# fonzcastellanos/scalable-video-codec

Measured on AMD Instinct MI355X. Metric: encoded frames/sec (1080p, 16x16 HBMA+DCT), higher is better.
Workload: dtype u8 (SAD, integer argmin) / f64 accumulate -> f32 (DCT, quant)

## Files before the change

### include/svc_hip.h

```cpp
#ifndef SVC_HIP_H
#define SVC_HIP_H

#include <stdint.h>

#ifdef __cplusplus
extern "C" {
#endif

typedef enum svc_status {
  SVC_OK = 0,
  SVC_ERR_INVALID_ARG = 1,
  SVC_ERR_UNSUPPORTED = 2,
  SVC_ERR_HIP = 3,
  SVC_ERR_NO_DEVICE = 4
} svc_status;

typedef struct svc_ransac_params {
  uint32_t subset_sz;
  float inlier_thresh;
  float success_prob;
  float inlier_ratio;
} svc_ransac_params;

typedef struct svc_segment_params {
// ... 4 lines not shown
  uint32_t max_iter_count;
  float epsilon;
  uint32_t connectivity;
} svc_segment_params;

#define SVC_HBMA_AUTO 0u
#define SVC_HBMA_FORCE_WAVE_PER_BLOCK 1u
#define SVC_HBMA_FORCE_FUSED 2u
#define SVC_HBMA_FORCE_TILED 4u
#define SVC_HBMA_FORCE_LANE 8u

const char* svc_hip_last_error(void);
int svc_hip_abi_version(void);
int svc_hip_device_count(int* count);

#define SVC_HOST_KEEP_LARGE_BLOCKS 1u
#define SVC_HOST_ONE_ARENA 2u
int svc_hip_tune_host_allocator(uint32_t flags);
int svc_hip_host_tuning_requested(void);

int svc_hip_probe_stream(const void* d_in, void* d_out, uint64_t bytes, uint32_t reads,
                         uint32_t writes, void* stream);

uint64_t svc_hip_pyramid_bytes(uint32_t frame_w, uint32_t frame_h, uint32_t level_count);


int svc_hip_hbma_pairs(const uint8_t* d_tracked, const uint8_t* d_anchor,
                       uint64_t pair_stride_bytes, uint32_t n_pairs,
                       uint32_t level_count, uint32_t frame_w, uint32_t frame_h,
                       uint32_t search_range, uint32_t block_w, uint32_t block_h,
                       float* d_mv_xy, float* d_min_mad, uint32_t flags,
                       void* stream);

const char* svc_hip_hbma_kernel_name(uint32_t level_count, uint32_t frame_w, uint32_t frame_h,
                                     uint32_t search_range, uint32_t block_w, uint32_t block_h,
                                     uint32_t flags);

int svc_hip_ebma_pairs(const uint8_t* d_tracked, const uint8_t* d_anchor,
                       uint64_t pair_stride_bytes, uint32_t n_pairs,
                       uint32_t frame_w, uint32_t frame_h, uint32_t search_range,
                       uint32_t block_w, uint32_t block_h, float* d_mv_xy,
                       float* d_min_mad, void* stream);

uint32_t svc_hip_ransac_iter_count(svc_ransac_params params);

int svc_hip_ransac_frames(const float* d_mv_xy, uint32_t blocks, uint32_t n_frames,
                          svc_ransac_params params, const uint32_t* d_samples,
                          uint32_t iter_count, float* d_gm_xy, float* d_rmse,
                          uint8_t* d_inlier_mask, uint32_t* d_inlier_count,
                          void* stream);

#define SVC_LAUNCH_BESIDE 1u
#define SVC_LAUNCH_NO_FORK 2u
#define SVC_LAUNCH_WIDE 4u
#define SVC_LAUNCH_NO_WIDE 8u
#define SVC_LAUNCH_DEFER_RMSE 16u
int svc_hip_ransac_frames_ex(const float* d_mv_xy, uint32_t blocks, uint32_t n_frames,
                             svc_ransac_params params, const uint32_t* d_samples,
                             uint32_t iter_count, float* d_gm_xy, float* d_rmse,
                             uint8_t* d_inlier_mask, uint32_t* d_inlier_count, uint32_t flags,
                             void* stream);

int svc_hip_ransac_rmse_frames(const float* d_mv_xy, uint32_t blocks, uint32_t n_frames,
                               svc_ransac_params params, const float* d_gm_xy,
                               const uint8_t* d_inlier_mask, const uint32_t* d_inlier_count,
                               float* d_rmse, void* stream);

int svc_hip_block_types_frames(const uint8_t* d_inlier_mask, uint32_t blocks,
                               uint32_t n_frames, uint32_t* d_block_types,
                               void* stream);

uint64_t svc_hip_segment_workspace_bytes(uint32_t mv_field_w, uint32_t mv_field_h,
                                         uint32_t n_frames, uint32_t attempt_count);

int svc_hip_segment_frames(const uint8_t* d_inlier_mask, const float* d_mv_xy,
                           uint32_t mv_field_w, uint32_t mv_field_h, uint32_t n_frames,
                           uint32_t mv_block_w, uint32_t mv_block_h,
                           svc_segment_params params, uint64_t seed,
                           uint8_t* d_workspace, uint64_t workspace_bytes,
                           uint32_t* d_block_types, void* stream);

int svc_hip_segment_frames_ex(const uint8_t* d_inlier_mask, const float* d_mv_xy,
                              uint32_t mv_field_w, uint32_t mv_field_h, uint32_t n_frames,
                              uint32_t mv_block_w, uint32_t mv_block_h,
                              svc_segment_params params, uint64_t seed,
                              uint8_t* d_workspace, uint64_t workspace_bytes,
                              uint32_t* d_block_types, uint32_t flags, void* stream);


int svc_hip_dct_frames(const uint8_t* d_bgr, uint64_t frame_stride_bytes,
                       uint32_t n_frames, uint32_t frame_w, uint32_t frame_h,
                       uint32_t block_w, uint32_t block_h, float* d_planes,
                       void* stream);

int svc_hip_dct_quant_frames(const uint8_t* d_bgr, uint64_t frame_stride_bytes,
                             uint32_t n_frames, uint32_t frame_w, uint32_t frame_h,
                             uint32_t block_w, uint32_t block_h,
                             const uint32_t* d_block_types, uint32_t mv_block_w,
                             uint32_t mv_block_h, uint32_t fg_step,
                             uint32_t bg_step, float* d_planes, void* stream);

int svc_hip_quant(float* d_coeffs, uint64_t n, uint32_t step, void* stream);

int svc_hip_quant_frames(float* d_planes, uint32_t n_frames, uint32_t frame_w,
                         uint32_t frame_h, uint32_t mv_block_w, uint32_t mv_block_h,
                         const uint32_t* d_block_types, uint32_t fg_step,
                         uint32_t bg_step, void* stream);


typedef struct svc_wire_header {
  uint32_t frame_count;
  uint32_t frame_w;
  uint32_t frame_h;
  uint32_t frame_excess_w;
  uint32_t frame_excess_h;
  uint32_t transform_block_w;
  uint32_t transform_block_h;
  uint32_t channel_count;
} svc_wire_header;

int svc_hip_wire_header(uint32_t clip_frame_count, uint32_t frame_w, uint32_t frame_h,
                        uint32_t mv_block_w, uint32_t mv_block_h, uint32_t level_count,
                        uint32_t transform_block_w, uint32_t transform_block_h,
                        svc_wire_header* out);

uint64_t svc_hip_serialized_frame_bytes(uint32_t frame_w, uint32_t frame_h,
                                        uint32_t transform_block_w, uint32_t transform_block_h);

int svc_hip_serialize_frames(const float* d_planes, uint64_t plane_elems, uint32_t n_frames,
                             const uint32_t* d_block_types, uint32_t frame_w, uint32_t frame_h,
                             uint32_t transform_block_w, uint32_t transform_block_h,
                             uint32_t mv_field_w, uint32_t mv_field_h, uint32_t mv_block_w,
                             uint32_t mv_block_h, uint8_t* d_out, uint64_t out_stride_bytes,
                             void* stream);

int svc_hip_dct_records_frames(const uint8_t* d_bgr, uint64_t frame_stride_bytes,
                               uint32_t n_frames, uint32_t frame_w, uint32_t frame_h,
                               uint32_t block, const uint32_t* d_block_types,
                               uint32_t mv_block_w, uint32_t mv_block_h, uint32_t fg_step,
                               uint32_t bg_step, uint32_t emit_frame_h, uint8_t* d_records,
                               uint64_t records_stride_bytes, void* stream);

int svc_hip_dct_records_luma_frames(const uint8_t* d_bgr, uint64_t frame_stride_bytes, uint32_t n_frames,
                                    uint32_t frame_w, uint32_t frame_h, uint32_t block, uint32_t emit_frame_h,
                                    uint8_t* d_records, uint64_t records_stride_bytes, uint8_t* d_pyr,
                                    uint64_t pyr_stride_bytes, void* stream);
int svc_hip_wire_patch_types_frames(const uint32_t* d_block_types, uint32_t n_frames, uint32_t frame_w, uint32_t frame_h,
                                    uint32_t emit_frame_h, uint32_t block, uint32_t mv_block_w, uint32_t mv_block_h,
                                    uint8_t* d_records, uint64_t records_stride_bytes, int all_tiles, void* stream);

int svc_hip_dct_quant_luma_frames(const uint8_t* d_bgr, uint64_t frame_stride_bytes, uint32_t n_frames, uint32_t frame_w,
                                  uint32_t frame_h, uint32_t block, uint32_t bg_step, float* d_planes, uint8_t* d_pyr,
                                  uint64_t pyr_stride_bytes, void* stream);
int svc_hip_count_foreground(const uint32_t* d_block_types, uint64_t n, uint32_t* d_count, void* stream);
uint64_t svc_hip_dct_redo_workspace_bytes(uint32_t n_frames, uint32_t frame_w, uint32_t frame_h, uint32_t mv_block_w,
                                          uint32_t mv_block_h);
int svc_hip_dct_quant_redo_frames(const uint8_t* d_bgr, uint64_t frame_stride_bytes, uint32_t n_frames, uint32_t frame_w,
                                  uint32_t frame_h, uint32_t block, const uint32_t* d_block_types, uint32_t mv_block_w,
                                  uint32_t mv_block_h, uint32_t fg_step, float* d_planes, uint8_t* d_ws, uint64_t ws_bytes,
                                  void* stream);

int svc_hip_decode_frames(const float* d_planes, uint32_t n_frames, uint32_t frame_w,
                          uint32_t frame_h, uint32_t block, const uint32_t* d_block_types,
                          uint32_t mv_block_w, uint32_t mv_block_h, uint32_t fg_step,
                          uint32_t bg_step, uint32_t gaze_x, uint32_t gaze_y, uint32_t gaze_w,
                          uint32_t gaze_h, float* d_bgr_f32, void* stream);

int svc_hip_sse_frames(const uint8_t* d_src_bgr, uint64_t src_frame_stride_bytes,
                       const float* d_rec_bgr_f32, uint32_t n_frames, uint32_t frame_w,
                       uint32_t frame_h, uint32_t region_w, uint32_t region_h, uint64_t* d_sse,
                       void* stream);


uint64_t svc_hip_levels_max_bytes(uint32_t n_frames, uint32_t frame_w, uint32_t frame_h,
                                  uint32_t block_w, uint32_t block_h, uint32_t mv_block_w,
                                  uint32_t mv_block_h);

uint64_t svc_hip_pack_levels_workspace_bytes(uint32_t n_frames, uint32_t frame_w,
                                             uint32_t frame_h, uint32_t block_w,
                                             uint32_t block_h);

int svc_hip_pack_levels_frames(const float* d_planes, const uint32_t* d_block_types,
                               uint32_t n_frames, uint32_t frame_w, uint32_t frame_h,
                               uint32_t block_w, uint32_t block_h, uint32_t mv_block_w,
                               uint32_t mv_block_h, uint32_t fg_step, uint32_t bg_step,
                               uint8_t* d_workspace, uint64_t workspace_bytes, uint8_t* d_out,
                               uint64_t out_capacity, uint64_t* d_frame_offsets, void* stream);

int svc_hip_unpack_levels_frames(const uint8_t* d_frames, uint64_t stream_bytes,
                                 const uint64_t* d_frame_offsets, uint32_t n_frames,
                                 uint32_t frame_w, uint32_t frame_h, uint32_t block_w,
                                 uint32_t block_h, uint32_t mv_block_w, uint32_t mv_block_h,
                                 uint8_t* d_workspace, uint64_t workspace_bytes, float* d_planes,
                                 uint32_t* d_block_types, uint32_t* d_status, void* stream);

int svc_hip_levels_drain(const uint8_t* d_frames, const uint64_t* d_frame_offsets,
                         uint32_t n_frames, uint32_t frame_w, uint32_t frame_h,
                         uint32_t block_w, uint32_t block_h, uint32_t mv_block_w,
                         uint32_t mv_block_h, void* host_dst, uint64_t capacity, void* stream);

uint64_t svc_hip_dct_pack_levels_workspace_bytes(uint32_t n_frames, uint32_t frame_w,
                                                 uint32_t frame_h, uint32_t block,
                                                 uint32_t mv_block_w, uint32_t mv_block_h);
int svc_hip_dct_pack_levels_frames(const uint8_t* d_bgr, uint64_t frame_stride_bytes,
                                   uint32_t n_frames, uint32_t frame_w, uint32_t frame_h,
                                   uint32_t block, const uint32_t* d_block_types,
                                   uint32_t mv_block_w, uint32_t mv_block_h, uint32_t fg_step,
                                   uint32_t bg_step, uint8_t* d_workspace,
                                   uint64_t workspace_bytes, uint8_t* d_out,
                                   uint64_t out_capacity, uint64_t* d_frame_offsets,
                                   void* stream);


uint64_t svc_hip_entropy_max_bytes(uint32_t n_frames, uint32_t frame_w, uint32_t frame_h, uint32_t block_w,
                                   uint32_t block_h, uint32_t mv_block_w, uint32_t mv_block_h);
uint64_t svc_hip_entropy_workspace_bytes(uint32_t n_frames, uint32_t frame_w, uint32_t frame_h, uint32_t block_w,
                                         uint32_t block_h, uint32_t mv_block_w, uint32_t mv_block_h);

int svc_hip_entropy_encode_frames(const uint8_t* d_svcq, uint64_t svcq_bytes, const uint64_t* d_svcq_offsets,
                                  uint32_t n_frames, uint32_t frame_w, uint32_t frame_h, uint32_t block_w,
                                  uint32_t block_h, uint32_t mv_block_w, uint32_t mv_block_h, uint8_t* d_workspace,
                                  uint64_t workspace_bytes, uint8_t* d_out, uint64_t out_capacity,
                                  uint64_t* d_out_offsets, uint32_t* d_status, void* stream);

int svc_hip_entropy_decode_frames(const uint8_t* d_svce, uint64_t svce_bytes, const uint64_t* d_offsets,
                                  uint32_t n_frames, uint32_t frame_w, uint32_t frame_h, uint32_t block_w,
                                  uint32_t block_h, uint32_t mv_block_w, uint32_t mv_block_h, uint8_t* d_workspace,
                                  uint64_t workspace_bytes, uint8_t* d_svcq_out, uint64_t capacity,
                                  uint64_t* d_svcq_offsets, uint32_t* d_status, void* stream);

int svc_hip_entropy_drain(const uint8_t* d_frames, const uint64_t* d_frame_offsets, uint32_t n_frames,
                          uint32_t frame_w, uint32_t frame_h, uint32_t block_w, uint32_t block_h,
                          uint32_t mv_block_w, uint32_t mv_block_h, void* host_dst, uint64_t capacity,
                          void* stream);

typedef struct {
  uint32_t fg_step, bg_step;
} svc_step_pair;

uint64_t svc_hip_pack_levels_budget_workspace_bytes(uint32_t n_frames, uint32_t frame_w, uint32_t frame_h,
                                                    uint32_t block_w, uint32_t block_h, uint32_t ladder_len);
int svc_hip_pack_levels_budget_frames(const float* d_planes, const uint32_t* d_block_types, uint32_t n_frames,
                                      uint32_t frame_w, uint32_t frame_h, uint32_t block_w, uint32_t block_h,
                                      uint32_t mv_block_w, uint32_t mv_block_h,
                                      const svc_step_pair* ladder , uint32_t ladder_len,
                                      const uint32_t* d_budget ,
                                      uint8_t* d_workspace, uint64_t workspace_bytes, uint8_t* d_out, uint64_t out_capacity,
                                      uint64_t* d_frame_offsets, uint32_t* d_choice , void* stream);

uint64_t svc_hip_dct_pack_levels_budget_workspace_bytes(uint32_t n_frames, uint32_t frame_w, uint32_t frame_h,
                                                        uint32_t block, uint32_t mv_block_w, uint32_t mv_block_h,
                                                        uint32_t ladder_len);
int svc_hip_dct_pack_levels_budget_frames(const uint8_t* d_bgr, uint64_t frame_stride_bytes, uint32_t n_frames,
                                          uint32_t frame_w, uint32_t frame_h, uint32_t block,
                                          const uint32_t* d_block_types, uint32_t mv_block_w, uint32_t mv_block_h,
                                          const svc_step_pair* ladder , uint32_t ladder_len,
                                          const uint32_t* d_budget ,
                                          uint8_t* d_workspace, uint64_t workspace_bytes, uint8_t* d_out, uint64_t out_capacity,
                                          uint64_t* d_frame_offsets, uint32_t* d_choice , void* stream);

uint64_t svc_hip_decode_levels_workspace_bytes(uint32_t n_frames, uint32_t frame_w,
                                               uint32_t frame_h, uint32_t block_w,
                                               uint32_t block_h);
int svc_hip_decode_levels_frames(const uint8_t* d_frames, uint64_t stream_bytes,
                                 const uint64_t* d_frame_offsets, uint32_t n_frames,
                                 uint32_t frame_w, uint32_t frame_h, uint32_t block_w,
                                 uint32_t block_h, uint32_t mv_block_w, uint32_t mv_block_h,
                                 uint32_t fg_step, uint32_t bg_step,
                                 const uint32_t* d_gaze ,
                                 uint8_t* d_workspace, uint64_t workspace_bytes,
                                 float* d_rec ,
                                 uint8_t* d_display ,
                                 uint32_t display_w, uint32_t display_h, uint32_t* d_status,
                                 void* stream);

int svc_hip_gaze_rect(uint32_t cx, uint32_t cy, uint32_t max_w, uint32_t max_h, uint32_t frame_w,
                      uint32_t frame_h, uint32_t padded_w, uint32_t padded_h,
                      uint32_t out_xywh[4]);

int svc_hip_decode_records_frames(const uint8_t* d_records, uint64_t records_stride_bytes, uint32_t n_frames,
                                  uint32_t frame_w, uint32_t frame_h , uint32_t block,
                                  uint32_t emit_frame_h, uint32_t fg_step, uint32_t bg_step,
                                  const uint32_t* d_gaze ,
                                  float* d_rec, uint8_t* d_display, uint32_t display_w, uint32_t display_h,
                                  void* stream);

int svc_hip_wire_layout(const svc_wire_header* hdr, uint64_t stream_bytes, uint32_t* emit_frame_h,
                        uint64_t* frame_bytes);

int svc_hip_luma_pyramid_frames(const uint8_t* d_bgr, uint64_t frame_stride_bytes,
                                uint32_t n_frames, uint32_t frame_w,
                                uint32_t frame_h, uint32_t level_count,
                                uint8_t* d_pyr, uint64_t pyr_stride_bytes,
                                void* stream);
int svc_hip_pyramid_levels_frames(uint8_t* d_pyr, uint64_t pyr_stride_bytes, uint32_t n_frames, uint32_t frame_w,
                                  uint32_t frame_h, uint32_t level_count, void* stream);

uint64_t svc_hip_global_ebma_workspace_bytes(uint32_t search_range, uint32_t n_pairs);

int svc_hip_global_ebma_pairs(const uint8_t* d_tracked, const uint8_t* d_anchor,
                              uint64_t pair_stride_bytes, uint32_t n_pairs, uint32_t frame_w,
                              uint32_t frame_h, uint32_t search_range, uint8_t* d_workspace,
                              uint64_t workspace_bytes, float* d_gm_xy, float* d_min_mad,
                              void* stream);

int svc_hip_global_avg_frames(const float* d_mv_xy, uint32_t blocks, uint32_t n_frames,
                              float* d_avg_xy, void* stream);

#define SVC_COMM_ID_BYTES 128u
#define SVC_SHIFT_CYCLIC 1u

int svc_hip_comm_available(void);
int svc_hip_comm_info(void* comm, uint32_t* ranks, uint32_t* rank, int32_t* device);
int svc_hip_comm_unique_id(uint8_t id[SVC_COMM_ID_BYTES]);
int svc_hip_comm_create(const uint8_t id[SVC_COMM_ID_BYTES], uint32_t rank, uint32_t world,
                        void** comm);
int svc_hip_comm_destroy(void* comm);

int svc_hip_halo_shift(void* comm, const uint8_t* d_send, uint8_t* d_recv, uint64_t bytes,
                       uint32_t rank, uint32_t world, uint32_t flags, void* stream);

int svc_hip_hbma_host(const uint8_t* const* tracked_pyr,
                      const uint8_t* const* anchor_pyr, uint32_t level_count,
                      uint32_t frame_w, uint32_t frame_h, uint32_t search_range,
                      uint32_t block_w, uint32_t block_h, float* mv_xy,
                      float* min_mad, uint32_t flags);

int svc_hip_ebma_host(const uint8_t* tracked, const uint8_t* anchor,
                      uint32_t frame_w, uint32_t frame_h, uint32_t search_range,
                      uint32_t block_w, uint32_t block_h, float* mv_xy,
                      float* min_mad);

int svc_hip_ransac_host(const float* mv_xy, uint32_t blocks,
                        svc_ransac_params params, const uint32_t* samples,
                        uint32_t iter_count, float* gm_xy, float* rmse,
                        uint32_t* inlier_indices, uint32_t* inlier_count);

int svc_hip_dct_host(const uint8_t* bgr, uint32_t frame_w, uint32_t frame_h,
                     uint32_t block_w, uint32_t block_h, float* planes);

int svc_hip_dct_planes_host(const uint8_t* bgr, uint32_t frame_w, uint32_t frame_h, uint32_t block_w,
                            uint32_t block_h, float* const planes[3]);


int svc_hip_bgr2yuv_host(const uint8_t* bgr, uint32_t w, uint32_t h, uint8_t* yuv);

int svc_hip_build_pyramid_host(const uint8_t* level0, uint32_t w, uint32_t h, uint32_t level_count,
                               uint8_t* const* out_levels);

#define SVC_MORPH_ERODE 0u
#define SVC_MORPH_DILATE 1u
#define SVC_MORPH_OPEN 2u
#define SVC_MORPH_CLOSE 3u
int svc_hip_morph_rect_host(const uint8_t* src, uint32_t w, uint32_t h, uint32_t kernel_w, uint32_t kernel_h,
                            uint32_t op, uint8_t* dst);

int svc_hip_kmeans_host(const float* features, uint32_t n, uint32_t dims, uint32_t k, uint32_t attempts,
                        uint32_t max_iter, float epsilon, uint64_t seed, int32_t* labels, double* compactness);

int svc_hip_connected_components_host(const uint8_t* image, uint32_t w, uint32_t h, uint32_t connectivity,
                                      int32_t* labels, uint32_t* count);

int svc_hip_dct_tiles_host(float* image, uint32_t w, uint32_t h, uint32_t block_w, uint32_t block_h,
                           const uint32_t* tiles_xy, uint32_t n_tiles);

int svc_hip_dct_quant_host(const uint8_t* bgr, uint32_t frame_w, uint32_t frame_h,
                           uint32_t block_w, uint32_t block_h,
                           const uint32_t* block_types, uint32_t mv_block_w,
                           uint32_t mv_block_h, uint32_t fg_step, uint32_t bg_step,
                           float* planes);

int svc_hip_quant_host(float* coeffs, uint64_t n, uint32_t step);

int svc_hip_global_ebma_host(const uint8_t* tracked, const uint8_t* anchor, uint32_t frame_w,
                             uint32_t frame_h, uint32_t search_range, float* gm_xy,
                             float* min_mad);

int svc_hip_global_hbma_host(const uint8_t* const* tracked_pyr,
                             const uint8_t* const* anchor_pyr, uint32_t level_count,
                             uint32_t frame_w, uint32_t frame_h, uint32_t search_range,
                             float* gm_xy);

int svc_hip_global_avg_host(const float* mv_xy, uint32_t blocks, float* avg_xy);

#ifdef __cplusplus
}
#endif

#endif
```

### scalable_video_codec_amd/csrc/capi.hip

```cpp
#include <algorithm>
#include <cmath>
#include <cstdlib>
#include <cstring>

#include <malloc.h>

#include "host/copy_crew.hpp"

#include <vector>
#include "svc_common.hpp"

namespace svc {

static thread_local char g_err[kErrBufSize] = "";
char* last_error_buf() { return g_err; }

bool fused_supported(uint32_t levels, uint32_t w, uint32_t h, uint32_t range, uint32_t bw, uint32_t bh);
bool tiled_supported(uint32_t levels, uint32_t w, uint32_t h, uint32_t range, uint32_t bw, uint32_t bh);
bool tiled_is_default();
int launch_hbma_fused(const uint8_t*, const uint8_t*, uint64_t, uint32_t, uint32_t, uint32_t, uint32_t,
                      uint32_t, uint32_t mv_block, float*, float*, int kernel, hipStream_t);
int launch_hbma_wave(const uint8_t*, const uint8_t*, uint64_t, uint32_t, uint32_t, uint32_t, uint32_t,
                     uint32_t, uint32_t, uint32_t, float*, float*, hipStream_t);

// ... 363 lines not shown
              (unsigned long long)svc_hip_segment_workspace_bytes(mv_field_w, mv_field_h, n_frames, params.attempt_count));
  SVC_REQUIRE(aligned(d_workspace, 16) && aligned(d_mv_xy, 8), "segment: workspace must be 16-byte, motion field 8-byte aligned");
  return launch_segment(d_inlier_mask, d_mv_xy, mv_field_w, mv_field_h, n_frames, mv_block_w, mv_block_h, params,
                        seed, d_workspace, d_block_types, flags, static_cast<hipStream_t>(stream));
}

static int validate_dct(const void* in, const void* out, uint32_t w, uint32_t h, uint32_t bw, uint32_t bh) {
  SVC_REQUIRE(in && out, "dct: null pointer");
  SVC_REQUIRE(bw > 0 && bh > 0, "dct: block must be positive (encoder.cpp:325-326)");
  SVC_REQUIRE(w > 0 && h > 0 && w % bw == 0 && h % bh == 0, "dct: frame %ux%u not divisible by block %ux%u", w, h, bw, bh);
  return SVC_OK;
}

static int validate_dct_alignment(const uint8_t* d_bgr, uint64_t frame_stride, const float* d_planes, uint32_t w, uint32_t bw,
                                  uint32_t bh) {
  if (bw == bh && (bw == 8 || bw == 16) && w % 16 == 0)
    SVC_REQUIRE(aligned(d_bgr, 16) && frame_stride % 16 == 0 && aligned(d_planes, 8),
                "dct: frames must be 16-byte aligned (stride too), planes 8-byte aligned");
  else
    SVC_REQUIRE(aligned(d_planes, 4), "dct: planes must be 4-byte aligned");
  return SVC_OK;
}

int svc_hip_dct_frames(const uint8_t* d_bgr, uint64_t frame_stride_bytes, uint32_t n_frames, uint32_t frame_w,
                       uint32_t frame_h, uint32_t block_w, uint32_t block_h, float* d_planes, void* stream) {
  if (n_frames == 0) return SVC_OK;
  int rc = validate_dct(d_bgr, d_planes, frame_w, frame_h, block_w, block_h);
  if (rc) return rc;
  rc = validate_dct_alignment(d_bgr, frame_stride_bytes, d_planes, frame_w, block_w, block_h);
  if (rc) return rc;
  return launch_dct(d_bgr, frame_stride_bytes, n_frames, frame_w, frame_h, block_w, block_h, nullptr, 0, 0, 1, 1,
                    false, d_planes, static_cast<hipStream_t>(stream));
}

int svc_hip_dct_quant_frames(const uint8_t* d_bgr, uint64_t frame_stride_bytes, uint32_t n_frames,
                             uint32_t frame_w, uint32_t frame_h, uint32_t block_w, uint32_t block_h,
                             const uint32_t* d_block_types, uint32_t mv_block_w, uint32_t mv_block_h,
                             uint32_t fg_step, uint32_t bg_step, float* d_planes, void* stream) {
  if (n_frames == 0) return SVC_OK;
  int rc = validate_dct(d_bgr, d_planes, frame_w, frame_h, block_w, block_h);
  if (rc) return rc;
  SVC_REQUIRE(d_block_types, "dct_quant: null block types");
  SVC_REQUIRE(fg_step > 0 && bg_step > 0, "dct_quant: quant steps must be positive (decoder.cpp:35-47)");
  SVC_REQUIRE(mv_block_w > 0 && mv_block_h > 0 && mv_block_w % block_w == 0 && mv_block_h % block_h == 0 &&
                  frame_w % mv_block_w == 0 && frame_h % mv_block_h == 0,
              "dct_quant: MV block %ux%u must be a multiple of the transform block %ux%u and divide the frame",
              mv_block_w, mv_block_h, block_w, block_h);
  rc = validate_dct_alignment(d_bgr, frame_stride_bytes, d_planes, frame_w, block_w, block_h);
  if (rc) return rc;
  return launch_dct(d_bgr, frame_stride_bytes, n_frames, frame_w, frame_h, block_w, block_h, d_block_types,
                    mv_block_w, mv_block_h, fg_step, bg_step, true, d_planes, static_cast<hipStream_t>(stream));
}

int svc_hip_dct_records_frames(const uint8_t* d_bgr, uint64_t frame_stride_bytes, uint32_t n_frames,
                               uint32_t frame_w, uint32_t frame_h, uint32_t block, const uint32_t* d_block_types,
                               uint32_t mv_block_w, uint32_t mv_block_h, uint32_t fg_step, uint32_t bg_step,
                               uint32_t emit_frame_h, uint8_t* d_records, uint64_t records_stride_bytes,
                               void* stream) {
  if (n_frames == 0) return SVC_OK;
  int rc = validate_dct(d_bgr, d_records, frame_w, frame_h, block, block);
  if (rc) return rc;
  SVC_REQUIRE(d_block_types, "dct_records: null block types");
  SVC_REQUIRE((fg_step == 0) == (bg_step == 0), "dct_records: give both quant steps or neither (0, 0 = no quant)");
  SVC_REQUIRE(mv_block_w > 0 && mv_block_h > 0 && mv_block_w % block == 0 && mv_block_h % block == 0 &&
                  frame_w % mv_block_w == 0 && frame_h % mv_block_h == 0,
              "dct_records: MV block %ux%u must be a multiple of the transform block %u and divide the frame",
              mv_block_w, mv_block_h, block);
  SVC_REQUIRE(emit_frame_h > 0 && emit_frame_h <= frame_h, "dct_records: emit_frame_h %u outside (0, %u]", emit_frame_h, frame_h);
  SVC_REQUIRE(aligned(d_bgr, 16) && frame_stride_bytes % 16 == 0 && aligned(d_records, 4) && records_stride_bytes % 4 == 0 &&
                  records_stride_bytes >= svc_hip_serialized_frame_bytes(frame_w, emit_frame_h, block, block),
              "dct_records: frames must be 16-byte aligned; records 4-byte aligned with a stride of at least one frame");
  const bool quant = fg_step != 0;
  return launch_dct(d_bgr, frame_stride_bytes, n_frames, frame_w, frame_h, block, block, d_block_types, mv_block_w,
                    mv_block_h, quant ? fg_step : 1, quant ? bg_step : 1, quant, nullptr,
                    static_cast<hipStream_t>(stream), d_records, records_stride_bytes, emit_frame_h);
}

int svc_hip_decode_frames(const float* d_planes, uint32_t n_frames, uint32_t frame_w, uint32_t frame_h,
                          uint32_t block, const uint32_t* d_block_types, uint32_t mv_block_w, uint32_t mv_block_h,
                          uint32_t fg_step, uint32_t bg_step, uint32_t gaze_x, uint32_t gaze_y, uint32_t gaze_w,
                          uint32_t gaze_h, float* d_bgr_f32, void* stream) {
  if (n_frames == 0) return SVC_OK;
  SVC_REQUIRE(d_planes && d_block_types && d_bgr_f32, "decode: null pointer");
  SVC_REQUIRE(block > 0 && frame_w > 0 && frame_h > 0 && frame_w % block == 0 && frame_h % block == 0,
              "decode: frame %ux%u not divisible by block %u", frame_w, frame_h, block);
  SVC_REQUIRE(fg_step > 0 && bg_step > 0, "decode: quant steps must be positive (libs/decoder.cpp:35-47)");
  SVC_REQUIRE(mv_block_w > 0 && mv_block_h > 0 && mv_block_w % block == 0 && mv_block_h % block == 0 &&
                  frame_w % mv_block_w == 0 && frame_h % mv_block_h == 0,
              "decode: MV block %ux%u must be a multiple of the transform block %u and divide the frame", mv_block_w, mv_block_h, block);
  SVC_REQUIRE(aligned(d_planes, 16) && aligned(d_bgr_f32, 8), "decode: planes must be 16-byte, output 8-byte aligned");
  return launch_decode(d_planes, n_frames, frame_w, frame_h, block, d_block_types, mv_block_w, mv_block_h, fg_step,
                       bg_step, gaze_x, gaze_y, gaze_w, gaze_h, d_bgr_f32, static_cast<hipStream_t>(stream));
}

int svc_hip_sse_frames(const uint8_t* d_src_bgr, uint64_t src_frame_stride_bytes, const float* d_rec_bgr_f32,
                       uint32_t n_frames, uint32_t frame_w, uint32_t frame_h, uint32_t region_w, uint32_t region_h,
                       uint64_t* d_sse, void* stream) {
  if (n_frames == 0) return SVC_OK;
  SVC_REQUIRE(d_src_bgr && d_rec_bgr_f32 && d_sse, "sse: null pointer");
  SVC_REQUIRE(region_w > 0 && region_h > 0 && region_w <= frame_w && region_h <= frame_h,
              "sse: region %ux%u outside the frame %ux%u", region_w, region_h, frame_w, frame_h);
  SVC_REQUIRE(aligned(d_sse, 8), "sse: output must be 8-byte aligned");
  return launch_sse(d_src_bgr, src_frame_stride_bytes, d_rec_bgr_f32, n_frames, frame_w, frame_h, region_w, region_h,
                    d_sse, static_cast<hipStream_t>(stream));
}

int svc_hip_quant(float* d_coeffs, uint64_t n, uint32_t step, void* stream) {
  SVC_REQUIRE(d_coeffs || n == 0, "quant: null pointer");
  SVC_REQUIRE(step > 0, "quant: step must be positive (decoder.cpp:35-47)");
  return launch_quant(d_coeffs, n, step, static_cast<hipStream_t>(stream));
}

int svc_hip_quant_frames(float* d_planes, uint32_t n_frames, uint32_t frame_w, uint32_t frame_h,
                         uint32_t mv_block_w, uint32_t mv_block_h, const uint32_t* d_block_types,
                         uint32_t fg_step, uint32_t bg_step, void* stream) {
  if (n_frames == 0) return SVC_OK;
  SVC_REQUIRE(d_planes && d_block_types, "quant_frames: null pointer");
  SVC_REQUIRE(fg_step > 0 && bg_step > 0, "quant_frames: steps must be positive");
  SVC_REQUIRE(mv_block_w > 0 && mv_block_h > 0 && frame_w % mv_block_w == 0 && frame_h % mv_block_h == 0,
              "quant_frames: frame %ux%u not divisible by MV block %ux%u", frame_w, frame_h, mv_block_w, mv_block_h);
  return launch_quant_frames(d_planes, n_frames, frame_w, frame_h, mv_block_w, mv_block_h, d_block_types,
                             fg_step, bg_step, static_cast<hipStream_t>(stream));
}

int svc_hip_luma_pyramid_frames(const uint8_t* d_bgr, uint64_t frame_stride_bytes, uint32_t n_frames,
                                uint32_t frame_w, uint32_t frame_h, uint32_t level_count, uint8_t* d_pyr,
                                uint64_t pyr_stride_bytes, void* stream) {
  if (n_frames == 0) return SVC_OK;
  SVC_REQUIRE(d_bgr && d_pyr, "luma_pyramid: null pointer");
  SVC_REQUIRE(level_count > 0 && level_count <= 16, "luma_pyramid: level_count %u out of range", level_count);
  const uint32_t f = 1u << (level_count - 1);
  SVC_REQUIRE(frame_w > 0 && frame_h > 0 && frame_w % f == 0 && frame_h % f == 0,
              "luma_pyramid: frame %ux%u must be divisible by 2^(levels-1) = %u", frame_w, frame_h, f);
  SVC_REQUIRE(aligned(d_bgr, 16) && frame_stride_bytes % 16 == 0 && aligned(d_pyr, 16) && pyr_stride_bytes % 16 == 0,
              "luma_pyramid: frames and pyramids must be 16-byte aligned (strides too)");
  SVC_REQUIRE(n_frames <= 1 || pyr_stride_bytes >= pyramid_bytes(frame_w, frame_h, level_count),
              "luma_pyramid: pyramid stride too small");
  return launch_luma_pyramid(d_bgr, frame_stride_bytes, n_frames, frame_w, frame_h, level_count, d_pyr,
                             pyr_stride_bytes, static_cast<hipStream_t>(stream));
}

int svc_hip_pyramid_levels_frames(uint8_t* d_pyr, uint64_t pyr_stride_bytes, uint32_t n_frames, uint32_t frame_w, uint32_t frame_h,
                                  uint32_t level_count, void* stream) {
  if (n_frames == 0) return SVC_OK;
  SVC_REQUIRE(d_pyr, "pyramid_levels: null pointer");
  SVC_REQUIRE(level_count > 0 && level_count <= 16, "pyramid_levels: level_count %u out of range", level_count);
  const uint32_t f = 1u << (level_count - 1);
  SVC_REQUIRE(frame_w > 0 && frame_h > 0 && frame_w % f == 0 && frame_h % f == 0,
              "pyramid_levels: frame %ux%u must be divisible by 2^(levels-1) = %u", frame_w, frame_h, f);
  SVC_REQUIRE(n_frames <= 1 || pyr_stride_bytes >= pyramid_bytes(frame_w, frame_h, level_count), "pyramid_levels: pyramid stride too small");
  return launch_pyr_down_levels(d_pyr, pyr_stride_bytes, n_frames, frame_w, frame_h, level_count, 0, static_cast<hipStream_t>(stream));
}

int svc_hip_dct_records_luma_frames(const uint8_t* d_bgr, uint64_t frame_stride_bytes, uint32_t n_frames, uint32_t frame_w,
                                    uint32_t frame_h, uint32_t block, uint32_t emit_frame_h, uint8_t* d_records,
                                    uint64_t records_stride_bytes, uint8_t* d_pyr, uint64_t pyr_stride_bytes, void* stream) {
  if (n_frames == 0) return SVC_OK;
  int rc = validate_dct(d_bgr, d_records, frame_w, frame_h, block, block);
  if (rc) return rc;
  SVC_REQUIRE(d_pyr, "dct_records_luma: null pyramid");
  SVC_REQUIRE(emit_frame_h > 0 && emit_frame_h <= frame_h, "dct_records_luma: emit_frame_h %u outside (0, %u]", emit_frame_h, frame_h);
  SVC_REQUIRE(aligned(d_bgr, 16) && frame_stride_bytes % 16 == 0 && aligned(d_records, 4) && records_stride_bytes % 4 == 0 &&
                  records_stride_bytes >= svc_hip_serialized_frame_bytes(frame_w, emit_frame_h, block, block),
              "dct_records_luma: frames must be 16-byte aligned; records 4-byte aligned with a stride of at least one frame");
  SVC_REQUIRE(aligned(d_pyr, 16) && pyr_stride_bytes % 16 == 0 && (n_frames <= 1 || pyr_stride_bytes >= (uint64_t)frame_w * frame_h),
              "dct_records_luma: pyramids must be 16-byte aligned (stride too), a stride of at least one luma plane");
  return launch_dct(d_bgr, frame_stride_bytes, n_frames, frame_w, frame_h, block, block, nullptr, block, block, 1, 1, false, nullptr,
                    static_cast<hipStream_t>(stream), d_records, records_stride_bytes, emit_frame_h, d_pyr, pyr_stride_bytes);
}

int svc_hip_dct_quant_luma_frames(const uint8_t* d_bgr, uint64_t frame_stride_bytes, uint32_t n_frames, uint32_t frame_w,
                                  uint32_t frame_h, uint32_t block, uint32_t bg_step, float* d_planes, uint8_t* d_pyr,
                                  uint64_t pyr_stride_bytes, void* stream) {
  if (n_frames == 0) return SVC_OK;
  int rc = validate_dct(d_bgr, d_planes, frame_w, frame_h, block, block);
  if (rc) return rc;
  SVC_REQUIRE(d_pyr, "dct_quant_luma: null pyramid");
  SVC_REQUIRE(bg_step > 0, "dct_quant_luma: quant step must be positive (libs/decoder.cpp:35-47)");
  if ((rc = validate_dct_alignment(d_bgr, frame_stride_bytes, d_planes, frame_w, block, block))) return rc;
  SVC_REQUIRE(aligned(d_pyr, 16) && pyr_stride_bytes % 16 == 0 && (n_frames <= 1 || pyr_stride_bytes >= (uint64_t)frame_w * frame_h),
              "dct_quant_luma: pyramids must be 16-byte aligned (stride too), a stride of at least one luma plane");
  return launch_dct_quant_speculative(d_bgr, frame_stride_bytes, n_frames, frame_w, frame_h, block, bg_step, d_planes, d_pyr,
                                      pyr_stride_bytes, static_cast<hipStream_t>(stream));
}

int svc_hip_count_foreground(const uint32_t* d_block_types, uint64_t n, uint32_t* d_count, void* stream) {
  SVC_REQUIRE(d_count && (d_block_types || n == 0), "count_foreground: null pointer");
  return launch_count_foreground(d_block_types, n, d_count, static_cast<hipStream_t>(stream));
}

uint64_t svc_hip_dct_redo_workspace_bytes(uint32_t n_frames, uint32_t frame_w, uint32_t frame_h, uint32_t mv_block_w, uint32_t mv_block_h) {
  if (!mv_block_w || !mv_block_h) return 0;
  return dct_redo_workspace_bytes(n_frames, (frame_w / mv_block_w) * (frame_h / mv_block_h));
}

int svc_hip_dct_quant_redo_frames(const uint8_t* d_bgr, uint64_t frame_stride_bytes, uint32_t n_frames, uint32_t frame_w, uint32_t frame_h,
                                  uint32_t block, const uint32_t* d_block_types, uint32_t mv_block_w, uint32_t mv_block_h,
                                  uint32_t fg_step, float* d_planes, uint8_t* d_ws, uint64_t ws_bytes, void* stream) {
  if (n_frames == 0) return SVC_OK;
  int rc = validate_dct(d_bgr, d_planes, frame_w, frame_h, block, block);
  if (rc) return rc;
  SVC_REQUIRE(d_block_types && d_ws, "dct_quant_redo: null pointer");
  SVC_REQUIRE(fg_step > 0, "dct_quant_redo: quant step must be positive (libs/decoder.cpp:35-47)");
  SVC_REQUIRE(mv_block_w > 0 && mv_block_h > 0 && mv_block_w % block == 0 && mv_block_h % block == 0 &&
                  frame_w % mv_block_w == 0 && frame_h % mv_block_h == 0,
              "dct_quant_redo: MV block %ux%u must be a multiple of the transform block %u and divide the frame", mv_block_w, mv_block_h, block);
  if ((rc = validate_dct_alignment(d_bgr, frame_stride_bytes, d_planes, frame_w, block, block))) return rc;
  SVC_REQUIRE(aligned(d_ws, 16) && ws_bytes >= svc_hip_dct_redo_workspace_bytes(n_frames, frame_w, frame_h, mv_block_w, mv_block_h),
              "dct_quant_redo: workspace must be 16-byte aligned and hold svc_hip_dct_redo_workspace_bytes()");
  return launch_dct_quant_redo_foreground(d_bgr, frame_stride_bytes, n_frames, frame_w, frame_h, block, d_block_types, mv_block_w, mv_block_h,
                                          fg_step, d_planes, d_ws, static_cast<hipStream_t>(stream));
}

int svc_hip_wire_patch_types_frames(const uint32_t* d_block_types, uint32_t n_frames, uint32_t frame_w, uint32_t frame_h,
                                    uint32_t emit_frame_h, uint32_t block, uint32_t mv_block_w, uint32_t mv_block_h, uint8_t* d_records,
                                    uint64_t records_stride_bytes, int all_tiles, void* stream) {
  if (n_frames == 0) return SVC_OK;
  SVC_REQUIRE(d_block_types && d_records, "wire_patch_types: null pointer");
  SVC_REQUIRE(block > 0 && frame_w > 0 && frame_h > 0 && frame_w % block == 0 && frame_h % block == 0 && block <= 64,
              "wire_patch_types: frame %ux%u not divisible by block %u", frame_w, frame_h, block);
  SVC_REQUIRE(mv_block_w > 0 && mv_block_h > 0 && mv_block_w % block == 0 && mv_block_h % block == 0 &&
                  frame_w % mv_block_w == 0 && frame_h % mv_block_h == 0,
              "wire_patch_types: MV block %ux%u must be a multiple of the transform block %u and divide the frame", mv_block_w, mv_block_h, block);
  SVC_REQUIRE(emit_frame_h > 0 && emit_frame_h <= frame_h, "wire_patch_types: emit_frame_h %u outside (0, %u]", emit_frame_h, frame_h);
  SVC_REQUIRE(aligned(d_records, 4) && records_stride_bytes % 4 == 0 &&
                  records_stride_bytes >= svc_hip_serialized_frame_bytes(frame_w, emit_frame_h, block, block),
              "wire_patch_types: records 4-byte aligned with a stride of at least one frame");
  return launch_wire_patch_types(d_block_types, n_frames, frame_w, frame_h, emit_frame_h, block, mv_block_w, mv_block_h, d_records,
                                 records_stride_bytes, all_tiles != 0, static_cast<hipStream_t>(stream));
}


static int validate_global_ebma(uint32_t w, uint32_t h, uint32_t range) {
  SVC_REQUIRE(w > 0 && h > 0, "global ebma: frame %ux%u must be positive", w, h);
  SVC_REQUIRE(range < w && range < h, "global ebma: search range %u must be smaller than the frame %ux%u (motion.cpp:63-64)", range, w, h);
  SVC_REQUIRE(range <= 1024, "global ebma: search range %u out of range", range);
  return SVC_OK;
}

uint64_t svc_hip_global_ebma_workspace_bytes(uint32_t search_range, uint32_t n_pairs) {
  return global_ebma_workspace_bytes(search_range, n_pairs);
}

int svc_hip_global_ebma_pairs(const uint8_t* d_tracked, const uint8_t* d_anchor, uint64_t pair_stride_bytes, uint32_t n_pairs,
                              uint32_t frame_w, uint32_t frame_h, uint32_t search_range, uint8_t* d_workspace,
                              uint64_t workspace_bytes, float* d_gm_xy, float* d_min_mad, void* stream) {
  if (n_pairs == 0) return SVC_OK;
  SVC_REQUIRE(d_tracked && d_anchor && d_gm_xy && d_workspace, "global ebma: null pointer (motion.cpp:58-61)");
  int rc = validate_global_ebma(frame_w, frame_h, search_range);
  if (rc) return rc;
  SVC_REQUIRE(workspace_bytes >= global_ebma_workspace_bytes(search_range, n_pairs) && aligned(d_workspace, 8),
              "global ebma: workspace too small or not 8-byte aligned");
  return launch_global_ebma(d_tracked, d_anchor, pair_stride_bytes, n_pairs, frame_w, frame_h, search_range, d_workspace,
                            d_gm_xy, d_min_mad, false, static_cast<hipStream_t>(stream));
}

int svc_hip_global_avg_frames(const float* d_mv_xy, uint32_t blocks, uint32_t n_frames, float* d_avg_xy, void* stream) {
  if (n_frames == 0) return SVC_OK;
  SVC_REQUIRE(d_mv_xy && d_avg_xy, "global avg: null pointer (motion.cpp:46)");
  return launch_global_avg(d_mv_xy, blocks, n_frames, d_avg_xy, static_cast<hipStream_t>(stream));
}

int svc_hip_hbma_host(const uint8_t* const* tracked_pyr, const uint8_t* const* anchor_pyr, uint32_t level_count,
                      uint32_t frame_w, uint32_t frame_h, uint32_t search_range, uint32_t block_w,
                      uint32_t block_h, float* mv_xy, float* min_mad, uint32_t flags) {
  SVC_REQUIRE(tracked_pyr && anchor_pyr && mv_xy && min_mad, "hbma: null pointer (motion.cpp:417-420)");
  int rc = validate_hbma(level_count, frame_w, frame_h, search_range, block_w, block_h);
  if (rc) return rc;
  for (uint32_t l = 0; l < level_count; ++l)
    SVC_REQUIRE(tracked_pyr[l] && anchor_pyr[l], "hbma: null plane at level %u", l);
  if ((rc = require_device())) return rc;
  const size_t pyr = up256(pyramid_bytes(frame_w, frame_h, level_count));
  const size_t blocks = (size_t)(frame_w / block_w) * (frame_h / block_h);
  const size_t out_off = 2 * pyr, out_bytes = blocks * 12;
  if ((rc = g_stage.ensure(out_off + up256(out_bytes)))) return rc;
  size_t o = 0;
  for (uint32_t l = 0; l < level_count; ++l) {
    const size_t n = (size_t)(frame_w >> l) * (frame_h >> l);
    host_copy(g_stage.pin + o, tracked_pyr[l], n);
    host_copy(g_stage.pin + pyr + o, anchor_pyr[l], n);
    o += n;
  }
  SVC_HIP_TRY(hipMemcpyAsync(g_stage.dev, g_stage.pin, 2 * pyr, hipMemcpyHostToDevice, g_stage.stream));
  float* d_mv = reinterpret_cast<float*>(g_stage.dev + out_off);
  float* d_mad = d_mv + 2 * blocks;
  rc = launch_hbma(g_stage.dev, g_stage.dev + pyr, pyr, 1, level_count, frame_w, frame_h, search_range, block_w,
                   block_h, d_mv, d_mad, flags, g_stage.stream);
  if (rc) return rc;
  SVC_HIP_TRY(hipMemcpyAsync(g_stage.pin + out_off, d_mv, out_bytes, hipMemcpyDeviceToHost, g_stage.stream));
  SVC_HIP_TRY(hipStreamSynchronize(g_stage.stream));
  std::memcpy(mv_xy, g_stage.pin + out_off, blocks * 8);
  std::memcpy(min_mad, g_stage.pin + out_off + blocks * 8, blocks * 4);
  return SVC_OK;
}

int svc_hip_ebma_host(const uint8_t* tracked, const uint8_t* anchor, uint32_t frame_w, uint32_t frame_h,
                      uint32_t search_range, uint32_t block_w, uint32_t block_h, float* mv_xy, float* min_mad) {
  SVC_REQUIRE(tracked && anchor && mv_xy && min_mad, "ebma: null pointer (motion.cpp:273-276)");
  SVC_REQUIRE(block_w > 0 && block_h > 0, "ebma: block must be positive (motion.cpp:278-279)");
  SVC_REQUIRE(frame_w > 0 && frame_h > 0 && frame_w % block_w == 0 && frame_h % block_h == 0,
              "ebma: frame %ux%u not divisible by block %ux%u (motion.cpp:281-282)", frame_w, frame_h, block_w, block_h);
  int rc = require_device();
  if (rc) return rc;
  const size_t plane = up256((size_t)frame_w * frame_h);
  const size_t blocks = (size_t)(frame_w / block_w) * (frame_h / block_h);
  const size_t out_off = 2 * plane, out_bytes = blocks * 12;
  if ((rc = g_stage.ensure(out_off + up256(out_bytes)))) return rc;
  host_copy(g_stage.pin, tracked, (size_t)frame_w * frame_h);
  host_copy(g_stage.pin + plane, anchor, (size_t)frame_w * frame_h);
  SVC_HIP_TRY(hipMemcpyAsync(g_stage.dev, g_stage.pin, 2 * plane, hipMemcpyHostToDevice, g_stage.stream));
  float* d_mv = reinterpret_cast<float*>(g_stage.dev + out_off);
  float* d_mad = d_mv + 2 * blocks;
  rc = launch_ebma(g_stage.dev, g_stage.dev + plane, plane, 1, frame_w, frame_h, search_range, block_w, block_h,
                   d_mv, d_mad, g_stage.stream);
  if (rc) return rc;
  SVC_HIP_TRY(hipMemcpyAsync(g_stage.pin + out_off, d_mv, out_bytes, hipMemcpyDeviceToHost, g_stage.stream));
  SVC_HIP_TRY(hipStreamSynchronize(g_stage.stream));
  std::memcpy(mv_xy, g_stage.pin + out_off, blocks * 8);
  std::memcpy(min_mad, g_stage.pin + out_off + blocks * 8, blocks * 4);
  return SVC_OK;
}

int svc_hip_ransac_host(const float* mv_xy, uint32_t blocks, svc_ransac_params params, const uint32_t* samples,
                        uint32_t iter_count, float* gm_xy, float* rmse, uint32_t* inlier_indices,
                        uint32_t* inlier_count) {
  SVC_REQUIRE(mv_xy && gm_xy && rmse && inlier_indices && inlier_count, "ransac: null pointer (motion.cpp:189-192)");
  SVC_REQUIRE(iter_count == 0 || samples, "ransac: null samples");
  SVC_REQUIRE(params.subset_sz > 0 && blocks >= params.subset_sz,
              "ransac: motion field of %u smaller than subset %u (motion.cpp:194)", blocks, params.subset_sz);
  for (size_t i = 0; i < (size_t)iter_count * params.subset_sz; ++i)
    SVC_REQUIRE(samples[i] < blocks, "ransac: sample index %u out of range [0, %u)", samples[i], blocks);
  int rc = require_device();
  if (rc) return rc;
  const size_t mv_b = up256((size_t)blocks * 8), smp_b = up256((size_t)iter_count * params.subset_sz * 4 + 4);
  const size_t mask_b = up256(blocks), misc_b = 256;
  if ((rc = g_stage.ensure(mv_b + smp_b + mask_b + misc_b))) return rc;
// ... 168 lines not shown
```

### scalable_video_codec_amd/csrc/dct.hip

```cpp
#include <algorithm>

#include "dct_core.hpp"
#include "luma16.hpp"
#include "quant_core.hpp"
#include "svc_common.hpp"

namespace svc {

struct DctArgs {
  const uint8_t* bgr;
  uint64_t frame_stride;
  uint32_t w, h;
  uint32_t segs_per_band;
  uint32_t bands_per_frame;
  uint32_t total_segcols;
  float* planes;
  const uint32_t* types;
  uint32_t mv_bw, mv_bh, mfw, mv_blocks;
  float fg_step, bg_step;
  float fg_inv, bg_inv;
  uint8_t* records;
  uint64_t records_stride;
  uint32_t emit_bands;
  uint8_t* luma;
  uint64_t luma_stride;
  const uint32_t* fg_list;
  const uint32_t* fg_count;
  uint32_t segs_per_block_x, segs_per_block;
};



constexpr int kSlabWire8 = 1664, kSlabWire16 = 3200;

typedef uint32_t u32x4_a4 __attribute__((ext_vector_type(4), aligned(4)));

template <int N, bool QUANT, bool WIRE, bool LUMA = false, int SPEC = 0>
__global__ __launch_bounds__(256) void dct_kernel(DctArgs a) {
  static_assert(!LUMA || (WIRE && !QUANT) || (QUANT && !WIRE && SPEC == 1), "the luma by-product rides on the raw-coefficient record emitter or on the speculative quantiser");
  static_assert(SPEC == 0 || (QUANT && !WIRE), "speculation is about the quantiser's step");
  constexpr int kSegPerWg = 256 / N;
  constexpr int kSlab = WIRE ? (N == 8 ? kSlabWire8 : kSlabWire16) : (N == 8 ? kSlab8 : kSlab16);
  __shared__ __attribute__((aligned(16))) uint8_t lds[kSegPerWg * kSlab];

  const uint32_t tid = threadIdx.x;
  const uint32_t sc_local = tid / N, j = tid % N;
  uint32_t n_units = 1, unit = 0;
  if (SPEC == 2) {
    const uint32_t total = *a.fg_count * a.segs_per_block;
    n_units = (total + kSegPerWg - 1) / kSegPerWg;
    unit = blockIdx.x;
  }
  for (; unit < n_units; unit += SPEC == 2 ? gridDim.x : 1u) {
  uint32_t gsc, frame, band, seg;
  if (SPEC == 2) {
    gsc = unit * kSegPerWg + sc_local;
    if (gsc >= *a.fg_count * a.segs_per_block) break;
    const uint32_t item = a.fg_list[gsc / a.segs_per_block], sub = gsc % a.segs_per_block;
    frame = item / a.mv_blocks;
    const uint32_t b = item - frame * a.mv_blocks, by = b / a.mfw, bx = b - by * a.mfw;
    band = by * (a.mv_bh / N) + sub / a.segs_per_block_x;
    seg = bx * a.segs_per_block_x + sub % a.segs_per_block_x;
  } else {
    gsc = xcd_contiguous_block(blockIdx.x, gridDim.x) * kSegPerWg + sc_local;
    if (gsc >= a.total_segcols) return;
    const uint32_t band_g = gsc / a.segs_per_band;
    seg = gsc - band_g * a.segs_per_band;
    frame = band_g / a.bands_per_frame;
    band = band_g - frame * a.bands_per_frame;
  }
  const uint32_t y_pix = band * N, x_pix = seg * 16;

  const uint8_t* src = a.bgr + (size_t)frame * a.frame_stride +
                       ((size_t)(y_pix + j) * a.w + x_pix) * 3;
  uint32_t wds[12];
  {
    const uint4* p = reinterpret_cast<const uint4*>(src);
    uint4 v0 = p[0], v1 = p[1], v2 = p[2];
    wds[0] = v0.x; wds[1] = v0.y; wds[2] = v0.z; wds[3] = v0.w;
    wds[4] = v1.x; wds[5] = v1.y; wds[6] = v1.z; wds[7] = v1.w;
    wds[8] = v2.x; wds[9] = v2.y; wds[10] = v2.z; wds[11] = v2.w;
  }

  if (LUMA) {
    uint32_t y16[4];
    luma16(wds, y16);
    *reinterpret_cast<uint4*>(a.luma + (size_t)frame * a.luma_stride + (size_t)(y_pix + j) * a.w + x_pix) = make_uint4(y16[0], y16[1], y16[2], y16[3]);
  }

  uint8_t* slab = lds + sc_local * kSlab;
  float* out_frame = a.planes + (size_t)frame * 3 * a.w * a.h;

  float step = 1.f, inv_step = 1.f;
  uint32_t t = SPEC == 2 ? 1u : 0u;
  if ((QUANT || WIRE) && !LUMA && SPEC == 0) {
    const uint32_t col = N == 8 ? x_pix + 2 * j : x_pix + j;
    t = a.types[(size_t)frame * a.mv_blocks + (y_pix / a.mv_bh) * a.mfw + col / a.mv_bw];
  }
  if (QUANT) {
    step = t == 0 ? a.bg_step : a.fg_step;
    inv_step = t == 0 ? a.bg_inv : a.fg_inv;
  }
  constexpr uint32_t kRec = 4 + 12 * N * N;
  const bool emit = WIRE && band < a.emit_bands;
  uint8_t* rec0 = nullptr;
  if (WIRE) {
    const uint32_t tiles_x = a.w / N, tile0 = band * tiles_x + (N == 8 ? 2 * seg : seg);
    rec0 = a.records + (size_t)frame * a.records_stride + (size_t)tile0 * kRec;
  }
  float keep[WIRE ? 3 : 1][16];

#pragma unroll
  for (int c = 0; c < 3; ++c) {
    int x[16];
    double r[16];
#pragma unroll
    for (int p = 0; p < 16; ++p) x[p] = (int)((wds[(3 * p + c) >> 2] >> (8 * ((3 * p + c) & 3))) & 0xFFu);
    if (N == 8) {
      dct1d<8, int>(x, r);
      dct1d<8, int>(x + 8, r + 8);
    } else {
      dct1d<16, int>(x, r);
    }
    double2* row = reinterpret_cast<double2*>(slab + j * kRowPitch);
#pragma unroll
    for (int i = 0; i < 8; ++i) row[i] = make_double2(r[2 * i], r[2 * i + 1]);
    wave_lds_sync();

    float* plane = out_frame + (size_t)c * a.w * a.h;
    if (N == 8) {
      double ca[8], cb[8], ya[8], yb[8];
#pragma unroll
      for (int y = 0; y < 8; ++y) {
        double2 t = *reinterpret_cast<const double2*>(slab + y * kRowPitch + j * 16);
        ca[y] = t.x;
        cb[y] = t.y;
      }
      dct1d<8, double>(ca, ya);
      dct1d<8, double>(cb, yb);
      float* dst = plane + (size_t)y_pix * a.w + x_pix + 2 * j;
#pragma unroll
      for (int v = 0; v < 8; ++v) {
        float fa = (float)ya[v], fb = (float)yb[v];
        if (QUANT) {
          const f32x2 qq = quant2_fast(f32x2{fa, fb}, step, inv_step);
          fa = qq.x; fb = qq.y;
        }
        if (WIRE) { keep[WIRE ? c : 0][2 * v] = fa; keep[WIRE ? c : 0][2 * v + 1] = fb; }
        else *reinterpret_cast<float2*>(dst + (size_t)v * a.w) = make_float2(fa, fb);
      }
    } else {
      double cc[16], yy[16];
#pragma unroll
      for (int y = 0; y < 16; ++y)
        cc[y] = *reinterpret_cast<const double*>(slab + y * kRowPitch + j * 8);
      dct1d<16, double>(cc, yy);
      float* dst = plane + (size_t)y_pix * a.w + x_pix + j;
#pragma unroll
      for (int v = 0; v < 16; v += 2) {
        f32x2 f = {(float)yy[v], (float)yy[v + 1]};
        if (QUANT) f = quant2_fast(f, step, inv_step);
        if (WIRE) {
          keep[WIRE ? c : 0][v] = f.x;
          keep[WIRE ? c : 0][v + 1] = f.y;
        } else {
          dst[(size_t)v * a.w] = f.x;
          dst[(size_t)(v + 1) * a.w] = f.y;
        }
      }
    }
    wave_lds_sync();
  }

  if constexpr (WIRE) {
    constexpr uint32_t kGroupBytes = N == 8 ? 2 * kRec : kRec;
    constexpr uint32_t kGroups = 64 / N;
    constexpr uint32_t kWaveBytes = kGroups * kGroupBytes;
    static_assert(kGroups * (uint32_t)kSlab >= kWaveBytes + 16, "a wave's slabs hold its stretch of the stream plus alignment slack");
    const uint32_t lane = tid & 63u, g = lane / N;
    const uint32_t gsc_last = gsc - g + kGroups - 1;
    bool stretch = gsc_last < a.total_segcols;
    if (stretch) {
      const uint32_t bg_last = gsc_last / a.segs_per_band, bg_first = (gsc - g) / a.segs_per_band;
      const uint32_t f_last = bg_last / a.bands_per_frame;
      stretch = f_last == bg_first / a.bands_per_frame && bg_last - f_last * a.bands_per_frame < a.emit_bands;
    }
    const uint32_t q = N == 8 ? j >> 2 : 0u;
    const uint32_t col_off = N == 8 ? (j & 3u) * 8u : j * 4u;
    if (stretch) {
      uint8_t* wave_rec = rec0 - (size_t)g * kGroupBytes;
      const uint32_t delta = (uint32_t)(reinterpret_cast<uintptr_t>(wave_rec) & 15u);
      uint8_t* wbase = lds + (sc_local - g) * kSlab + delta;
      uint8_t* mine = wbase + g * kGroupBytes + q * kRec;
      if (N == 8 ? (j & 3u) == 0 : j == 0) *reinterpret_cast<uint32_t*>(mine) = t;
#pragma unroll
      for (int c = 0; c < 3; ++c)
#pragma unroll
        for (int v = 0; v < N; ++v) {
          uint32_t* d = reinterpret_cast<uint32_t*>(mine + 4 + c * (4 * N * N) + v * (4 * N) + col_off);
          if (N == 8) { d[0] = __float_as_uint(keep[c][2 * v]); d[1] = __float_as_uint(keep[c][2 * v + 1]); }
          else d[0] = __float_as_uint(keep[c][v]);
        }
      wave_lds_sync();
      const uint32_t head = (16u - delta) & 15u;
      const uint32_t nfull = (kWaveBytes - head) / 16u, tail = (kWaveBytes - head) % 16u;
      for (uint32_t k = lane; k < nfull; k += 64u) {
        const uint32_t o = head + 16u * k;
        *reinterpret_cast<uint4*>(wave_rec + o) = *reinterpret_cast<const uint4*>(wbase + o);
      }
      const uint32_t hd = head / 4u, ne = hd + tail / 4u;
      if (lane < ne) {
        const uint32_t o = lane < hd ? 4u * lane : head + 16u * nfull + 4u * (lane - hd);
        *reinterpret_cast<uint32_t*>(wave_rec + o) = *reinterpret_cast<const uint32_t*>(wbase + o);
      }
    } else if (emit) {
      uint8_t* mine = rec0 + q * kRec;
      if (N == 8 ? (j & 3u) == 0 : j == 0) *reinterpret_cast<uint32_t*>(mine) = t;
#pragma unroll
      for (int c = 0; c < 3; ++c)
#pragma unroll
        for (int v = 0; v < N; ++v) {
          uint32_t* d = reinterpret_cast<uint32_t*>(mine + 4 + c * (4 * N * N) + v * (4 * N) + col_off);
          if (N == 8) { d[0] = __float_as_uint(keep[c][2 * v]); d[1] = __float_as_uint(keep[c][2 * v + 1]); }
          else d[0] = __float_as_uint(keep[c][v]);
        }
    }
  }
  }
}

__global__ __launch_bounds__(256) void fg_list_kernel(const uint32_t* types, uint32_t total_blocks, uint32_t* list, uint32_t* count) {
  const uint32_t g = blockIdx.x * 256u + threadIdx.x;
  const bool fg = g < total_blocks && types[g] != 0;
  const uint64_t m = __builtin_amdgcn_ballot_w64(fg);
  if (m == 0) return;
  const uint32_t lane = threadIdx.x & 63u, n = (uint32_t)__builtin_popcountll(m);
  uint32_t base = 0;
  if (lane == (uint32_t)__builtin_ctzll(m)) base = atomicAdd(count, n);
  base = __builtin_amdgcn_readlane(base, __builtin_ctzll(m));
  if (fg) list[base + (uint32_t)__builtin_popcountll(m & ((1ull << lane) - 1ull))] = g;
}

struct DctGenArgs {
  const uint8_t* bgr;
  uint64_t frame_stride;
  uint32_t w, h, bw, bh;
  uint32_t sw;
  uint32_t strips_per_band;
  uint32_t bands_per_frame;
  uint32_t total_strips;
  float* planes;
  const uint32_t* types;
  uint32_t mv_bw, mv_bh, mfw, mv_blocks;
  float fg_step, bg_step, fg_inv, bg_inv;
  uint8_t* records;
  uint64_t records_stride;
  uint32_t emit_bands;
};

__device__ __forceinline__ double dct_basis(uint32_t k, uint32_t n, uint32_t N) {
  const uint32_t j = ((2 * n + 1) * k) % (4 * N);
  const double s = k == 0 ? 1.0 / (double)N : 2.0 / (double)N;
  return __builtin_sqrt(s) * cospi((double)j / (double)(2 * N));
}

template <bool QUANT, bool WIRE>
__global__ __launch_bounds__(256) void dct_general_kernel(DctGenArgs a) {
  extern __shared__ __attribute__((aligned(16))) uint8_t gen_lds[];
  const uint32_t tid = threadIdx.x, bw = a.bw, bh = a.bh, sw = a.sw;
  const uint32_t pw = bw + 1, ph = bh + 1;
  double* cw = reinterpret_cast<double*>(gen_lds);
  double* ch = cw + bw * pw;
  double* yrow = ch + bh * ph;
  float* xin = reinterpret_cast<float*>(yrow + bh * sw);
  for (uint32_t i = tid; i < bw * bw; i += 256) cw[(i / bw) * pw + i % bw] = dct_basis(i / bw, i % bw, bw);
  for (uint32_t i = tid; i < bh * bh; i += 256) ch[(i / bh) * ph + i % bh] = dct_basis(i / bh, i % bh, bh);
  __syncthreads();
  for (uint32_t unit = blockIdx.x; unit < a.total_strips; unit += gridDim.x) {
    const uint32_t band_g = unit / a.strips_per_band, strip = unit - band_g * a.strips_per_band;
    const uint32_t frame = band_g / a.bands_per_frame, band = band_g - frame * a.bands_per_frame;
    const uint32_t y0 = band * bh, x0 = strip * sw;
    const uint32_t cols = a.w - x0 < sw ? a.w - x0 : sw;
    const uint32_t n = bh * cols;
    const uint8_t* src = a.bgr + (size_t)frame * a.frame_stride;
    float* out_frame = a.planes + (size_t)frame * 3 * a.w * a.h;
    for (uint32_t c = 0; c < 3; ++c) {
      for (uint32_t i = tid; i < n; i += 256) {
        const uint32_t r = i / cols, x = i - r * cols;
        xin[r * sw + x] = (float)src[((size_t)(y0 + r) * a.w + x0 + x) * 3 + c];
      }
      __syncthreads();
      for (uint32_t i = tid; i < n; i += 256) {
        const uint32_t r = i / cols, x = i - r * cols, u = x % bw;
        const float* xr = xin + r * sw + (x - u);
        const double* cr = cw + u * pw;
        double acc = 0.0;
        for (uint32_t k = 0; k < bw; ++k) acc = __builtin_fma(cr[k], (double)xr[k], acc);
        yrow[r * sw + x] = acc;
      }
      __syncthreads();
      float* plane = out_frame + (size_t)c * a.w * a.h;
      for (uint32_t i = tid; i < n; i += 256) {
        const uint32_t v = i / cols, x = i - v * cols;
        const double* cr = ch + v * ph;
        double acc = 0.0;
        for (uint32_t m = 0; m < bh; ++m) acc = __builtin_fma(cr[m], yrow[m * sw + x], acc);
        float f = (float)acc;
        uint32_t t = 0;
        if (QUANT || WIRE)
          t = a.types[(size_t)frame * a.mv_blocks + (y0 / a.mv_bh) * a.mfw + (x0 + x) / a.mv_bw];
        if (QUANT) f = quant1_fast(f, t == 0 ? a.bg_step : a.fg_step, t == 0 ? a.bg_inv : a.fg_inv);
        if (WIRE) {
          if (band < a.emit_bands) {
            const uint32_t u = x % bw, tile = band * (a.w / bw) + (x0 + x) / bw, rec_dw = 1 + 3 * bw * bh;
            uint32_t* rec = reinterpret_cast<uint32_t*>(a.records + (size_t)frame * a.records_stride) + (size_t)tile * rec_dw;
            rec[1 + c * bw * bh + v * bh + u] = __float_as_uint(f);
            if (c == 0 && v == 0 && u == 0) rec[0] = t;
          }
        } else {
          plane[(size_t)(y0 + v) * a.w + x0 + x] = f;
        }
      }
      __syncthreads();
    }
  }
}

constexpr uint32_t kDctGenMaxSide = 64;

static int launch_dct_general(const uint8_t* d_bgr, uint64_t frame_stride, uint32_t n_frames, uint32_t w, uint32_t h,
                              uint32_t bw, uint32_t bh, const uint32_t* d_types, uint32_t mv_bw, uint32_t mv_bh,
                              uint32_t fg_step, uint32_t bg_step, bool quant, float* d_planes, hipStream_t stream,
                              uint8_t* d_records = nullptr, uint64_t records_stride = 0, uint32_t emit_h = 0) {
  const bool wire = d_records != nullptr;
  if (wire && (bw != bh || w % bw != 0))
    return fail(SVC_ERR_UNSUPPORTED, "dct_records: the fused record emitter takes square transform blocks that divide the frame "
                                     "width; for %ux%u call svc_hip_dct[_quant]_frames, then svc_hip_serialize_frames", bw, bh);
  if ((bw > 1 && bw % 2) || (bh > 1 && bh % 2) || (bw == 1 && bh == 1))
    return fail(SVC_ERR_INVALID_ARG, "dct: transform block %ux%u: cv::dct implements even sizes only", bw, bh);
  if (bw > kDctGenMaxSide || bh > kDctGenMaxSide)
    return fail(SVC_ERR_UNSUPPORTED, "dct: transform block %ux%u exceeds %ux%u", bw, bh, kDctGenMaxSide, kDctGenMaxSide);
  DctGenArgs a{};
  a.bgr = d_bgr; a.frame_stride = frame_stride;
  a.w = w; a.h = h; a.bw = bw; a.bh = bh;
  uint32_t tiles = 4096 / (bw * bh);
  if (tiles < 1) tiles = 1;
  if (tiles > w / bw) tiles = w / bw;
  a.sw = tiles * bw;
  a.strips_per_band = div_up(w, a.sw);
  a.bands_per_frame = h / bh;
  const uint64_t total = (uint64_t)n_frames * a.strips_per_band * a.bands_per_frame;
  if (total == 0) return SVC_OK;
  if (total > 0x7FFFFFFFull) return fail(SVC_ERR_UNSUPPORTED, "dct: %llu strips exceed one launch", (unsigned long long)total);
  a.total_strips = (uint32_t)total;
  a.planes = d_planes;
  a.records = d_records;
  a.records_stride = records_stride;
  a.emit_bands = wire ? div_up(emit_h, bh) : 0;
  if (quant || wire) {
    a.types = d_types;
    a.mv_bw = mv_bw; a.mv_bh = mv_bh;
    a.mfw = w / mv_bw;
    a.mv_blocks = a.mfw * (h / mv_bh);
  }
  if (quant) {
    a.fg_step = (float)fg_step; a.bg_step = (float)bg_step;
    a.fg_inv = 1.0f / a.fg_step; a.bg_inv = 1.0f / a.bg_step;
  }
  const size_t lds = 8 * ((size_t)bw * (bw + 1) + (size_t)bh * (bh + 1) + (size_t)bh * a.sw) + 4 * (size_t)bh * a.sw;
  const uint32_t grid = (uint32_t)(total < 4096 ? total : 4096);
  if (wire) {
    if (quant) hipLaunchKernelGGL((dct_general_kernel<true, true>), dim3(grid), dim3(256), lds, stream, a);
    else hipLaunchKernelGGL((dct_general_kernel<false, true>), dim3(grid), dim3(256), lds, stream, a);
  } else {
    if (quant) hipLaunchKernelGGL((dct_general_kernel<true, false>), dim3(grid), dim3(256), lds, stream, a);
    else hipLaunchKernelGGL((dct_general_kernel<false, false>), dim3(grid), dim3(256), lds, stream, a);
  }
  return check_launch("dct_general_kernel");
}

int launch_dct(const uint8_t* d_bgr, uint64_t frame_stride, uint32_t n_frames, uint32_t w,
               uint32_t h, uint32_t bw, uint32_t bh, const uint32_t* d_types, uint32_t mv_bw,
               uint32_t mv_bh, uint32_t fg_step, uint32_t bg_step, bool quant, float* d_planes,
               hipStream_t stream, uint8_t* d_records, uint64_t records_stride, uint32_t emit_h, uint8_t* d_luma,
               uint64_t luma_stride) {
  const bool wire = d_records != nullptr;
  const bool fast = bw == bh && (bw == 8 || bw == 16) && w % 16 == 0;
  if (d_luma && !(fast && wire && !quant))
    return fail(SVC_ERR_UNSUPPORTED, "dct: the luma by-product needs the tuned record emitter (8x8 / 16x16 blocks, width a multiple of 16, no quant)");
  if (!fast)
    return launch_dct_general(d_bgr, frame_stride, n_frames, w, h, bw, bh, d_types, mv_bw, mv_bh, fg_step, bg_step, quant,
                              d_planes, stream, d_records, records_stride, emit_h);
  DctArgs a{};
  a.bgr = d_bgr;
  a.frame_stride = frame_stride;
  a.w = w; a.h = h;
  a.segs_per_band = w / 16;
  a.bands_per_frame = h / bh;
  const uint64_t total = (uint64_t)n_frames * a.segs_per_band * a.bands_per_frame;
  if (total == 0) return SVC_OK;
  if (total > 0x7FFFFFFFull) return fail(SVC_ERR_UNSUPPORTED, "dct: %llu segment columns exceed one launch", (unsigned long long)total);
  a.total_segcols = (uint32_t)total;
  a.planes = d_planes;
  a.records = d_records;
  a.records_stride = records_stride;
  a.emit_bands = wire ? div_up(emit_h, bh) : 0;
  a.luma = d_luma;
  a.luma_stride = luma_stride;
  if (quant || wire) {
    a.types = d_types;
    a.mv_bw = mv_bw; a.mv_bh = mv_bh;
    a.mfw = w / mv_bw;
    a.mv_blocks = a.mfw * (h / mv_bh);
  }
  if (quant) {
    a.fg_step = (float)fg_step;
    a.bg_step = (float)bg_step;
    a.fg_inv = 1.0f / a.fg_step;
    a.bg_inv = 1.0f / a.bg_step;
  }
  const uint32_t seg_per_wg = 256 / bw;
  const dim3 grid(div_up(a.total_segcols, seg_per_wg)), block(256);
#define SVC_DCT_LAUNCH(N_, Q_, W_) hipLaunchKernelGGL((dct_kernel<N_, Q_, W_>), grid, block, 0, stream, a)
  if (d_luma) {
    if (bw == 8) hipLaunchKernelGGL((dct_kernel<8, false, true, true>), grid, block, 0, stream, a);
    else hipLaunchKernelGGL((dct_kernel<16, false, true, true>), grid, block, 0, stream, a);
  } else if (bw == 8) {
    if (wire) { if (quant) SVC_DCT_LAUNCH(8, true, true); else SVC_DCT_LAUNCH(8, false, true); }
    else { if (quant) SVC_DCT_LAUNCH(8, true, false); else SVC_DCT_LAUNCH(8, false, false); }
  } else {
    if (wire) { if (quant) SVC_DCT_LAUNCH(16, true, true); else SVC_DCT_LAUNCH(16, false, true); }
    else { if (quant) SVC_DCT_LAUNCH(16, true, false); else SVC_DCT_LAUNCH(16, false, false); }
  }
#undef SVC_DCT_LAUNCH
  return check_launch("dct_kernel");
}

__global__ __launch_bounds__(256) void fg_count_kernel(const uint32_t* types, uint32_t total_blocks, uint32_t* count) {
  __shared__ uint32_t part[4];
  uint32_t n = 0;
  for (uint32_t g = blockIdx.x * 256u + threadIdx.x; g < total_blocks; g += gridDim.x * 256u) n += types[g] != 0 ? 1u : 0u;
#pragma unroll
  for (int o = 32; o > 0; o >>= 1) n += __shfl_down(n, o, 64);
  if ((threadIdx.x & 63u) == 0) part[threadIdx.x >> 6] = n;
  __syncthreads();
  if (threadIdx.x == 0) {
    const uint32_t s = part[0] + part[1] + part[2] + part[3];
    if (s) atomicAdd(count, s);
  }
}

int launch_count_foreground(const uint32_t* d_types, uint64_t n, uint32_t* d_count, hipStream_t stream) {
  hipError_t e = hipMemsetAsync(d_count, 0, 4, stream);
  if (e != hipSuccess) return fail(SVC_ERR_HIP, "count_foreground: hipMemsetAsync: %s", hipGetErrorString(e));
  if (n == 0) return SVC_OK;
  if (n > 0x7FFFFFFFull) return fail(SVC_ERR_UNSUPPORTED, "count_foreground: too many MV blocks for one launch");
  hipLaunchKernelGGL(fg_count_kernel, dim3(std::min<uint32_t>(div_up((uint32_t)n, 1024), 512u)), dim3(256), 0, stream, d_types, (uint32_t)n, d_count);
  return check_launch("fg_count_kernel");
}

static bool spec_shape_ok(uint32_t w, uint32_t block) { return (block == 8 || block == 16) && w % 16 == 0; }

int launch_dct_quant_speculative(const uint8_t* d_bgr, uint64_t frame_stride, uint32_t n_frames, uint32_t w, uint32_t h, uint32_t block,
                                 uint32_t bg_step, float* d_planes, uint8_t* d_luma, uint64_t luma_stride, hipStream_t stream) {
  if (!spec_shape_ok(w, block))
    return fail(SVC_ERR_UNSUPPORTED, "dct_quant_luma: the speculative form needs the tuned transform (8x8 / 16x16 blocks, width a multiple of 16)");
  DctArgs a{};
  a.bgr = d_bgr; a.frame_stride = frame_stride;
  a.w = w; a.h = h;
  a.segs_per_band = w / 16;
  a.bands_per_frame = h / block;
  const uint64_t total = (uint64_t)n_frames * a.segs_per_band * a.bands_per_frame;
  if (total == 0) return SVC_OK;
  if (total > 0x7FFFFFFFull) return fail(SVC_ERR_UNSUPPORTED, "dct: %llu segment columns exceed one launch", (unsigned long long)total);
  a.total_segcols = (uint32_t)total;
  a.planes = d_planes;
  a.luma = d_luma; a.luma_stride = luma_stride;
  a.fg_step = a.bg_step = (float)bg_step;
  a.fg_inv = a.bg_inv = 1.0f / a.bg_step;
  const dim3 grid(div_up(a.total_segcols, 256 / block)), blk(256);
  if (block == 8) hipLaunchKernelGGL((dct_kernel<8, true, false, true, 1>), grid, blk, 0, stream, a);
  else hipLaunchKernelGGL((dct_kernel<16, true, false, true, 1>), grid, blk, 0, stream, a);
  return check_launch("dct_kernel<speculative>");
}

uint64_t dct_redo_workspace_bytes(uint32_t n_frames, uint32_t mv_blocks) { return 16 + 4ull * n_frames * mv_blocks; }

int launch_dct_quant_redo_foreground(const uint8_t* d_bgr, uint64_t frame_stride, uint32_t n_frames, uint32_t w, uint32_t h, uint32_t block,
                                     const uint32_t* d_types, uint32_t mv_bw, uint32_t mv_bh, uint32_t fg_step, float* d_planes,
                                     uint8_t* d_ws, hipStream_t stream) {
  if (!spec_shape_ok(w, block) || mv_bw % 16 != 0 || mv_bh % block != 0)
    return fail(SVC_ERR_UNSUPPORTED, "dct_quant_redo: needs the tuned transform (8x8 / 16x16, width a multiple of 16) and MV blocks that are whole "
                                     "16-pixel segments wide and whole transform blocks tall");
  DctArgs a{};
  a.bgr = d_bgr; a.frame_stride = frame_stride;
  a.w = w; a.h = h;
  a.segs_per_band = w / 16;
  a.bands_per_frame = h / block;
  a.planes = d_planes;
  a.mv_bw = mv_bw; a.mv_bh = mv_bh;
  a.mfw = w / mv_bw;
  a.mv_blocks = a.mfw * (h / mv_bh);
  const uint64_t total_blocks = (uint64_t)n_frames * a.mv_blocks;
  if (total_blocks == 0) return SVC_OK;
  if (total_blocks * (mv_bw / 16) * (mv_bh / block) > 0x7FFFFFFFull) return fail(SVC_ERR_UNSUPPORTED, "dct_quant_redo: too many MV blocks for one launch");
  a.fg_step = a.bg_step = (float)fg_step;
  a.fg_inv = a.bg_inv = 1.0f / a.fg_step;
  uint32_t* count = reinterpret_cast<uint32_t*>(d_ws);
  uint32_t* list = reinterpret_cast<uint32_t*>(d_ws + 16);
  a.fg_count = count; a.fg_list = list;
  a.segs_per_block_x = mv_bw / 16;
  a.segs_per_block = a.segs_per_block_x * (mv_bh / block);
  hipError_t e = hipMemsetAsync(count, 0, 16, stream);
  if (e != hipSuccess) return fail(SVC_ERR_HIP, "dct_quant_redo: hipMemsetAsync: %s", hipGetErrorString(e));
  hipLaunchKernelGGL(fg_list_kernel, dim3(div_up((uint32_t)total_blocks, 256)), dim3(256), 0, stream, d_types, (uint32_t)total_blocks, list, count);
  int rc = check_launch("fg_list_kernel");
  if (rc) return rc;
  const uint64_t worst = div_up((uint32_t)(total_blocks * a.segs_per_block), 256 / block);
  const dim3 grid((uint32_t)std::min<uint64_t>(worst, 2048)), blk(256);
  if (block == 8) hipLaunchKernelGGL((dct_kernel<8, true, false, false, 2>), grid, blk, 0, stream, a);
  else hipLaunchKernelGGL((dct_kernel<16, true, false, false, 2>), grid, blk, 0, stream, a);
  return check_launch("dct_kernel<redo foreground>");
}

struct DctTilesArgs {
  float* img;
  const uint32_t* xy;
  uint32_t w, h, bw, bh, n_tiles, grid_w, tpb;
};

__global__ __launch_bounds__(256) void dct_tiles_kernel(DctTilesArgs a) {
  extern __shared__ __attribute__((aligned(16))) uint8_t tiles_lds[];
  const uint32_t tid = threadIdx.x, bw = a.bw, bh = a.bh, area = bw * bh;
  const uint32_t pw = bw + 1, ph = bh + 1;
  double* cw = reinterpret_cast<double*>(tiles_lds);
  double* ch = cw + bw * pw;
  double* yrow = ch + bh * ph;
  float* xin = reinterpret_cast<float*>(yrow + (size_t)a.tpb * area);
  for (uint32_t i = tid; i < bw * bw; i += 256) cw[(i / bw) * pw + i % bw] = dct_basis(i / bw, i % bw, bw);
  for (uint32_t i = tid; i < bh * bh; i += 256) ch[(i / bh) * ph + i % bh] = dct_basis(i / bh, i % bh, bh);
  __syncthreads();
  for (uint32_t base = blockIdx.x * a.tpb; base < a.n_tiles; base += gridDim.x * a.tpb) {
    const uint32_t nt = a.n_tiles - base < a.tpb ? a.n_tiles - base : a.tpb, ne = nt * area;
    auto origin = [&](uint32_t t, uint32_t& tx, uint32_t& ty) {
      const uint32_t g = base + t;
      if (a.xy) { tx = a.xy[2 * g]; ty = a.xy[2 * g + 1]; }
      else { ty = (g / a.grid_w) * bh; tx = (g % a.grid_w) * bw; }
    };
    for (uint32_t i = tid; i < ne; i += 256) {
      const uint32_t t = i / area, e = i - t * area, r = e / bw, u = e - r * bw;
      uint32_t tx, ty;
      origin(t, tx, ty);
      xin[i] = a.img[(size_t)(ty + r) * a.w + tx + u];
    }
    __syncthreads();
    for (uint32_t i = tid; i < ne; i += 256) {
      const uint32_t t = i / area, e = i - t * area, r = e / bw, u = e - r * bw;
      const float* xr = xin + t * area + r * bw;
      const double* cr = cw + u * pw;
      double acc = 0.0;
      for (uint32_t k = 0; k < bw; ++k) acc = __builtin_fma(cr[k], (double)xr[k], acc);
      yrow[i] = acc;
    }
    __syncthreads();
    for (uint32_t i = tid; i < ne; i += 256) {
      const uint32_t t = i / area, e = i - t * area, v = e / bw, u = e - v * bw;
      const double* cr = ch + v * ph;
      const double* yc = yrow + t * area + u;
      double acc = 0.0;
      for (uint32_t m = 0; m < bh; ++m) acc = __builtin_fma(cr[m], yc[m * bw], acc);
      uint32_t tx, ty;
      origin(t, tx, ty);
      a.img[(size_t)(ty + v) * a.w + tx + u] = (float)acc;
    }
    __syncthreads();
  }
}

int launch_dct_tiles(float* d_img, uint32_t w, uint32_t h, uint32_t bw, uint32_t bh, const uint32_t* d_xy, uint32_t n_tiles,
                     hipStream_t stream) {
  if ((bw > 1 && bw % 2) || (bh > 1 && bh % 2) || (bw == 1 && bh == 1) || bw == 0 || bh == 0)
    return fail(SVC_ERR_INVALID_ARG, "dct: transform block %ux%u: cv::dct implements even sizes only", bw, bh);
  if (bw > kDctGenMaxSide || bh > kDctGenMaxSide)
    return fail(SVC_ERR_UNSUPPORTED, "dct: transform block %ux%u exceeds %ux%u", bw, bh, kDctGenMaxSide, kDctGenMaxSide);
  if (n_tiles == 0) return SVC_OK;
  DctTilesArgs a{};
  a.img = d_img; a.xy = d_xy;
  a.w = w; a.h = h; a.bw = bw; a.bh = bh; a.n_tiles = n_tiles;
  a.grid_w = w / bw;
  uint32_t tpb = 4096 / (bw * bh);
  a.tpb = tpb < 1 ? 1 : tpb > 64 ? 64 : tpb;
  const size_t lds = 8 * ((size_t)bw * (bw + 1) + (size_t)bh * (bh + 1)) + (size_t)a.tpb * bw * bh * 12;
  const uint32_t trips = div_up(n_tiles, a.tpb);
  hipLaunchKernelGGL(dct_tiles_kernel, dim3(trips < 2048 ? trips : 2048), dim3(256), lds, stream, a);
  return check_launch("dct_tiles_kernel");
}


__global__ __launch_bounds__(256) void quant_kernel(float* c, uint64_t n, float step) {
  const uint64_t stride = (uint64_t)gridDim.x * 256 * 4;
  for (uint64_t i = ((uint64_t)blockIdx.x * 256 + threadIdx.x) * 4; i < n; i += stride) {
    if (i + 4 <= n && (reinterpret_cast<uintptr_t>(c + i) & 15) == 0) {
      float4 v = *reinterpret_cast<float4*>(c + i);
      v.x = quant1(v.x, step); v.y = quant1(v.y, step);
      v.z = quant1(v.z, step); v.w = quant1(v.w, step);
      *reinterpret_cast<float4*>(c + i) = v;
    } else {
      for (uint64_t k = i; k < n && k < i + 4; ++k) c[k] = quant1(c[k], step);
    }
  }
}

struct QuantFramesArgs {
  float* planes;
  const uint32_t* types;
  uint32_t w, h, mv_bw, mv_bh, mfw, mv_blocks;
  uint64_t total;
  float fg_step, bg_step;
};

__global__ __launch_bounds__(256) void quant_frames_kernel(QuantFramesArgs a) {
  const uint64_t stride = (uint64_t)gridDim.x * 256;
  const uint64_t plane_sz = (uint64_t)a.w * a.h;
  for (uint64_t i = (uint64_t)blockIdx.x * 256 + threadIdx.x; i < a.total; i += stride) {
    const uint64_t pl = i / plane_sz, rem = i - pl * plane_sz;
    const uint32_t frame = (uint32_t)(pl / 3);
    const uint32_t y = (uint32_t)(rem / a.w), x = (uint32_t)(rem - (uint64_t)y * a.w);
    const uint32_t t = a.types[(size_t)frame * a.mv_blocks + (y / a.mv_bh) * a.mfw + x / a.mv_bw];
    a.planes[i] = quant1(a.planes[i], t == 0 ? a.bg_step : a.fg_step);
  }
}

// ... 29 lines not shown
```

### scalable_video_codec_amd/csrc/host/clip_encoder.cpp

```cpp
#include "svc/clip_encoder.hpp"

#include <algorithm>
#include <cstring>
#include <stdexcept>
#include <string>
#include <utility>
#include <vector>

#include "encode_geometry.hpp"
#include "hip_raii.hpp"
#include "svc_clip.h"

namespace svc {
namespace {

using namespace host;

constexpr Who kWho{"svc::ClipEncoder"};
void Hip(hipError_t e, const char* what) { kWho.Hip(e, what); }
void Abi(int rc, const char* what) { kWho.Abi(rc, what); }
bool Ready(hipEvent_t e) { return kWho.Ready(e); }

constexpr uint32_t kStages = (uint32_t)Stage::kCount;

}

Shard PlanShard(uint32_t clip_frames, uint32_t world, uint32_t rank) {
  Shard s;
  if (world == 0 || rank >= world) return s;
  const uint32_t base = clip_frames / world, extra = clip_frames % world;
  s.frames = base + (rank < extra ? 1u : 0u);
  s.first_frame = rank * base + std::min(rank, extra);
  s.needs_halo = s.first_frame > 0 && s.frames > 0;
  s.pairs = s.frames == 0 ? 0 : s.frames - (s.needs_halo ? 0u : 1u);
  s.first_encoded = s.needs_halo ? s.first_frame : s.first_frame + 1;
  return s;
}

struct ClipEncoder::Impl : EncodeGeometry {
  ClipEncoderConfig c;
  Shard sh;
  uint32_t iters = 0;
  uint64_t record_bytes = 0, seg_ws_bytes = 0;
  static constexpr int kMaxDepth = 3, kSets = kMaxDepth + 2;
  int depth = 1, nsets = 1;
  uint32_t nch = 1, cp = 0;
  struct Micro { uint32_t step = 0, p0 = 0, pn = 0; bool first = true; uint8_t order = 0; const uint8_t* frames = nullptr; };
  static constexpr int kRing = 8;
  Micro ring[kRing], next_micro;
  uint32_t n_steps = 0;
  const uint8_t* step_frames = nullptr;
  Event e_step[kRing];
  uint64_t step_last_micro[kRing] = {};
  void MarkStepDone(uint64_t d) {
    const uint32_t s = StepOf(d);
    if (step_last_micro[s % kRing] == d) Hip(hipEventRecord(e_step[s % kRing], sM), "hipEventRecord");
  }
  const Micro& At(uint64_t m) const { return ring[(int)(m % (uint64_t)kRing)]; }
  uint32_t StepOf(uint64_t m) const { return At(m).step; }
  uint32_t P0(uint64_t m) const { return At(m).p0; }
  uint32_t Pn(uint64_t m) const { return At(m).pn; }
  int Slot(uint64_t m) const { return (int)(m % (uint64_t)nsets); }
  DevBuf<uint8_t> bgr, pyr[2], mask[kSets], seg_ws[kMaxDepth], records[kSets + 1];
  DevBuf<float> mv[kSets], mad[kSets], gm[kSets], rmse[kSets], coeffs[kSets + 1];
  DevBuf<uint8_t> redo_ws[kMaxDepth];
  DevBuf<uint32_t> count[kSets], types[kSets], samples;
  DevBuf<uint8_t> compact, compact_ws;
  DevBuf<uint64_t> compact_off;
  std::vector<svc_step_pair> budget_ladder;
  DevBuf<uint32_t> compact_budget, compact_choice;
  Event e_pyr[2], e_halo[2], e_fork, e_join[kSets], e_rfork, e_rmse[kSets];
  bool halo_recorded[2] = {false, false}, join_pending[kSets] = {}, rmse_pending[kSets] = {};
  bool defer_rmse = false;
  uint64_t iter = 0, fork_iter[kSets] = {};
  void* comm = nullptr;
  HaloFn halo;
  uint64_t n_luma = 0, n_hbma = 0, n_lat = 0, n_dct = 0;
  uint32_t lat_flags = 0;
  bool fused_records = false;
  bool one_bgr_pass = false;
  int rec_sets = 1;
  DevBuf<uint8_t>& Records(uint64_t m) { return records[(int)(StepOf(m) % (uint32_t)rec_sets)]; }
  bool spec_quant = false;
  int coeff_sets = 1;
  DevBuf<float>& Coeffs(uint64_t m) { return coeffs[coeff_sets > 1 ? (int)(StepOf(m) % (uint32_t)coeff_sets) : 0]; }
  bool GrowCoeffSets() {
    if (coeff_sets == rec_sets) return true;
    while (n_dct < n_luma) Iterate(false, last_timed);
    for (int b = 1; b < rec_sets; ++b)
      if (!coeffs[b].TryAlloc(coeffs[0].n)) {
        for (int k = 1; k < b; ++k) coeffs[k].Free();
        spec_quant = false;
        return false;
      }
    coeff_sets = rec_sets;
    return true;
  }
  bool spec_step[kSets + 1] = {};
  bool& SpecStep(uint64_t m) { return spec_step[(int)(m % (uint64_t)(kSets + 1))]; }
  static constexpr int kFgSlots = 8;
  static constexpr double kSpecMaxShare = 0.02;
  static constexpr uint64_t kSpecMinPixels = 50000000ull;
  static constexpr uint64_t kChunkMinPixels = 300000000ull;
  static constexpr uint64_t kIdleRuleMinPixels = 400000000ull;
  static constexpr uint32_t kMaxAutoChunks = 1;
  DevBuf<uint32_t> fg_dev;
  PinBuf<uint32_t> fg_host;
  Event e_fg[kFgSlots];
  bool fg_pending[kFgSlots] = {};
  uint64_t fg_blocks[kFgSlots] = {};
  uint64_t n_fg = 0;
  double fg_share = -1.0;
  uint64_t n_spec = 0, n_decided = 0;
  void MeasureForeground(uint64_t m, hipStream_t st) {
    if (!spec_quant || c.two_bgr_passes || c.always_speculate || !Pn(m)) return;
    const int slot = (int)(n_fg % kFgSlots);
    if (fg_pending[slot] && !Ready(e_fg[slot])) return;
    Abi(svc_hip_count_foreground(types[Set(m)].p + (uint64_t)P0(m) * blocks, (uint64_t)Pn(m) * blocks, fg_dev.p + slot, st), "svc_hip_count_foreground");
    Hip(hipMemcpyAsync(fg_host.p + slot, fg_dev.p + slot, 4, hipMemcpyDeviceToHost, st), "hipMemcpyAsync");
    Hip(hipEventRecord(e_fg[slot], st), "hipEventRecord");
    fg_pending[slot] = true;
    fg_blocks[slot] = (uint64_t)Pn(m) * blocks;
    ++n_fg;
  }
  void PollForeground() {
    for (uint64_t k = n_fg; k > 0 && k + kFgSlots > n_fg; --k) {
      const int slot = (int)((k - 1) % kFgSlots);
      if (!fg_pending[slot]) continue;
      if (!Ready(e_fg[slot])) continue;
      fg_share = (double)fg_host.p[slot] / (double)fg_blocks[slot];
      break;
    }
  }
  bool DecideSpeculation(uint64_t m) {
    if (!spec_quant || c.two_bgr_passes) return false;
    ++n_decided;
    bool yes = c.always_speculate;
    if (c.random_policy) {
      const uint32_t s = StepOf(m);
      yes = s == 0 ? false : s == 1 ? !At(m).first : (Hash32(n_decided * kHashStride) & 1u) != 0;
    } else if (!yes) {
      PollForeground();
      yes = fg_share >= 0.0 && fg_share <= kSpecMaxShare;
    }
    n_spec += yes;
    return yes;
  }
  bool WouldReadOnce() {
    if (one_bgr_pass) return true;
    if (!spec_quant || c.two_bgr_passes) return false;
    if (c.always_speculate) return true;
    PollForeground();
    return fg_share >= 0.0 && fg_share <= kSpecMaxShare;
  }
  void ResetPolicy() {
    fg_share = -1.0;
    n_fg = 0;
    for (bool& p : fg_pending) p = false;
  }
  bool last_timed = false;
  std::vector<std::pair<Event, Event>> timed[kStages];
  std::vector<Event> event_pool;

  Event TimingEvent() {
    if (event_pool.empty()) return Event(kWho, true);
    Event e = std::move(event_pool.back());
    event_pool.pop_back();
    return e;
  }

  uint64_t timed_pairs[kStages] = {};
  uint64_t cur_pairs = 0;
  template <typename F> void Run(Stage st, hipStream_t stream, bool timing, F&& fn) {
    if (!timing) { fn(); return; }
    timed_pairs[(uint32_t)st] += cur_pairs;
    Event a = TimingEvent(), b = TimingEvent();
    Hip(hipEventRecord(a, stream), "hipEventRecord");
    fn();
    Hip(hipEventRecord(b, stream), "hipEventRecord");
    timed[(uint32_t)st].emplace_back(std::move(a), std::move(b));
  }

  int Par(uint64_t m) const { return c.schedule == Schedule::kPipelined ? (int)(StepOf(m) & 1u) : 0; }
  int Set(uint64_t m) const { return (int)(StepOf(m) % (uint32_t)nsets); }

  uint32_t Skip() const { return sh.needs_halo ? 0u : 1u; }
  bool decided = false;
  void Decide(uint64_t m) {
    if (At(m).order && spec_quant && Pn(m)) {
      decided = At(m).order == 2;
      ++n_decided;
      n_spec += decided;
      return;
    }
    decided = spec_quant && Pn(m) && DecideSpeculation(m);
    if (decided && coeff_sets != rec_sets && (!At(m).first || !GrowCoeffSets())) {
      decided = false;
      --n_spec;
    }
  }
  template <typename Between> void Luma(uint64_t m, hipStream_t st, bool timing, Between&& between) {
    cur_pairs = Pn(m);
    const int b = Par(m);
    const uint32_t p0 = P0(m), pn = Pn(m), skip = Skip();
    const bool first_chunk = At(m).first;
    if (spec_quant) SpecStep(m) = pn ? decided : false;
    if (pn && (one_bgr_pass || (spec_quant && SpecStep(m)))) {
      const uint8_t* enc = At(m).frames + (uint64_t)(skip + p0) * frame_bytes;
      uint8_t* slots = pyr[b].p + (uint64_t)(1 + skip + p0) * pyr_stride;
      Run(Stage::kTransform, st, timing, [&] {
        if (!one_bgr_pass)
          Abi(svc_hip_dct_quant_luma_frames(enc, frame_bytes, pn, pw, ph, c.dct_block_w, c.bg_step,
                                            Coeffs(m).p + (uint64_t)p0 * 3 * plane_elems, slots, pyr_stride, st), "svc_hip_dct_quant_luma_frames");
        else
          Abi(svc_hip_dct_records_luma_frames(enc, frame_bytes, pn, pw, ph, c.dct_block_w, ph,
                                              Records(m).p + (uint64_t)p0 * record_bytes, record_bytes, slots, pyr_stride, st), "svc_hip_dct_records_luma_frames");
      });
      between();
      cur_pairs = pn;
      Run(Stage::kLumaPyramid, st, timing, [&] {
        if (skip && first_chunk)
          Abi(svc_hip_luma_pyramid_frames(At(m).frames, frame_bytes, 1, pw, ph, c.levels, pyr[b].p + pyr_stride, pyr_stride, st),
              "svc_hip_luma_pyramid_frames");
        Abi(svc_hip_pyramid_levels_frames(slots, pyr_stride, pn, pw, ph, c.levels, st), "svc_hip_pyramid_levels_frames");
      });
      return;
    }
    const uint32_t f0 = first_chunk ? 0u : p0 + skip, f1 = p0 + pn + skip;
    if (f1 <= f0) return;
    Run(Stage::kLumaPyramid, st, timing, [&] {
      Abi(svc_hip_luma_pyramid_frames(At(m).frames + (uint64_t)f0 * frame_bytes, frame_bytes, f1 - f0, pw, ph, c.levels,
                                      pyr[b].p + (uint64_t)(1 + f0) * pyr_stride, pyr_stride, st), "svc_hip_luma_pyramid_frames");
    });
  }

  void Halo(uint64_t m, bool timing) {
    cur_pairs = 0;
    const int b = Par(m);
    Hip(hipEventRecord(e_pyr[b], sM), "hipEventRecord");
    Hip(hipStreamWaitEvent(sC, e_pyr[b], 0), "hipStreamWaitEvent");
    Run(Stage::kHalo, sC, timing, [&] {
      const uint8_t* send = pyr[b].p + (uint64_t)sh.frames * pyr_stride;
      if (halo) halo(send, pyr[b].p, pyr_stride, sC);
      else if (comm) Abi(svc_hip_halo_shift(comm, send, pyr[b].p, pyr_stride, c.rank, c.world, 0, sC), "svc_hip_halo_shift");
      else throw std::runtime_error("svc::ClipEncoder: world > 1 needs SetComm() or SetHaloTransport() before Step()");
    });
    Hip(hipEventRecord(e_halo[b], sC), "hipEventRecord");
    halo_recorded[b] = true;
  }

  void Hbma(uint64_t m, hipStream_t st, bool timing) {
    cur_pairs = Pn(m);
    const uint32_t p0 = P0(m), pn = Pn(m);
    if (!pn) return;
    const int b = Par(m), q = Set(m), k = Slot(m);
    const uint64_t t0 = (sh.needs_halo ? 0 : 1) + p0;
    if (rmse_pending[k]) {
      Hip(hipStreamWaitEvent(st, e_rmse[k], 0), "hipStreamWaitEvent");
      rmse_pending[k] = false;
    }
    Run(Stage::kHbma, st, timing, [&] {
      Abi(svc_hip_hbma_pairs(pyr[b].p + t0 * pyr_stride, pyr[b].p + (t0 + 1) * pyr_stride, pyr_stride, pn, c.levels, pw, ph,
                             c.search_range, c.mv_block, c.mv_block, mv[q].p + (uint64_t)p0 * blocks * 2, mad[q].p + (uint64_t)p0 * blocks,
                             c.hbma_flags, st), "svc_hip_hbma_pairs");
    });
  }

  void Lat(uint64_t m, hipStream_t st, bool timing) {
    cur_pairs = Pn(m);
    const uint32_t p0 = P0(m), pn = Pn(m);
    if (!pn) return;
    const int b = Set(m), k = Slot(m);
    DevBuf<uint8_t>& ws = seg_ws[c.schedule == Schedule::kPipelined ? (int)(m % (uint64_t)depth) : 0];
    const uint64_t g0 = sh.first_encoded - 1 + p0;
    float* gm_c = gm[b].p + (uint64_t)p0 * 2;
    float* rmse_c = rmse[b].p + p0;
    const float* mv_c = mv[b].p + (uint64_t)p0 * blocks * 2;
    uint8_t* mask_c = mask[b].p + (uint64_t)p0 * blocks;
    uint32_t* count_c = count[b].p + p0;
    uint32_t* types_c = types[b].p + (uint64_t)p0 * blocks;
    const uint32_t* samples_c = samples.p + (uint64_t)p0 * iters * c.ransac.subset_sz;
    Run(Stage::kRansac, st, timing, [&] {
      Hip(hipMemsetAsync(gm_c, 0, (size_t)pn * 2 * sizeof(float), st), "hipMemsetAsync");
      Abi(svc_hip_ransac_frames_ex(mv_c, blocks, pn, c.ransac, samples_c, iters, gm_c, rmse_c, mask_c, count_c,
                                   lat_flags | (defer_rmse ? SVC_LAUNCH_DEFER_RMSE : 0u), st), "svc_hip_ransac_frames");
    });
    if (defer_rmse && c.world == 1) {
      Hip(hipEventRecord(e_rfork, st), "hipEventRecord");
      Hip(hipStreamWaitEvent(sC, e_rfork, 0), "hipStreamWaitEvent");
      Abi(svc_hip_ransac_rmse_frames(mv_c, blocks, pn, c.ransac, gm_c, mask_c, count_c, rmse_c, sC), "svc_hip_ransac_rmse_frames");
      Hip(hipEventRecord(e_rmse[k], sC), "hipEventRecord");
      rmse_pending[k] = true;
    }
    Run(Stage::kSegment, st, timing, [&] {
      if (c.segmentation)
        Abi(svc_hip_segment_frames_ex(mask_c, mv_c, mfw, mfh, pn, c.mv_block, c.mv_block, c.segment,
                                      c.seed * 1000003ull + g0, ws.p, seg_ws_bytes, types_c, lat_flags, st),
            "svc_hip_segment_frames");
      else
        Abi(svc_hip_block_types_frames(mask_c, blocks, pn, types_c, st), "svc_hip_block_types_frames");
    });
    MeasureForeground(m, st);
    if (c.schedule == Schedule::kPipelined && OnePassStep(m)) FinishOnePass(m, st, timing);
  }

  bool OnePassStep(uint64_t m) { return Pn(m) && (one_bgr_pass || (spec_quant && SpecStep(m))); }

  void FinishOnePass(uint64_t m, hipStream_t st, bool timing) {
    cur_pairs = Pn(m);
    const uint32_t p0 = P0(m), pn = Pn(m);
    if (!pn || !c.dct_block_w) return;
    const int b = Set(m);
    const uint8_t* enc = At(m).frames + (uint64_t)(Skip() + p0) * frame_bytes;
    const uint32_t* types_c = types[b].p + (uint64_t)p0 * blocks;
    DevBuf<uint8_t>& rws = redo_ws[c.schedule == Schedule::kPipelined ? (int)(m % (uint64_t)depth) : 0];
    Run(Stage::kTypePatch, st, timing, [&] {
      if (one_bgr_pass)
        Abi(svc_hip_wire_patch_types_frames(types_c, pn, pw, ph, ph, c.dct_block_w, c.mv_block, c.mv_block,
                                            Records(m).p + (uint64_t)p0 * record_bytes, record_bytes, 0, st), "svc_hip_wire_patch_types_frames");
      else
        Abi(svc_hip_dct_quant_redo_frames(enc, frame_bytes, pn, pw, ph, c.dct_block_w, types_c, c.mv_block, c.mv_block, c.fg_step,
                                          Coeffs(m).p + (uint64_t)p0 * 3 * plane_elems, rws.p, rws.bytes(), st), "svc_hip_dct_quant_redo_frames");
    });
  }

  void Transform(uint64_t m, hipStream_t st, bool timing) {
    cur_pairs = Pn(m);
    const uint32_t p0 = P0(m), pn = Pn(m);
    if (!pn || !c.dct_block_w) return;
    const int b = Set(m);
    const uint8_t* enc = At(m).frames + (uint64_t)(Skip() + p0) * frame_bytes;
    const uint32_t* types_c = types[b].p + (uint64_t)p0 * blocks;
    if (OnePassStep(m)) {
      if (c.schedule != Schedule::kPipelined) FinishOnePass(m, st, timing);
      return;
    }
    Run(Stage::kTransform, st, timing, [&] {
      if (c.compact && !budget_ladder.empty())
        Abi(svc_hip_dct_pack_levels_budget_frames(enc, frame_bytes, pn, pw, ph, c.dct_block_w, types_c, c.mv_block, c.mv_block,
                                                  budget_ladder.data(), (uint32_t)budget_ladder.size(), compact_budget.p, compact_ws.p,
                                                  compact_ws.bytes(), compact.p, compact.bytes(), compact_off.p, compact_choice.p, st),
            "svc_hip_dct_pack_levels_budget_frames");
      else if (c.compact)
        Abi(svc_hip_dct_pack_levels_frames(enc, frame_bytes, pn, pw, ph, c.dct_block_w, types_c, c.mv_block, c.mv_block, c.fg_step, c.bg_step,
                                           compact_ws.p, compact_ws.bytes(), compact.p, compact.bytes(), compact_off.p, st),
            "svc_hip_dct_pack_levels_frames");
      else if (c.wire && fused_records)
        Abi(svc_hip_dct_records_frames(enc, frame_bytes, pn, pw, ph, c.dct_block_w, types_c, c.mv_block, c.mv_block,
                                       0, 0, ph, Records(m).p + (uint64_t)p0 * record_bytes, record_bytes, st), "svc_hip_dct_records_frames");
      else if (c.wire) {
        float* planes = coeffs[0].p + (uint64_t)p0 * 3 * plane_elems;
        Abi(svc_hip_dct_frames(enc, frame_bytes, pn, pw, ph, c.dct_block_w, c.dct_block_h, planes, st), "svc_hip_dct_frames");
        Abi(svc_hip_serialize_frames(planes, plane_elems, pn, types_c, pw, ph, c.dct_block_w, c.dct_block_h, mfw, mfh,
                                     c.mv_block, c.mv_block, Records(m).p + (uint64_t)p0 * record_bytes, record_bytes, st), "svc_hip_serialize_frames");
      } else
        Abi(svc_hip_dct_quant_frames(enc, frame_bytes, pn, pw, ph, c.dct_block_w, c.dct_block_h, types_c, c.mv_block,
                                     c.mv_block, c.fg_step, c.bg_step, Coeffs(m).p + (uint64_t)p0 * 3 * plane_elems, st), "svc_hip_dct_quant_frames");
    });
  }

  void ForkLat(uint64_t l, bool timing) {
    hipStream_t st = sL[l % (uint64_t)depth];
    Hip(hipEventRecord(e_fork, sM), "hipEventRecord");
    Hip(hipStreamWaitEvent(st, e_fork, 0), "hipStreamWaitEvent");
    Lat(l, st, timing);
    Hip(hipEventRecord(e_join[Slot(l)], st), "hipEventRecord");
    join_pending[Slot(l)] = true;
    fork_iter[Slot(l)] = iter;
    if (defer_rmse && c.world > 1 && Pn(l)) {
      const int b = Set(l);
      const uint32_t p0 = P0(l), pn = Pn(l);
      Abi(svc_hip_ransac_rmse_frames(mv[b].p + (uint64_t)p0 * blocks * 2, blocks, pn, c.ransac, gm[b].p + (uint64_t)p0 * 2,
                                     mask[b].p + (uint64_t)p0 * blocks, count[b].p + p0, rmse[b].p + p0, st), "svc_hip_ransac_rmse_frames");
      Hip(hipEventRecord(e_rmse[Slot(l)], st), "hipEventRecord");
      rmse_pending[Slot(l)] = true;
    }
  }
  void JoinLat(uint64_t l) {
    if (!join_pending[Slot(l)]) return;
    Hip(hipStreamWaitEvent(sM, e_join[Slot(l)], 0), "hipStreamWaitEvent");
    join_pending[Slot(l)] = false;
  }

  void Iterate(bool new_step, bool timing) {
    if (new_step) {
      ring[(int)(n_luma % (uint64_t)kRing)] = next_micro;
      Decide(n_luma);
    }
    const uint64_t lumas_before = n_luma, hbmas = n_hbma, lats = n_lat;
    const bool do_lat = n_lat < hbmas;
    const uint64_t l = n_lat, d = n_dct;
    const bool do_dct = n_dct < lats && (!new_step || iter - fork_iter[Slot(d)] >= (uint64_t)depth);
    const bool fork_late = c.fork_behind_front && c.world == 1 && new_step && next_micro.pn && (one_bgr_pass || (spec_quant && decided));
    if (do_lat && !fork_late) ForkLat(l, timing);
    const bool reorder = c.search_after_transform && c.world == 1;
    bool hbma_done = false;
    auto pending_searches = [&](uint64_t upto) {
      while (n_hbma < upto) { Hbma(n_hbma, sM, timing); ++n_hbma; }
    };
    if (new_step) {
      const uint64_t m = n_luma;
      const int b = Par(m);
      if (c.world > 1 && halo_recorded[b])
        Hip(hipStreamWaitEvent(sM, e_halo[b], 0), "hipStreamWaitEvent");
      Luma(m, sM, timing, [&] {
        if (do_lat && fork_late) ForkLat(l, timing);
        if (reorder) { pending_searches(lumas_before); hbma_done = true; }
      });
      if (c.world > 1) Halo(m, timing);
      ++n_luma;
    }
    if (reorder) {
      if (do_dct) { JoinLat(d); Transform(d, sM, timing); MarkStepDone(d); }
      if (!hbma_done) pending_searches(n_luma);
      n_lat += do_lat; n_dct += do_dct;
      ++iter;
      return;
    }
    const bool do_hbma = (c.world > 1 && new_step) ? n_hbma < lumas_before : n_hbma < n_luma;
    const uint64_t h = n_hbma;
    if (do_hbma && c.world > 1) Hip(hipStreamWaitEvent(sM, e_halo[Par(h)], 0), "hipStreamWaitEvent");
    if (do_hbma) Hbma(h, sM, timing);
    if (do_dct) {
      JoinLat(d);
      Transform(d, sM, timing);
      MarkStepDone(d);
    }
    n_hbma += do_hbma; n_lat += do_lat; n_dct += do_dct;
    ++iter;
  }

  void SerialStep(bool timing) {
    const uint64_t s = n_luma;
    ring[(int)(s % (uint64_t)kRing)] = Micro{n_steps++, 0u, sh.pairs, true, 0, step_frames};
    step_last_micro[(n_steps - 1) % kRing] = s;
    Decide(s);
    const int b = Par(s);
    if (c.world > 1 && halo_recorded[b]) Hip(hipStreamWaitEvent(sM, e_halo[b], 0), "hipStreamWaitEvent");
    Luma(s, sM, timing, [] {});
    if (c.world > 1) {
      Halo(s, timing);
      Hip(hipStreamWaitEvent(sM, e_halo[b], 0), "hipStreamWaitEvent");
    }
    Hbma(s, sM, timing);
    Lat(s, sM, timing);
    Transform(s, sM, timing);
    MarkStepDone(s);
    ++n_luma; ++n_hbma; ++n_lat; ++n_dct;
  }

  Stream sM, sL[kMaxDepth], sC;
};

ClipEncoder::ClipEncoder(const ClipEncoderConfig& config) : p_(new Impl) {
  Impl& m = *p_;
  m.c = config;
  const ClipEncoderConfig& c = m.c;
  if (!c.width || !c.height || !c.levels || c.levels > 16 || !c.mv_block || c.world == 0 || c.rank >= c.world)
    throw std::runtime_error("svc::ClipEncoder: invalid configuration");
  if (c.clip_frames < 2 || c.clip_frames < c.world)
    throw std::runtime_error("svc::ClipEncoder: a clip needs at least two frames and one frame per rank");
  if ((c.dct_block_w == 0) != (c.dct_block_h == 0))
    throw std::runtime_error("svc::ClipEncoder: transform block needs both sides");
  if (c.compact) {
    if (c.wire) throw std::runtime_error("svc::ClipEncoder: compact and wire are two different outputs: choose one");
    if (c.chunk_pairs) throw std::runtime_error("svc::ClipEncoder: compact needs whole-shard launches (chunk_pairs = 0): one launch per step makes the shard's frames one stream");
    if (c.dct_block_w != c.dct_block_h || (c.dct_block_w != 8 && c.dct_block_w != 16))
      throw std::runtime_error("svc::ClipEncoder: compact needs an 8x8 or 16x16 transform block");
    if (c.mv_block % c.dct_block_w != 0) throw std::runtime_error("svc::ClipEncoder: compact needs an MV block that is a multiple of the transform block");
    if (c.fg_step == 0 || c.bg_step == 0) throw std::runtime_error("svc::ClipEncoder: compact needs quant steps > 0");
  }
  m.sh = PlanShard(c.clip_frames, c.world, c.rank);
  if (c.schedule == Schedule::kPipelined) {
    if (!c.standalone_shapes) m.lat_flags |= SVC_LAUNCH_BESIDE;
    if (!c.segment_fork) m.lat_flags |= SVC_LAUNCH_NO_FORK;
  }
  if (c.narrow_attempts) m.lat_flags |= SVC_LAUNCH_NO_WIDE;
  if (c.lat_depth > (uint32_t)Impl::kMaxDepth) throw std::runtime_error("svc::ClipEncoder: lat_depth must be 0..3");
  static_cast<EncodeGeometry&>(m) = EncodeGeometry(c.width, c.height, c.levels, c.mv_block, c.mv_block);
  const bool transform = c.dct_block_w != 0;
  if (c.compact && m.pw % 16 != 0) throw std::runtime_error("svc::ClipEncoder: compact needs a padded width of whole 16-pixel segments");
  m.record_bytes = (c.wire && transform) ? svc_hip_serialized_frame_bytes(m.pw, m.ph, c.dct_block_w, c.dct_block_h) : 0;
  m.iters = svc_hip_ransac_iter_count(c.ransac);
  const uint32_t P = m.sh.pairs, N = m.sh.frames;
  const bool pipelined = c.schedule == Schedule::kPipelined;
  m.depth = 1;
  if (pipelined) m.depth = c.lat_depth ? (int)c.lat_depth : 2;
  m.nsets = !pipelined ? 1 : m.depth + 2;
  m.nch = 1;
  if (pipelined && c.world == 1 && P > 1) {
    if (c.chunk_pairs) m.nch = (P + c.chunk_pairs - 1) / c.chunk_pairs;
    else m.nch = (uint32_t)std::min<uint64_t>(Impl::kMaxAutoChunks, std::max<uint64_t>(1, (uint64_t)P * m.pw * m.ph / Impl::kChunkMinPixels));
    m.nch = std::min(m.nch, P);
  }
  m.cp = P ? (P + m.nch - 1) / m.nch : 0;
  if (m.cp) m.nch = (P + m.cp - 1) / m.cp;
  m.defer_rmse = pipelined && !c.inline_rmse && m.blocks > 8192;
  m.sM = Stream(kWho);
  m.sC = Stream(kWho);
  if (m.defer_rmse) {
    m.e_rfork = Event(kWho);
    for (int b = 0; b < m.nsets; ++b) m.e_rmse[b] = Event(kWho);
  }
  for (int k = 0; k < m.depth; ++k) m.sL[k] = Stream(kWho);
  for (Event* e : {&m.e_pyr[0], &m.e_pyr[1], &m.e_halo[0], &m.e_halo[1], &m.e_fork}) *e = Event(kWho);
  for (int b = 0; b < m.nsets; ++b) m.e_join[b] = Event(kWho);
  for (Event& e : m.e_step) e = Event(kWho);
  m.bgr.Alloc(kWho, (size_t)N * m.frame_bytes);
  for (int b = 0; b < (pipelined ? 2 : 1); ++b) {
    m.pyr[b].Alloc(kWho, (size_t)(N + 1) * m.pyr_stride);
    Hip(hipMemset(m.pyr[b].p, 0, (size_t)(N + 1) * m.pyr_stride), "hipMemset");
  }
  for (int b = 0; b < m.nsets; ++b) {
    m.mv[b].Alloc(kWho, (size_t)P * m.blocks * 2); m.mad[b].Alloc(kWho, (size_t)P * m.blocks);
    m.gm[b].Alloc(kWho, (size_t)P * 2); m.rmse[b].Alloc(kWho, P);
    m.mask[b].Alloc(kWho, (size_t)P * m.blocks); m.count[b].Alloc(kWho, P); m.types[b].Alloc(kWho, (size_t)P * m.blocks);
  }
  m.seg_ws_bytes = c.segmentation ? svc_hip_segment_workspace_bytes(m.mfw, m.mfh, std::max(m.cp, 1u), c.segment.attempt_count) : 0;
  for (int k = 0; k < m.depth; ++k) m.seg_ws[k].Alloc(kWho, m.seg_ws_bytes);
  m.fused_records = c.wire && c.dct_block_w == c.dct_block_h && c.dct_block_w <= 64 && c.dct_block_w % 2 == 0;
  m.one_bgr_pass = m.fused_records && !c.two_bgr_passes && transform && (c.dct_block_w == 8 || c.dct_block_w == 16) && m.pw % 16 == 0 &&
                   c.mv_block % c.dct_block_w == 0 && P > 0;
  m.spec_quant = !c.wire && !c.compact && !c.two_bgr_passes && transform && c.dct_block_w == c.dct_block_h && (c.dct_block_w == 8 || c.dct_block_w == 16) &&
                 m.pw % 16 == 0 && c.mv_block % 16 == 0 && c.mv_block % c.dct_block_w == 0 && c.fg_step > 0 && c.bg_step > 0 && P > 0 &&
                 (c.always_speculate || c.idle_rule_any_size || (uint64_t)P * m.pw * m.ph >= Impl::kSpecMinPixels);
  m.rec_sets = (m.one_bgr_pass || m.spec_quant) && pipelined ? (m.nsets + 1 + (int)m.nch - 1) / (int)m.nch : 1;
  if (transform) {
    if (c.wire)
      for (int b = 0; b < m.rec_sets; ++b) m.records[b].Alloc(kWho, (size_t)P * m.record_bytes);
    if (c.compact) {
      m.compact.Alloc(kWho, svc_hip_levels_max_bytes(P, m.pw, m.ph, c.dct_block_w, c.dct_block_h, c.mv_block, c.mv_block));
      m.compact_off.Alloc(kWho, (size_t)P + 1);
      m.compact_ws.Alloc(kWho, svc_hip_dct_pack_levels_workspace_bytes(P, m.pw, m.ph, c.dct_block_w, c.mv_block, c.mv_block));
    } else if (!c.wire || !m.fused_records)
      m.coeffs[0].Alloc(kWho, (size_t)P * 3 * m.plane_elems);
    if (m.spec_quant) {
      for (int k = 0; k < m.depth; ++k) m.redo_ws[k].Alloc(kWho, svc_hip_dct_redo_workspace_bytes(m.cp, m.pw, m.ph, c.mv_block, c.mv_block));
      m.fg_dev.Alloc(kWho, Impl::kFgSlots);
      m.fg_host.Alloc(kWho, Impl::kFgSlots);
      for (Event& e : m.e_fg) e = Event(kWho);
    }
  }
  {
    const size_t n = (size_t)P * m.iters * c.ransac.subset_sz;
    std::vector<uint32_t> h(std::max<size_t>(n, 1));
    FillRansacDraws(h.data(), m.sh.first_encoded - 1, P, m.iters, c.ransac.subset_sz, m.blocks, c.seed);
    m.samples.Alloc(kWho, n);
    if (n) Hip(hipMemcpy(m.samples.p, h.data(), n * sizeof(uint32_t), hipMemcpyHostToDevice), "hipMemcpy");
  }
  Hip(hipDeviceSynchronize(), "hipDeviceSynchronize");
}

ClipEncoder::~ClipEncoder() = default;
const Shard& ClipEncoder::shard() const { return p_->sh; }
uint32_t ClipEncoder::padded_width() const { return p_->pw; }
uint32_t ClipEncoder::padded_height() const { return p_->ph; }
uint32_t ClipEncoder::blocks() const { return p_->blocks; }
uint64_t ClipEncoder::pyramid_stride() const { return p_->pyr_stride; }
uint32_t ClipEncoder::steps_submitted() const { return p_->n_steps; }
uint32_t ClipEncoder::chunks_per_step() const { return p_->nch; }
uint32_t ClipEncoder::output_sets() const { return (uint32_t)(p_->one_bgr_pass ? p_->rec_sets : p_->coeff_sets); }

void ClipEncoder::ResetPolicy() {
  Sync();
  p_->ResetPolicy();
}

void ClipEncoder::PolicyInfo(uint64_t* chunks_decided, uint64_t* chunks_speculated, double* foreground_share) {
  Sync();
  p_->PollForeground();
  if (chunks_decided) *chunks_decided = p_->n_decided;
  if (chunks_speculated) *chunks_speculated = p_->n_spec;
  if (foreground_share) *foreground_share = p_->fg_share;
}

void ClipEncoder::LoadFrames(const uint8_t* src, uint32_t first_local, uint32_t n, bool src_on_device) {
  Impl& m = *p_;
  if (!src || (uint64_t)first_local + n > m.sh.frames) throw std::runtime_error("svc::ClipEncoder: LoadFrames out of range");
  Sync();
  if (!m.c.keep_foreground_prior) m.ResetPolicy();
  Hip(hipMemcpy(m.bgr.p + (size_t)first_local * m.frame_bytes, src, (size_t)n * m.frame_bytes,
                src_on_device ? hipMemcpyDeviceToDevice : hipMemcpyHostToDevice), "hipMemcpy");
  Hip(hipStreamSynchronize(nullptr), "hipStreamSynchronize");
}

void ClipEncoder::SetComm(void* nccl_comm) { p_->comm = nccl_comm; }
void ClipEncoder::SetHaloTransport(HaloFn fn) { p_->halo = std::move(fn); }

void ClipEncoder::Step(bool timed) { StepOn(p_->bgr.p, timed); }

uint32_t ClipEncoder::StepFrames(const uint8_t* device_frames, bool timed) {
  if (!device_frames) throw std::runtime_error("svc::ClipEncoder: StepFrames needs the shard's frames in device memory");
  if (reinterpret_cast<uintptr_t>(device_frames) % 16 != 0) throw std::runtime_error("svc::ClipEncoder: StepFrames: the frames must be 16-byte aligned");
  StepOn(device_frames, timed);
  return p_->n_steps - 1;
}

void ClipEncoder::WaitStep(uint32_t step) {
  Impl& m = *p_;
  if (step >= m.n_steps) throw std::runtime_error("svc::ClipEncoder: WaitStep of a step that has not been submitted");
  if (m.n_steps - step > (uint32_t)Impl::kRing) step = m.n_steps - (uint32_t)Impl::kRing;
  if (m.step_last_micro[step % Impl::kRing] >= m.n_dct) Flush();
  Hip(hipEventSynchronize(m.e_step[step % Impl::kRing]), "hipEventSynchronize");
}

void ClipEncoder::StepOn(const uint8_t* frames, bool timed) {
  Impl& m = *p_;
  m.last_timed = timed;
  m.step_frames = frames;
  if (m.c.schedule != Schedule::kPipelined) { m.SerialStep(timed); return; }
  const uint32_t P = m.sh.pairs;
  uint32_t n = m.nch, cp = m.cp;
  uint8_t order[2] = {0, 0};
  const bool idle = !m.c.chunk_pairs && !m.c.compact && m.c.world == 1 && !m.c.whole_shard_steps && m.n_dct == m.n_luma && P >= 2 &&
                    (m.c.idle_rule_any_size || (uint64_t)P * m.pw * m.ph >= Impl::kIdleRuleMinPixels);
  if (idle && !m.WouldReadOnce()) {
    n = 2; cp = (P + 1) / 2;
    if (m.spec_quant && !m.c.two_bgr_passes && m.c.mixed_steps && m.fg_share < 0.0) { order[0] = 1; order[1] = 2; }
  }
  for (uint32_t k = 0; k < n; ++k) {
    const uint32_t p0 = std::min(P, k * cp);
    m.next_micro = Impl::Micro{m.n_steps, p0, std::min(cp, P - p0), k == 0, n == 2 ? order[k] : (uint8_t)0, frames};
    if (k + 1 == n) m.step_last_micro[m.n_steps % Impl::kRing] = m.n_luma;
    m.Iterate(true, timed);
  }
  ++m.n_steps;
}

void ClipEncoder::SetCompactBudget(const svc_step_pair* ladder, uint32_t ladder_len, uint32_t bytes_per_frame) {
  Sync();
  Impl& m = *p_;
  const ClipEncoderConfig& c = m.c;
  if (!c.compact) throw std::runtime_error("svc::ClipEncoder: a byte budget is a setting of the compact stream (compact)");
  if (ladder_len == 0) { m.budget_ladder.clear(); return; }
  const uint32_t P = m.sh.pairs;
  Abi(svc_hip_dct_pack_levels_budget_frames(nullptr, m.frame_bytes, 0, m.pw, m.ph, c.dct_block_w, nullptr, c.mv_block, c.mv_block, ladder, ladder_len,
                                            nullptr, nullptr, ~0ull, nullptr, ~0ull, nullptr, nullptr, nullptr),
      "svc_hip_dct_pack_levels_budget_frames");
  if (!m.compact_budget.p) {
    m.compact_ws.Alloc(kWho, svc_hip_dct_pack_levels_budget_workspace_bytes(P, m.pw, m.ph, c.dct_block_w, c.mv_block, c.mv_block, 64));
    m.compact_budget.Alloc(kWho, std::max(P, 1u));
    m.compact_choice.Alloc(kWho, std::max(P, 1u));
    Hip(hipMemset(m.compact_choice.p, 0, m.compact_choice.bytes()), "hipMemset");
  }
  const std::vector<uint32_t> b(std::max(P, 1u), bytes_per_frame);
  Hip(hipMemcpy(m.compact_budget.p, b.data(), b.size() * sizeof(uint32_t), hipMemcpyHostToDevice), "hipMemcpy");
  m.budget_ladder.assign(ladder, ladder + ladder_len);
}

void ClipEncoder::Flush() {
  Impl& m = *p_;
  while (m.n_dct < m.n_luma) m.Iterate(false, m.last_timed);
}

void ClipEncoder::Sync() {
  Flush();
  for (const Stream* s : {&p_->sC, &p_->sL[0], &p_->sL[1], &p_->sL[2], &p_->sM})
    if (*s) Hip(hipStreamSynchronize(*s), "hipStreamSynchronize");
}

uint64_t ClipEncoder::StagePairs(Stage s) {
  Sync();
  return p_->timed_pairs[(uint32_t)s];
}

void ClipEncoder::StageTime(Stage s, double* total_ms, uint32_t* launches) {
  Sync();
  double t = 0;
  for (auto& pr : p_->timed[(uint32_t)s]) {
    float ms = 0;
    Hip(hipEventElapsedTime(&ms, pr.first, pr.second), "hipEventElapsedTime");
    t += ms;
  }
  if (total_ms) *total_ms = t;
  if (launches) *launches = (uint32_t)p_->timed[(uint32_t)s].size();
}

void ClipEncoder::ResetTimers() {
// ... 221 lines not shown
```

### scalable_video_codec_amd/csrc/luma_pyramid.hip

```cpp
#include "luma16.hpp"
#include "svc_common.hpp"

namespace svc {

struct LumaArgs {
  const uint8_t* bgr;
  uint64_t frame_stride;
  uint8_t* pyr;
  uint64_t pyr_stride;
  uint32_t groups_per_frame;
  uint32_t total_groups;
};

__global__ __launch_bounds__(256) void luma_kernel(LumaArgs a) {
  const uint32_t g = blockIdx.x * 256u + threadIdx.x;
  if (g >= a.total_groups) return;
  const uint32_t frame = g / a.groups_per_frame, gi = g - frame * a.groups_per_frame;
  const uint4* src = reinterpret_cast<const uint4*>(a.bgr + (size_t)frame * a.frame_stride + (size_t)gi * 48);
  const uint4 v0 = src[0], v1 = src[1], v2 = src[2];
  const uint32_t w[12] = {v0.x, v0.y, v0.z, v0.w, v1.x, v1.y, v1.z, v1.w, v2.x, v2.y, v2.z, v2.w};
  uint32_t out[4];
  luma16(w, out);
  uint4* dst = reinterpret_cast<uint4*>(a.pyr + (size_t)frame * a.pyr_stride + (size_t)gi * 16);
  *dst = make_uint4(out[0], out[1], out[2], out[3]);
}

typedef uint32_t u32x4_a4 __attribute__((ext_vector_type(4), aligned(4)));

struct PyrDownArgs {
  uint8_t* pyr;
  uint64_t pyr_stride;
  uint64_t src_off, dst_off;
  uint32_t sw, sh;
  uint32_t dw, dh;
  uint32_t quads_per_row;
  uint32_t total;
  uint32_t bytewise;
};

__device__ __forceinline__ int reflect101(int i, int n) {
  i = i < 0 ? -i : i;
  return i >= n ? 2 * (n - 1) - i : i;
}

__global__ __launch_bounds__(256) void pyr_down_kernel(PyrDownArgs a) {
  const uint32_t q = xcd_contiguous_block(blockIdx.x, gridDim.x) * 256u + threadIdx.x;
  if (q >= a.total) return;
  const uint32_t pairs = (a.dh + 1) / 2, per_frame = pairs * a.quads_per_row;
  const uint32_t frame = q / per_frame, rem = q - frame * per_frame;
  const uint32_t dp = rem / a.quads_per_row, dq = rem - dp * a.quads_per_row;
  const uint32_t dy = 2 * dp;
  const uint8_t* src = a.pyr + (size_t)frame * a.pyr_stride + a.src_off;
  const int sx0 = (int)dq * 8;
  const bool border = dq == 0 || dq + 1 == a.quads_per_row || a.bytewise != 0;

  uint32_t acc0[4] = {0, 0, 0, 0}, acc1[4] = {0, 0, 0, 0};
  const uint32_t taps[5] = {1, 4, 6, 4, 1};
  const uint8_t* rows[7];
#pragma unroll
  for (int r = 0; r < 7; ++r)
    rows[r] = src + (size_t)reflect101(min((int)dy * 2 + r - 2, 2 * (int)a.sh - 2), (int)a.sh) * a.sw;
  constexpr uint32_t kTaps = 1u | (4u << 8) | (6u << 16) | (4u << 24);

  uint32_t h[7][4];
  if (!border) {
    u32x4_a4 w[7];
#pragma unroll
    for (int r = 0; r < 7; ++r) w[r] = *reinterpret_cast<const u32x4_a4*>(rows[r] + sx0 - 4);
#pragma unroll
    for (int r = 0; r < 7; ++r) {
      const uint32_t w0 = w[r].x, w1 = w[r].y, w2 = w[r].z, w3 = w[r].w;
      h[r][0] = __builtin_amdgcn_udot4(__builtin_amdgcn_alignbyte(w1, w0, 2), kTaps, (w1 >> 16) & 0xFFu, false);
      h[r][1] = __builtin_amdgcn_udot4(w1, kTaps, w2 & 0xFFu, false);
      h[r][2] = __builtin_amdgcn_udot4(__builtin_amdgcn_alignbyte(w2, w1, 2), kTaps, (w2 >> 16) & 0xFFu, false);
      h[r][3] = __builtin_amdgcn_udot4(w2, kTaps, w3 & 0xFFu, false);
    }
  } else {
#pragma unroll
    for (int r = 0; r < 7; ++r) {
      uint32_t px[11];
#pragma unroll
      for (int i = 0; i < 11; ++i)
        px[i] = rows[r][min(max(reflect101(sx0 - 2 + i, (int)a.sw), 0), (int)a.sw - 1)];
#pragma unroll
      for (int o = 0; o < 4; ++o) h[r][o] = px[2 * o] + 4 * px[2 * o + 1] + 6 * px[2 * o + 2] + 4 * px[2 * o + 3] + px[2 * o + 4];
    }
  }
#pragma unroll
  for (int r = 0; r < 7; ++r)
#pragma unroll
    for (int o = 0; o < 4; ++o) {
      if (r < 5) acc0[o] += taps[r] * h[r][o];
      if (r >= 2) acc1[o] += taps[r - 2] * h[r][o];
    }
  uint32_t out0 = 0, out1 = 0;
#pragma unroll
  for (int o = 0; o < 4; ++o) {
    out0 |= ((acc0[o] + 128u) >> 8) << (8 * o);
    out1 |= ((acc1[o] + 128u) >> 8) << (8 * o);
  }
  uint8_t* dst = a.pyr + (size_t)frame * a.pyr_stride + a.dst_off;
  if (a.bytewise) {
    const uint32_t n = min(4u, a.dw - dq * 4);
    for (uint32_t o = 0; o < n; ++o) {
      dst[(size_t)dy * a.dw + dq * 4 + o] = (uint8_t)(out0 >> (8 * o));
      if (dy + 1 < a.dh) dst[(size_t)(dy + 1) * a.dw + dq * 4 + o] = (uint8_t)(out1 >> (8 * o));
    }
    return;
  }
  *reinterpret_cast<uint32_t*>(dst + (size_t)dy * a.dw + dq * 4) = out0;
  if (dy + 1 < a.dh) *reinterpret_cast<uint32_t*>(dst + (size_t)(dy + 1) * a.dw + dq * 4) = out1;
}

constexpr int kTW = 128, kTH = 32, kOff = 16, kPitch = kTW + 2 * kOff;
static_assert(kPitch % 16 == 0 && kOff % 16 == 0, "LDS rows keep 16-byte alignment for the ds_write_b128");

struct LumaPyr1Args {
  const uint8_t* bgr;
  uint64_t frame_stride;
  uint8_t* pyr;
  uint64_t pyr_stride;
  uint64_t src_off;
  uint64_t dst_off;
  uint32_t w, h;
  uint32_t tiles_x, tiles_per_frame, total_tiles;
};

__device__ __forceinline__ uint32_t luma_of(uint32_t b, uint32_t g, uint32_t r) {
  return (1868u * b + 9617u * g + 4899u * r + 8192u) >> 14;
}

__device__ __forceinline__ void luma_pyr1_tile(const LumaPyr1Args& a, uint32_t t, uint8_t* tile) {
  const uint32_t tid = threadIdx.x;
  const uint32_t frame = t / a.tiles_per_frame, tr = t - frame * a.tiles_per_frame;
  const uint32_t ty = tr / a.tiles_x, tx = tr - ty * a.tiles_x;
  const int x0 = (int)tx * kTW, y0 = (int)ty * kTH;
  const int w = (int)a.w, h = (int)a.h;
  const int segs = min(kTW, w - x0) / 16;
  const int xe = x0 + segs * 16;
  const uint8_t* src = a.bgr + (size_t)frame * a.frame_stride;
  uint8_t* y_plane = a.pyr + (size_t)frame * a.pyr_stride;

  const int rows = min(kTH + 4, h - y0 + 3);
  for (int task = (int)tid; task < rows * segs; task += 256) {
    const int r = task / segs, sgm = task - r * segs;
    const int y = y0 - 2 + r, yr = reflect101(y, h);
    const int x = x0 + sgm * 16;
    const uint4* p = reinterpret_cast<const uint4*>(src + ((size_t)yr * w + x) * 3);
    const uint4 v0 = p[0], v1 = p[1], v2 = p[2];
    const uint32_t wd[12] = {v0.x, v0.y, v0.z, v0.w, v1.x, v1.y, v1.z, v1.w, v2.x, v2.y, v2.z, v2.w};
    uint32_t out[4];
    luma16(wd, out);
    const uint4 o4 = make_uint4(out[0], out[1], out[2], out[3]);
    *reinterpret_cast<uint4*>(&tile[r * kPitch + kOff + sgm * 16]) = o4;
    if (r >= 2 && r < kTH + 2 && y < h) *reinterpret_cast<uint4*>(y_plane + (size_t)y * w + x) = o4;
  }
  for (int task = (int)tid; task < rows * 4; task += 256) {
    const int r = task >> 2, k = task & 3;
    const int yr = reflect101(y0 - 2 + r, h);
    const int x = k < 2 ? x0 - 2 + k : xe + (k - 2);
    const uint8_t* p = src + ((size_t)yr * w + reflect101(x, w)) * 3;
    tile[r * kPitch + kOff + (x - x0)] = (uint8_t)luma_of(p[0], p[1], p[2]);
  }
  __syncthreads();

  constexpr int kQuads = kTW / 8;
  constexpr uint32_t kTaps = 1u | (4u << 8) | (6u << 16) | (4u << 24);
  constexpr int taps[5] = {1, 4, 6, 4, 1};
  for (int task = (int)tid; task < kQuads * (kTH / 2); task += 256) {
    const int q = task % kQuads, oy = task / kQuads;
    const int gx = (x0 >> 1) + 4 * q, gy = (y0 >> 1) + oy;
    if (gx >= (w >> 1) || gy >= (h >> 1)) continue;
    uint32_t acc[4] = {0, 0, 0, 0};
#pragma unroll
    for (int r = 0; r < 5; ++r) {
      const uint8_t* rowp = &tile[(2 * oy + r) * kPitch + kOff + 8 * q];
      const uint32_t w0 = *reinterpret_cast<const uint32_t*>(rowp - 4);
      const uint2 mid = *reinterpret_cast<const uint2*>(rowp);
      const uint32_t w3 = *reinterpret_cast<const uint32_t*>(rowp + 8);
      const uint32_t h0 = __builtin_amdgcn_udot4(__builtin_amdgcn_alignbyte(mid.x, w0, 2), kTaps, (mid.x >> 16) & 0xFFu, false);
      const uint32_t h1 = __builtin_amdgcn_udot4(mid.x, kTaps, mid.y & 0xFFu, false);
      const uint32_t h2 = __builtin_amdgcn_udot4(__builtin_amdgcn_alignbyte(mid.y, mid.x, 2), kTaps, (mid.y >> 16) & 0xFFu, false);
      const uint32_t h3 = __builtin_amdgcn_udot4(mid.y, kTaps, w3 & 0xFFu, false);
      acc[0] += (uint32_t)taps[r] * h0;
      acc[1] += (uint32_t)taps[r] * h1;
      acc[2] += (uint32_t)taps[r] * h2;
      acc[3] += (uint32_t)taps[r] * h3;
    }
#pragma unroll
    for (int o = 0; o < 1; ++o) {
      if (gy + o >= (h >> 1)) break;
      uint32_t out = 0;
#pragma unroll
      for (int k = 0; k < 4; ++k) out |= ((acc[k] + 128u) >> 8) << (8 * k);
      *reinterpret_cast<uint32_t*>(y_plane + a.dst_off + (size_t)gy * (w >> 1) + gx) = out;
    }
  }
}

__global__ __launch_bounds__(256) void luma_pyr1_kernel(LumaPyr1Args a) {
  __shared__ __attribute__((aligned(16))) uint8_t tile[(kTH + 4) * kPitch + 16];
  const uint32_t t = xcd_contiguous_block(blockIdx.x, gridDim.x);
  if (t < a.total_tiles) luma_pyr1_tile(a, t, tile);
}

struct PyrStripArgs {
  uint8_t* pyr;
  uint64_t pyr_stride, src_off, dst_off;
  uint32_t sw, sh;
  uint32_t strips, bands, total_waves;
};

typedef uint16_t u16x2_t __attribute__((ext_vector_type(2)));
__device__ __forceinline__ uint32_t pk_mad(uint32_t a, uint16_t k, uint32_t c) {
  return __builtin_bit_cast(uint32_t, (u16x2_t)(__builtin_bit_cast(u16x2_t, a) * k + __builtin_bit_cast(u16x2_t, c)));
}

template <int OB>
__global__ __launch_bounds__(256) void pyr_strip_kernel(PyrStripArgs a, const uint8_t* __restrict__ pyr_in, uint8_t* __restrict__ pyr_out) {
  const uint32_t lane = threadIdx.x & 63u;
  const uint32_t wv = __builtin_amdgcn_readfirstlane(xcd_contiguous_block(blockIdx.x, gridDim.x) * 4u + (threadIdx.x >> 6));
  if (wv >= a.total_waves) return;
  const uint32_t strip = wv % a.strips, t = wv / a.strips, band = t % a.bands, frame = t / a.bands;
  const int w = (int)a.sw, h = (int)a.sh, dw = w >> 1, dh = h >> 1;
  const int x0 = (int)strip * 512, valid = min(512, w - x0), la = valid / 8 - 1, xe = x0 + valid;
  const int oy0 = (int)band * OB, rows = min(OB, dh - oy0);
  const uint8_t* src = pyr_in + (size_t)frame * a.pyr_stride + a.src_off;
  uint8_t* dst = pyr_out + (size_t)frame * a.pyr_stride + a.dst_off;

  const uint32_t col = (uint32_t)x0 + min(lane, (uint32_t)la) * 8u;
  const bool last = lane == (uint32_t)la;
  const uint32_t hcol_l = x0 ? (uint32_t)x0 - 4u : 0u, hcol_r = xe < w ? (uint32_t)xe : (uint32_t)w - 4u;
  const uint32_t hsel_l = x0 ? 0x0c030c02u : 0x0c010c02u, hsel_r = xe < w ? 0x0c0c0c00u : 0x0c0c0c02u;
  uint32_t hcol = col, hsel = 0x0c0c0c0cu;
  if (lane == 0) { hcol = hcol_l; hsel = hsel_l; }
  if (last) { hcol = hcol_r; hsel = hsel_r; }

  struct Row { uint32_t e0, o0, e1, o1; };
  auto row_offset = [&](int r) { return (uint32_t)reflect101(min(2 * oy0 - 2 + r, h), h) * (uint32_t)w; };
  auto split = [&](const uint2& v) {
    Row r;
    r.e0 = v.x & 0x00FF00FFu; r.o0 = __builtin_amdgcn_perm(0u, v.x, 0x0c030c01u);
    r.e1 = v.y & 0x00FF00FFu; r.o1 = __builtin_amdgcn_perm(0u, v.y, 0x0c030c01u);
    return r;
  };

  constexpr int kRows = 2 * OB + 3;
  uint2 rv[kRows];
  uint32_t hh[kRows];
#pragma unroll
  for (int r = 0; r < kRows; ++r) hh[r] = 0;
  if (lane == 0 || last) {
#pragma unroll
    for (int r = 0; r < kRows; ++r) hh[r] = *reinterpret_cast<const uint32_t*>(src + row_offset(r) + hcol);
  }
#pragma unroll
  for (int r = 0; r < kRows; ++r) hh[r] = __builtin_amdgcn_perm(0u, hh[r], hsel);
#pragma unroll
  for (int r = 0; r < kRows; ++r)
    rv[r] = *reinterpret_cast<const uint2*>(src + row_offset(r) + col);

  constexpr uint32_t k8 = 0x00080008u;
  Row s, e;
  uint32_t s_h, e_h;
  {
    const Row r0 = split(rv[0]), r1 = split(rv[1]);
    e = split(rv[2]);
    s.e0 = (r1.e0 << 2) + r0.e0 + k8; s.o0 = (r1.o0 << 2) + r0.o0 + k8;
    s.e1 = (r1.e1 << 2) + r0.e1 + k8; s.o1 = (r1.o1 << 2) + r0.o1 + k8;
    s_h = (hh[1] << 2) + hh[0] + k8; e_h = hh[2];
  }
  uint8_t* out = dst + (size_t)oy0 * dw + (x0 >> 1) + 4 * lane;
  const bool mine = lane <= (uint32_t)la;
#pragma unroll
  for (int i = 0; i < OB; ++i) {
    const Row o = split(rv[3 + 2 * i]), n = split(rv[4 + 2 * i]);
    Row v;
    { const uint32_t q = o.e0 << 2; v.e0 = pk_mad(e.e0, 6, s.e0) + q + n.e0; s.e0 = q + e.e0 + k8; }
    { const uint32_t q = o.o0 << 2; v.o0 = pk_mad(e.o0, 6, s.o0) + q + n.o0; s.o0 = q + e.o0 + k8; }
    { const uint32_t q = o.e1 << 2; v.e1 = pk_mad(e.e1, 6, s.e1) + q + n.e1; s.e1 = q + e.e1 + k8; }
    { const uint32_t q = o.o1 << 2; v.o1 = pk_mad(e.o1, 6, s.o1) + q + n.o1; s.o1 = q + e.o1 + k8; }
    e = n;
    uint32_t v_h;
    { const uint32_t q = hh[3 + 2 * i] << 2; v_h = pk_mad(e_h, 6, s_h) + q + hh[4 + 2 * i]; s_h = q + e_h + k8; e_h = hh[4 + 2 * i]; }
    const uint32_t pe = __builtin_amdgcn_update_dpp(v_h << 16, v.e1, 0x138, 0xf, 0xf, false);
    const uint32_t po = __builtin_amdgcn_update_dpp(v_h, v.o1, 0x138, 0xf, 0xf, false);
    uint32_t ne = __builtin_amdgcn_update_dpp(v_h, v.e0, 0x130, 0xf, 0xf, false);
    ne = last ? v_h : ne;
    const uint32_t l2a = __builtin_amdgcn_alignbyte(v.e0, pe, 2), l1a = __builtin_amdgcn_alignbyte(v.o0, po, 2);
    const uint32_t mid = __builtin_amdgcn_alignbyte(v.e1, v.e0, 2), l1b = __builtin_amdgcn_alignbyte(v.o1, v.o0, 2);
    const uint32_t r2b = __builtin_amdgcn_alignbyte(ne, v.e1, 2);
    const uint32_t qa = pk_mad(v.e0, 6, ((l1a + v.o0) << 2) + l2a + mid);
    const uint32_t qb = pk_mad(v.e1, 6, ((l1b + v.o1) << 2) + mid + r2b);
    const uint32_t px = __builtin_amdgcn_perm(qb, qa, 0x07050301u);
    if (mine && i < rows) *reinterpret_cast<uint32_t*>(out) = px;
    out += dw;
  }
}

__global__ __launch_bounds__(256) void luma_any_kernel(const uint8_t* bgr, uint64_t frame_stride, uint8_t* pyr, uint64_t pyr_stride,
                                                        uint32_t px_per_frame, uint32_t total) {
  const uint32_t i = blockIdx.x * 256u + threadIdx.x;
  if (i >= total) return;
  const uint32_t frame = i / px_per_frame, p = i - frame * px_per_frame;
  const uint8_t* s = bgr + (size_t)frame * frame_stride + (size_t)p * 3;
  pyr[(size_t)frame * pyr_stride + p] = (uint8_t)luma_of(s[0], s[1], s[2]);
}

int launch_luma_pyramid(const uint8_t* d_bgr, uint64_t frame_stride, uint32_t n_frames, uint32_t w,
                        uint32_t h, uint32_t levels, uint8_t* d_pyr, uint64_t pyr_stride,
                        hipStream_t stream) {
  if (n_frames == 0) return SVC_OK;
  if (w % 16 != 0) {
    const uint64_t px = (uint64_t)w * h, tot = px * n_frames;
    if (tot > 0x7FFFFFFFull) return fail(SVC_ERR_UNSUPPORTED, "luma: too many pixels for one launch");
    hipLaunchKernelGGL(luma_any_kernel, dim3((uint32_t)((tot + 255) / 256)), dim3(256), 0, stream, d_bgr, frame_stride, d_pyr,
                       pyr_stride, (uint32_t)px, (uint32_t)tot);
    int rc0 = check_launch("luma_any_kernel");
    if (rc0) return rc0;
    return launch_pyr_down_levels(d_pyr, pyr_stride, n_frames, w, h, levels, 0, stream);
  }
  LumaArgs la;
  la.bgr = d_bgr;
  la.frame_stride = frame_stride;
  la.pyr = d_pyr;
  la.pyr_stride = pyr_stride;
  la.groups_per_frame = (uint32_t)(((uint64_t)w * h) / 16);
  const uint64_t tg = (uint64_t)la.groups_per_frame * n_frames;
  if (tg > 0x7FFFFFFFull) return fail(SVC_ERR_UNSUPPORTED, "luma: too many pixels for one launch");
  la.total_groups = (uint32_t)tg;
  int rc;
  uint32_t first_plain_level = 0;
  if (levels >= 2 && (w / 2) % 4 == 0 && h % 2 == 0) {
    LumaPyr1Args fa{};
    fa.bgr = d_bgr;
    fa.frame_stride = frame_stride;
    fa.pyr = d_pyr;
    fa.pyr_stride = pyr_stride;
    fa.dst_off = (uint64_t)w * h;
    fa.w = w; fa.h = h;
    fa.tiles_x = div_up(w, kTW);
    fa.tiles_per_frame = fa.tiles_x * div_up(h, kTH);
    const uint64_t tt = (uint64_t)fa.tiles_per_frame * n_frames;
    if (tt > 0x7FFFFFFFull) return fail(SVC_ERR_UNSUPPORTED, "luma: too many tiles for one launch");
    fa.total_tiles = (uint32_t)tt;
    hipLaunchKernelGGL(luma_pyr1_kernel, dim3(fa.total_tiles), dim3(256), 0, stream, fa);
    if ((rc = check_launch("luma_pyr1_kernel"))) return rc;
    first_plain_level = 1;
  } else {
// ... 53 lines not shown
```

### scalable_video_codec_amd/csrc/svc_common.hpp

```cpp
#pragma once

#include <hip/hip_runtime.h>

#include <cstdarg>
#include <cstdint>
#include <cstdio>

#include "svc_hip.h"

namespace svc {

char* last_error_buf();
constexpr int kErrBufSize = 512;

inline int fail(int code, const char* fmt, ...) {
  va_list ap;
  va_start(ap, fmt);
  vsnprintf(last_error_buf(), kErrBufSize, fmt, ap);
  va_end(ap);
  return code;
}

#define SVC_HIP_TRY(expr)                                                       \
  do {                                                                          \
    hipError_t e_ = (expr);                                                     \
    if (e_ != hipSuccess)                                                       \
      return ::svc::fail(SVC_ERR_HIP, "%s failed: %s (%s:%d)", #expr,           \
                         hipGetErrorString(e_), __FILE__, __LINE__);            \
  } while (0)

#define SVC_REQUIRE(cond, ...)                                                  \
  do {                                                                          \
    if (!(cond)) return ::svc::fail(SVC_ERR_INVALID_ARG, __VA_ARGS__);          \
  } while (0)

inline int check_launch(const char* what, const char* pass = nullptr) {
  hipError_t e = hipGetLastError();
  if (e != hipSuccess)
    return fail(SVC_ERR_HIP, "launch of %s%s%s failed: %s", what, pass ? " " : "", pass ? pass : "", hipGetErrorString(e));
  return SVC_OK;
}

inline uint64_t pyramid_bytes(uint32_t w, uint32_t h, uint32_t levels) {
  uint64_t n = 0;
  for (uint32_t l = 0; l < levels; ++l) n += (uint64_t)(w >> l) * (h >> l);
  return n;
}

__host__ __device__ inline uint32_t div_up(uint32_t a, uint32_t b) { return (a + b - 1) / b; }
inline bool aligned(const void* p, uintptr_t a) { return (reinterpret_cast<uintptr_t>(p) & (a - 1)) == 0; }

struct Staging {
  hipStream_t stream = nullptr;
  uint8_t* dev = nullptr;
  uint8_t* pin = nullptr;
  size_t cap = 0;
  hipEvent_t piece[8] = {};
  ~Staging();
  int ensure(size_t bytes);
  int download(const uint8_t* d_src, size_t pin_off, size_t bytes, uint8_t* const* dst, uint32_t n_dst);
};
Staging& host_stage();
void host_copy(void* dst, const void* src, size_t bytes);
int require_device();
inline size_t up256(size_t v) { return (v + 255) & ~(size_t)255; }

__device__ __forceinline__ uint32_t xcd_contiguous_block(uint32_t bid, uint32_t nblocks) {
  const uint32_t q = nblocks >> 3, r = nblocks & 7u, xcd = bid & 7u, k = bid >> 3;
  return (xcd < r ? xcd * (q + 1) : r * (q + 1) + (xcd - r) * q) + k;
}


int launch_stream_probe(const void* d_in, void* d_out, uint64_t bytes, uint32_t reads, uint32_t writes, hipStream_t stream);

int launch_hbma(const uint8_t* d_tracked, const uint8_t* d_anchor, uint64_t pair_stride,
                uint32_t n_pairs, uint32_t levels, uint32_t w, uint32_t h, uint32_t range,
                uint32_t bw, uint32_t bh, float* d_mv, float* d_mad, uint32_t flags,
                hipStream_t stream);
int launch_ebma(const uint8_t* d_tracked, const uint8_t* d_anchor, uint64_t pair_stride,
                uint32_t n_pairs, uint32_t w, uint32_t h, uint32_t range, uint32_t bw,
                uint32_t bh, float* d_mv, float* d_mad, hipStream_t stream);
int launch_dct(const uint8_t* d_bgr, uint64_t frame_stride, uint32_t n_frames, uint32_t w,
               uint32_t h, uint32_t bw, uint32_t bh, const uint32_t* d_types, uint32_t mv_bw,
               uint32_t mv_bh, uint32_t fg_step, uint32_t bg_step, bool quant, float* d_planes,
               hipStream_t stream, uint8_t* d_records = nullptr, uint64_t records_stride = 0,
               uint32_t emit_h = 0, uint8_t* d_luma = nullptr, uint64_t luma_stride = 0);
int launch_dct_quant_speculative(const uint8_t* d_bgr, uint64_t frame_stride, uint32_t n_frames, uint32_t w, uint32_t h, uint32_t block,
                                 uint32_t bg_step, float* d_planes, uint8_t* d_luma, uint64_t luma_stride, hipStream_t stream);
uint64_t dct_redo_workspace_bytes(uint32_t n_frames, uint32_t mv_blocks);
int launch_count_foreground(const uint32_t* d_types, uint64_t n, uint32_t* d_count, hipStream_t stream);
int launch_dct_quant_redo_foreground(const uint8_t* d_bgr, uint64_t frame_stride, uint32_t n_frames, uint32_t w, uint32_t h, uint32_t block,
                                     const uint32_t* d_types, uint32_t mv_bw, uint32_t mv_bh, uint32_t fg_step, float* d_planes,
                                     uint8_t* d_ws, hipStream_t stream);
int launch_wire_patch_types(const uint32_t* d_types, uint32_t n_frames, uint32_t frame_w, uint32_t frame_h, uint32_t emit_h, uint32_t tb,
                            uint32_t mv_bw, uint32_t mv_bh, uint8_t* d_out, uint64_t out_stride, bool force_all, hipStream_t stream);
int launch_dct_tiles(float* d_img, uint32_t w, uint32_t h, uint32_t bw, uint32_t bh, const uint32_t* d_xy, uint32_t n_tiles,
                     hipStream_t stream);
int launch_quant(float* d_coeffs, uint64_t n, uint32_t step, hipStream_t stream);
int launch_quant_frames(float* d_planes, uint32_t n_frames, uint32_t w, uint32_t h,
                        uint32_t mv_bw, uint32_t mv_bh, const uint32_t* d_types,
                        uint32_t fg_step, uint32_t bg_step, hipStream_t stream);
int launch_ransac(const float* d_mv, uint32_t blocks, uint32_t n_frames,
                  svc_ransac_params params, const uint32_t* d_samples, uint32_t iters,
                  float* d_gm, float* d_rmse, uint8_t* d_mask, uint32_t* d_count,
                  uint32_t flags, hipStream_t stream);
int launch_ransac_rmse(const float* d_mv, uint32_t blocks, uint32_t n_frames, svc_ransac_params params, const float* d_gm,
                       const uint8_t* d_mask, const uint32_t* d_count, float* d_rmse, hipStream_t stream);
int launch_block_types(const uint8_t* d_mask, uint64_t n, uint32_t* d_types, hipStream_t stream);
int launch_serialize(const float* d_planes, uint64_t plane_elems, uint32_t n_frames, const uint32_t* d_types,
                     uint32_t mv_blocks, uint32_t frame_w, uint32_t frame_h, uint32_t tbw, uint32_t tbh,
                     uint32_t mfw, uint32_t mv_bw, uint32_t mv_bh, uint8_t* d_out, uint64_t out_stride,
                     hipStream_t stream);
int launch_decode(const float* d_planes, uint32_t n_frames, uint32_t w, uint32_t h, uint32_t block,
                  const uint32_t* d_types, uint32_t mv_bw, uint32_t mv_bh, uint32_t fg_step, uint32_t bg_step,
                  uint32_t gx, uint32_t gy, uint32_t gw, uint32_t gh, float* d_bgr, hipStream_t stream);
int launch_sse(const uint8_t* d_src, uint64_t src_stride, const float* d_rec, uint32_t n_frames, uint32_t w,
               uint32_t h, uint32_t region_w, uint32_t region_h, uint64_t* d_sse, hipStream_t stream);
uint64_t segment_workspace_per_frame(uint32_t n, uint32_t attempts);
int launch_segment(const uint8_t* d_mask, const float* d_mv, uint32_t mfw, uint32_t mfh, uint32_t n_frames,
                   uint32_t mv_bw, uint32_t mv_bh, const svc_segment_params& p, uint64_t seed, uint8_t* d_ws,
                   uint32_t* d_types, uint32_t flags, hipStream_t stream);
uint64_t global_ebma_workspace_bytes(uint32_t range, uint32_t n_pairs);
int launch_global_ebma(const uint8_t* d_tracked, const uint8_t* d_anchor, uint64_t pair_stride, uint32_t n_pairs, uint32_t w,
                       uint32_t h, uint32_t range, uint8_t* d_ws, float* d_gm, float* d_min_mad, bool combine,
                       hipStream_t stream);
int launch_global_avg(const float* d_mv, uint32_t blocks, uint32_t n_frames, float* d_out, hipStream_t stream);
int launch_pyr_down_levels(uint8_t* d_pyr, uint64_t pyr_stride, uint32_t n_frames, uint32_t w, uint32_t h, uint32_t levels,
                           uint32_t first_plain_level, hipStream_t stream);
int launch_luma_pyramid(const uint8_t* d_bgr, uint64_t frame_stride, uint32_t n_frames,
                        uint32_t w, uint32_t h, uint32_t levels, uint8_t* d_pyr,
                        uint64_t pyr_stride, hipStream_t stream);

}
```

### scalable_video_codec_amd/native.py

```python
from __future__ import annotations

import ctypes as C
import os
from typing import Optional, Tuple

import torch

PKG = os.path.dirname(os.path.abspath(__file__))
LIB_PATH = os.path.join(PKG, "libsvc_hip.so")
MOTION_LIB_PATH = os.path.join(PKG, "libsvc_motion.so")

SVC_OK, SVC_ERR_INVALID_ARG, SVC_ERR_UNSUPPORTED, SVC_ERR_HIP, SVC_ERR_NO_DEVICE = range(5)
HBMA_AUTO, HBMA_FORCE_WAVE_PER_BLOCK, HBMA_FORCE_FUSED, HBMA_FORCE_TILED, HBMA_FORCE_LANE = 0, 1, 2, 4, 8


class SvcError(RuntimeError):
    def __init__(self, status: int, message: str):
        super().__init__(f"svc_hip status {status}: {message}")
        self.status = status


class RansacParams(C.Structure):
    _fields_ = [("subset_sz", C.c_uint32), ("inlier_thresh", C.c_float),
                ("success_prob", C.c_float), ("inlier_ratio", C.c_float)]


class SegmentParams(C.Structure):
    _fields_ = [("morph_rect_w", C.c_uint32), ("morph_rect_h", C.c_uint32), ("cluster_count", C.c_uint32),
                ("attempt_count", C.c_uint32), ("max_iter_count", C.c_uint32), ("epsilon", C.c_float),
                ("connectivity", C.c_uint32)]


class StepPair(C.Structure):
    _fields_ = [("fg_step", C.c_uint32), ("bg_step", C.c_uint32)]


class WireHeader(C.Structure):
    _fields_ = [(n, C.c_uint32) for n in ("frame_count", "frame_w", "frame_h", "frame_excess_w", "frame_excess_h",
                                          "transform_block_w", "transform_block_h", "channel_count")]


DEFAULT_SEGMENT = dict(morph_rect_w=3, morph_rect_h=3, cluster_count=10, attempt_count=3, max_iter_count=10,
                       epsilon=1.0, connectivity=4)

_vp = C.c_void_p
_u32, _u64 = C.c_uint32, C.c_uint64

SIGNATURES = {
    "svc_hip_last_error": (C.c_char_p, []),
    "svc_hip_abi_version": (C.c_int, []),
    "svc_hip_device_count": (C.c_int, [C.POINTER(C.c_int)]),
    "svc_hip_tune_host_allocator": (C.c_int, [_u32]),
    "svc_hip_host_tuning_requested": (C.c_int, []),
    "svc_hip_pyramid_bytes": (_u64, [_u32, _u32, _u32]),
    "svc_hip_hbma_pairs": (C.c_int, [_vp, _vp, _u64, _u32, _u32, _u32, _u32, _u32, _u32, _u32, _vp, _vp, _u32, _vp]),
    "svc_hip_hbma_kernel_name": (C.c_char_p, [_u32, _u32, _u32, _u32, _u32, _u32, _u32]),
    "svc_hip_ebma_pairs": (C.c_int, [_vp, _vp, _u64, _u32, _u32, _u32, _u32, _u32, _u32, _vp, _vp, _vp]),
    "svc_hip_ransac_iter_count": (_u32, [RansacParams]),
    "svc_hip_ransac_frames": (C.c_int, [_vp, _u32, _u32, RansacParams, _vp, _u32, _vp, _vp, _vp, _vp, _vp]),
    "svc_hip_ransac_frames_ex": (C.c_int, [_vp, _u32, _u32, RansacParams, _vp, _u32, _vp, _vp, _vp, _vp, _u32, _vp]),
    "svc_hip_ransac_rmse_frames": (C.c_int, [_vp, _u32, _u32, RansacParams, _vp, _vp, _vp, _vp, _vp]),
    "svc_hip_segment_frames_ex": (C.c_int, [_vp, _vp, _u32, _u32, _u32, _u32, _u32, SegmentParams, _u64, _vp, _u64, _vp, _u32, _vp]),
    "svc_hip_block_types_frames": (C.c_int, [_vp, _u32, _u32, _vp, _vp]),
    "svc_hip_probe_stream": (C.c_int, [_vp, _vp, _u64, _u32, _u32, _vp]),
    "svc_hip_segment_workspace_bytes": (_u64, [_u32, _u32, _u32, _u32]),
    "svc_hip_segment_frames": (C.c_int, [_vp, _vp, _u32, _u32, _u32, _u32, _u32, SegmentParams, _u64, _vp, _u64, _vp, _vp]),
    "svc_hip_wire_header": (C.c_int, [_u32] * 8 + [C.POINTER(WireHeader)]),
    "svc_hip_serialized_frame_bytes": (_u64, [_u32, _u32, _u32, _u32]),
    "svc_hip_serialize_frames": (C.c_int, [_vp, _u64, _u32, _vp] + [_u32] * 8 + [_vp, _u64, _vp]),
    "svc_hip_dct_records_frames": (C.c_int, [_vp, _u64, _u32, _u32, _u32, _u32, _vp, _u32, _u32, _u32, _u32, _u32, _vp, _u64, _vp]),
    "svc_hip_decode_frames": (C.c_int, [_vp, _u32, _u32, _u32, _u32, _vp] + [_u32] * 8 + [_vp, _vp]),
    "svc_hip_sse_frames": (C.c_int, [_vp, _u64, _vp] + [_u32] * 5 + [_vp, _vp]),
    "svc_hip_dct_frames": (C.c_int, [_vp, _u64, _u32, _u32, _u32, _u32, _u32, _vp, _vp]),
    "svc_hip_dct_quant_frames": (C.c_int, [_vp, _u64, _u32, _u32, _u32, _u32, _u32, _vp, _u32, _u32, _u32, _u32, _vp, _vp]),
    "svc_hip_quant": (C.c_int, [_vp, _u64, _u32, _vp]),
    "svc_hip_quant_frames": (C.c_int, [_vp, _u32, _u32, _u32, _u32, _u32, _vp, _u32, _u32, _vp]),
    "svc_hip_luma_pyramid_frames": (C.c_int, [_vp, _u64, _u32, _u32, _u32, _u32, _vp, _u64, _vp]),
    "svc_hip_pyramid_levels_frames": (C.c_int, [_vp, _u64, _u32, _u32, _u32, _u32, _vp]),
    "svc_hip_dct_records_luma_frames": (C.c_int, [_vp, _u64, _u32, _u32, _u32, _u32, _u32, _vp, _u64, _vp, _u64, _vp]),
    "svc_hip_wire_patch_types_frames": (C.c_int, [_vp, _u32, _u32, _u32, _u32, _u32, _u32, _u32, _vp, _u64, C.c_int, _vp]),
    "svc_hip_dct_quant_luma_frames": (C.c_int, [_vp, _u64, _u32, _u32, _u32, _u32, _u32, _vp, _vp, _u64, _vp]),
    "svc_hip_dct_redo_workspace_bytes": (_u64, [_u32, _u32, _u32, _u32, _u32]),
    "svc_hip_count_foreground": (C.c_int, [_vp, _u64, _vp, _vp]),
    "svc_hip_dct_quant_redo_frames": (C.c_int, [_vp, _u64, _u32, _u32, _u32, _u32, _vp, _u32, _u32, _u32, _vp, _vp, _u64, _vp]),
    "svc_hip_hbma_host": (C.c_int, [_vp, _vp, _u32, _u32, _u32, _u32, _u32, _u32, _vp, _vp, _u32]),
    "svc_hip_ebma_host": (C.c_int, [_vp, _vp, _u32, _u32, _u32, _u32, _u32, _vp, _vp]),
    "svc_hip_ransac_host": (C.c_int, [_vp, _u32, RansacParams, _vp, _u32, _vp, _vp, _vp, _vp]),
    "svc_hip_dct_host": (C.c_int, [_vp, _u32, _u32, _u32, _u32, _vp]),
    "svc_hip_dct_quant_host": (C.c_int, [_vp, _u32, _u32, _u32, _u32, _vp, _u32, _u32, _u32, _u32, _vp]),
    "svc_hip_quant_host": (C.c_int, [_vp, _u64, _u32]),
    "svc_hip_global_ebma_workspace_bytes": (_u64, [_u32, _u32]),
    "svc_hip_global_ebma_pairs": (C.c_int, [_vp, _vp, _u64, _u32, _u32, _u32, _u32, _vp, _u64, _vp, _vp, _vp]),
    "svc_hip_global_avg_frames": (C.c_int, [_vp, _u32, _u32, _vp, _vp]),
    "svc_hip_global_ebma_host": (C.c_int, [_vp, _vp, _u32, _u32, _u32, _vp, _vp]),
    "svc_hip_global_hbma_host": (C.c_int, [_vp, _vp, _u32, _u32, _u32, _u32, _vp]),
    "svc_hip_global_avg_host": (C.c_int, [_vp, _u32, _vp]),
    "svc_hip_comm_available": (C.c_int, []),
    "svc_hip_comm_info": (C.c_int, [_vp, C.POINTER(_u32), C.POINTER(_u32), C.POINTER(C.c_int32)]),
    "svc_hip_comm_unique_id": (C.c_int, [_vp]),
    "svc_hip_comm_create": (C.c_int, [_vp, _u32, _u32, C.POINTER(_vp)]),
    "svc_hip_comm_destroy": (C.c_int, [_vp]),
    "svc_hip_halo_shift": (C.c_int, [_vp, _vp, _vp, _u64, _u32, _u32, _u32, _vp]),
    "svc_hip_dct_planes_host": (C.c_int, [_vp, _u32, _u32, _u32, _u32, C.POINTER(_vp)]),
    "svc_hip_bgr2yuv_host": (C.c_int, [_vp, _u32, _u32, _vp]),
    "svc_hip_build_pyramid_host": (C.c_int, [_vp, _u32, _u32, _u32, C.POINTER(_vp)]),
    "svc_hip_morph_rect_host": (C.c_int, [_vp, _u32, _u32, _u32, _u32, _u32, _vp]),
    "svc_hip_kmeans_host": (C.c_int, [_vp, _u32, _u32, _u32, _u32, _u32, C.c_float, _u64, _vp, C.POINTER(C.c_double)]),
    "svc_hip_connected_components_host": (C.c_int, [_vp, _u32, _u32, _u32, _vp, C.POINTER(_u32)]),
    "svc_hip_dct_tiles_host": (C.c_int, [_vp, _u32, _u32, _u32, _u32, _vp, _u32]),
    "svc_hip_levels_max_bytes": (_u64, [_u32] * 7),
    "svc_hip_pack_levels_workspace_bytes": (_u64, [_u32] * 5),
    "svc_hip_pack_levels_frames": (C.c_int, [_vp, _vp] + [_u32] * 9 + [_vp, _u64, _vp, _u64, _vp, _vp]),
    "svc_hip_unpack_levels_frames": (C.c_int, [_vp, _u64, _vp] + [_u32] * 7 + [_vp, _u64, _vp, _vp, _vp, _vp]),
    "svc_hip_dct_pack_levels_workspace_bytes": (_u64, [_u32] * 6),
    "svc_hip_dct_pack_levels_frames": (C.c_int, [_vp, _u64] + [_u32] * 4 + [_vp] + [_u32] * 4 + [_vp, _u64, _vp, _u64, _vp, _vp]),
    "svc_hip_levels_drain": (C.c_int, [_vp, _vp] + [_u32] * 7 + [_vp, _u64, _vp]),
    "svc_hip_entropy_max_bytes": (_u64, [_u32] * 7),
    "svc_hip_entropy_workspace_bytes": (_u64, [_u32] * 7),
    "svc_hip_entropy_encode_frames": (C.c_int, [_vp, _u64, _vp] + [_u32] * 7 + [_vp, _u64, _vp, _u64, _vp, _vp, _vp]),
    "svc_hip_entropy_decode_frames": (C.c_int, [_vp, _u64, _vp] + [_u32] * 7 + [_vp, _u64, _vp, _u64, _vp, _vp, _vp]),
    "svc_hip_entropy_drain": (C.c_int, [_vp, _vp] + [_u32] * 7 + [_vp, _u64, _vp]),
    "svc_hip_dct_pack_levels_budget_workspace_bytes": (_u64, [_u32] * 7),
    "svc_hip_dct_pack_levels_budget_frames": (C.c_int, [_vp, _u64] + [_u32] * 4 + [_vp] + [_u32] * 2 + [C.POINTER(StepPair), _u32, _vp, _vp, _u64,
                                                        _vp, _u64, _vp, _vp, _vp]),
    "svc_hip_pack_levels_budget_workspace_bytes": (_u64, [_u32] * 6),
    "svc_hip_pack_levels_budget_frames": (C.c_int, [_vp, _vp] + [_u32] * 7 + [C.POINTER(StepPair), _u32, _vp, _vp, _u64, _vp, _u64, _vp,
                                                                             _vp, _vp]),
    "svc_hip_decode_levels_workspace_bytes": (_u64, [_u32] * 5),
    "svc_hip_decode_levels_frames": (C.c_int, [_vp, _u64, _vp] + [_u32] * 9 + [_vp, _vp, _u64, _vp, _vp, _u32, _u32, _vp, _vp]),
    "svc_hip_gaze_rect": (C.c_int, [_u32] * 8 + [C.POINTER(_u32)]),
    "svc_hip_decode_records_frames": (C.c_int, [_vp, _u64] + [_u32] * 7 + [_vp, _vp, _vp, _u32, _u32, _vp]),
    "svc_hip_wire_layout": (C.c_int, [C.POINTER(WireHeader), _u64, C.POINTER(_u32), C.POINTER(_u64)]),
}

_lib: Optional[C.CDLL] = None


def load() -> C.CDLL:
    global _lib
    if _lib is None:
        if not os.path.exists(LIB_PATH):
            raise FileNotFoundError(
                f"{LIB_PATH} is missing: build it with `python -m scalable_video_codec_amd.build` "
                "(or __graft_entry__.build()); the MI355X path has no CPU fallback")
        lib = C.CDLL(LIB_PATH)
        for name, (res, args) in SIGNATURES.items():
            fn = getattr(lib, name)
            fn.restype, fn.argtypes = res, args
        _lib = lib
    return _lib


def _check(rc: int) -> None:
    if rc != SVC_OK:
        raise SvcError(rc, load().svc_hip_last_error().decode())


def _stream() -> int:
    return torch.cuda.current_stream().cuda_stream


def _bwbh(block) -> Tuple[int, int]:
    return (block, block) if isinstance(block, int) else (int(block[0]), int(block[1]))


def _dev(t: torch.Tensor, dtype) -> int:
    assert t.is_cuda and t.is_contiguous() and t.dtype == dtype, (t.device, t.dtype, t.is_contiguous())
    return t.data_ptr()


def ransac_iter_count(subset_sz=1, inlier_thresh=7.5, success_prob=0.99, inlier_ratio=0.5) -> int:
    return int(load().svc_hip_ransac_iter_count(RansacParams(subset_sz, inlier_thresh, success_prob, inlier_ratio)))


def pyramid_bytes(w: int, h: int, levels: int) -> int:
    return int(load().svc_hip_pyramid_bytes(w, h, levels))


def pyramid_stride(w: int, h: int, levels: int) -> int:
    return (pyramid_bytes(w, h, levels) + 255) // 256 * 256



def hbma_pairs(tracked: torch.Tensor, anchor: torch.Tensor, pair_stride: int, n_pairs: int,
               levels: int, w: int, h: int, search_range: int, block_w: int = 16, block_h: int = 16,
               flags: int = HBMA_AUTO, out: Optional[Tuple[torch.Tensor, torch.Tensor]] = None):
    blocks = (w // block_w) * (h // block_h)
    if out is None:
        mv = torch.empty((n_pairs, blocks, 2), dtype=torch.float32, device=tracked.device)
        mad = torch.empty((n_pairs, blocks), dtype=torch.float32, device=tracked.device)
    else:
        mv, mad = out
    _check(load().svc_hip_hbma_pairs(_dev(tracked, torch.uint8), _dev(anchor, torch.uint8), pair_stride, n_pairs,
                                     levels, w, h, search_range, block_w, block_h,
                                     _dev(mv, torch.float32), _dev(mad, torch.float32), flags, _stream()))
    return mv, mad


def hbma_kernel_name(levels: int, w: int, h: int, search_range: int, block_w: int = 16, block_h: int = 16,
                     flags: int = HBMA_AUTO) -> str:
    name = load().svc_hip_hbma_kernel_name(levels, w, h, search_range, block_w, block_h, flags)
    if name is None:
        msg = load().svc_hip_last_error().decode()
        raise SvcError(SVC_ERR_UNSUPPORTED if "does not cover" in msg else SVC_ERR_INVALID_ARG, msg)
    return name.decode()


def ebma_pairs(tracked: torch.Tensor, anchor: torch.Tensor, pair_stride: int, n_pairs: int, w: int, h: int,
               search_range: int, block_w: int, block_h: int):
    blocks = (w // block_w) * (h // block_h)
    mv = torch.empty((n_pairs, blocks, 2), dtype=torch.float32, device=tracked.device)
    mad = torch.empty((n_pairs, blocks), dtype=torch.float32, device=tracked.device)
    _check(load().svc_hip_ebma_pairs(_dev(tracked, torch.uint8), _dev(anchor, torch.uint8), pair_stride, n_pairs,
                                     w, h, search_range, block_w, block_h,
                                     _dev(mv, torch.float32), _dev(mad, torch.float32), _stream()))
    return mv, mad


LAUNCH_BESIDE = 1
LAUNCH_NO_FORK = 2


def ransac_frames(mv: torch.Tensor, samples: torch.Tensor, gm_in: Optional[torch.Tensor] = None,
                  subset_sz=1, inlier_thresh=7.5, success_prob=0.99, inlier_ratio=0.5, out=None, flags: int = 0):
    frames, blocks, _ = mv.shape
    iters = samples.shape[1] if samples.numel() else 0
    if out is None:
        gm = torch.zeros((frames, 2), dtype=torch.float32, device=mv.device) if gm_in is None else gm_in.clone()
        rmse = torch.empty(frames, dtype=torch.float32, device=mv.device)
        mask = torch.empty((frames, blocks), dtype=torch.uint8, device=mv.device)
        count = torch.empty(frames, dtype=torch.int32, device=mv.device)
    else:
        gm, rmse, mask, count = out
    p = RansacParams(subset_sz, inlier_thresh, success_prob, inlier_ratio)
# ... 34 lines not shown

def segment_frames(mask: torch.Tensor, mv: torch.Tensor, mfw: int, mfh: int, mv_block: int = 16, seed: int = 0,
                   out: Optional[torch.Tensor] = None, workspace: Optional[torch.Tensor] = None, flags: int = 0,
                   **params) -> torch.Tensor:
    frames, blocks = mask.shape
    assert blocks == mfw * mfh
    p = SegmentParams(**{**DEFAULT_SEGMENT, **params})
    need = int(load().svc_hip_segment_workspace_bytes(mfw, mfh, frames, p.attempt_count))
    if workspace is None:
        workspace = torch.empty(need, dtype=torch.uint8, device=mask.device)
    if out is None:
        out = torch.empty((frames, blocks), dtype=torch.int32, device=mask.device)
    _check(load().svc_hip_segment_frames_ex(_dev(mask, torch.uint8), _dev(mv, torch.float32), mfw, mfh, frames,
                                            mv_block, mv_block, p, seed, _dev(workspace, torch.uint8),
                                            workspace.numel(), _dev(out, torch.int32), flags, _stream()))
    return out


def wire_header(clip_frames: int, w: int, h: int, mv_block: int, levels: int, tb: int) -> bytes:
    hdr = WireHeader()
    _check(load().svc_hip_wire_header(clip_frames, w, h, mv_block, mv_block, levels, tb, tb, C.byref(hdr)))
    return bytes(hdr)


def serialized_frame_bytes(frame_w: int, frame_h: int, tbw: int, tbh: int) -> int:
    return int(load().svc_hip_serialized_frame_bytes(frame_w, frame_h, tbw, tbh))


def serialize_frames(planes: torch.Tensor, block_types: torch.Tensor, frame_w: int, frame_h: int, tbw: int,
                     tbh: int, mfw: int, mfh: int, mv_block: int = 16, out: Optional[torch.Tensor] = None) -> torch.Tensor:
    n, _, ph, pw = planes.shape
    per = serialized_frame_bytes(frame_w, frame_h, tbw, tbh)
    if out is None:
        out = torch.empty((n, per), dtype=torch.uint8, device=planes.device)
    _check(load().svc_hip_serialize_frames(_dev(planes, torch.float32), ph * pw, n, _dev(block_types, torch.int32),
                                           frame_w, frame_h, tbw, tbh, mfw, mfh, mv_block, mv_block,
                                           _dev(out, torch.uint8), out.stride(0), _stream()))
    return out


def dct_records_frames(bgr: torch.Tensor, block: int, block_types: torch.Tensor, mv_block: int = 16,
                       fg_step: int = 0, bg_step: int = 0, emit_h: Optional[int] = None,
                       out: Optional[torch.Tensor] = None) -> torch.Tensor:
    n, h, w, _ = bgr.shape
    emit_h = h if emit_h is None else emit_h
    per = serialized_frame_bytes(w, emit_h, block, block)
    if out is None:
        out = torch.empty((n, per), dtype=torch.uint8, device=bgr.device)
    _check(load().svc_hip_dct_records_frames(_dev(bgr, torch.uint8), h * w * 3, n, w, h, block,
                                             _dev(block_types, torch.int32), mv_block, mv_block, fg_step, bg_step,
                                             emit_h, _dev(out, torch.uint8), out.stride(0), _stream()))
    return out


def decode_frames(planes: torch.Tensor, block: int, block_types: torch.Tensor, mv_block: int = 16, fg_step: int = 1,
                  bg_step: int = 640, gaze=(0, 0, 0, 0), out: Optional[torch.Tensor] = None) -> torch.Tensor:
    n, _, h, w = planes.shape
    if out is None:
        out = torch.empty((n, h, w, 3), dtype=torch.float32, device=planes.device)
    _check(load().svc_hip_decode_frames(_dev(planes, torch.float32), n, w, h, block, _dev(block_types, torch.int32),
                                        mv_block, mv_block, fg_step, bg_step, *gaze, _dev(out, torch.float32), _stream()))
    return out


def sse_frames(src_bgr: torch.Tensor, rec: torch.Tensor, region_w: int, region_h: int) -> torch.Tensor:
    n, h, w, _ = src_bgr.shape
    out = torch.empty(n, dtype=torch.int64, device=src_bgr.device)
    _check(load().svc_hip_sse_frames(_dev(src_bgr, torch.uint8), h * w * 3, _dev(rec, torch.float32), n, w, h,
                                     region_w, region_h, _dev(out, torch.int64), _stream()))
    return out


def dct_frames(bgr: torch.Tensor, block, out: Optional[torch.Tensor] = None) -> torch.Tensor:
    n, h, w, _ = bgr.shape
    bw, bh = _bwbh(block)
    if out is None:
        out = torch.empty((n, 3, h, w), dtype=torch.float32, device=bgr.device)
    _check(load().svc_hip_dct_frames(_dev(bgr, torch.uint8), h * w * 3, n, w, h, bw, bh,
                                     _dev(out, torch.float32), _stream()))
    return out


def dct_quant_frames(bgr: torch.Tensor, block, block_types: torch.Tensor, mv_block: int, fg_step: int,
                     bg_step: int, out: Optional[torch.Tensor] = None) -> torch.Tensor:
    n, h, w, _ = bgr.shape
    bw, bh = _bwbh(block)
    if out is None:
        out = torch.empty((n, 3, h, w), dtype=torch.float32, device=bgr.device)
    _check(load().svc_hip_dct_quant_frames(_dev(bgr, torch.uint8), h * w * 3, n, w, h, bw, bh,
                                           _dev(block_types, torch.int32), mv_block, mv_block, fg_step, bg_step,
                                           _dev(out, torch.float32), _stream()))
    return out


def quant_(coeffs: torch.Tensor, step: int) -> torch.Tensor:
    _check(load().svc_hip_quant(_dev(coeffs, torch.float32), coeffs.numel(), step, _stream()))
    return coeffs


def quant_frames_(planes: torch.Tensor, block_types: torch.Tensor, mv_block: int, fg_step: int, bg_step: int):
    n, _, h, w = planes.shape
    _check(load().svc_hip_quant_frames(_dev(planes, torch.float32), n, w, h, mv_block, mv_block,
                                       _dev(block_types, torch.int32), fg_step, bg_step, _stream()))
    return planes


def luma_pyramid_frames(bgr: torch.Tensor, levels: int, out: Optional[torch.Tensor] = None,
                        stride: Optional[int] = None) -> Tuple[torch.Tensor, int]:
    n, h, w, _ = bgr.shape
    stride = pyramid_stride(w, h, levels) if stride is None else stride
    if out is None:
        out = torch.empty(n * stride, dtype=torch.uint8, device=bgr.device)
    _check(load().svc_hip_luma_pyramid_frames(_dev(bgr, torch.uint8), h * w * 3, n, w, h, levels,
                                              _dev(out, torch.uint8), stride, _stream()))
    return out, stride


def dct_records_luma_frames(bgr: torch.Tensor, block: int, levels: int, emit_h: Optional[int] = None,
                            records: Optional[torch.Tensor] = None, pyr: Optional[torch.Tensor] = None,
                            stride: Optional[int] = None) -> Tuple[torch.Tensor, torch.Tensor, int]:
    n, h, w, _ = bgr.shape
    emit_h = h if emit_h is None else emit_h
    per = serialized_frame_bytes(w, emit_h, block, block)
    if records is None:
        records = torch.empty((n, per), dtype=torch.uint8, device=bgr.device)
    stride = pyramid_stride(w, h, levels) if stride is None else stride
    if pyr is None:
        pyr = torch.empty(n * stride, dtype=torch.uint8, device=bgr.device)
    _check(load().svc_hip_dct_records_luma_frames(_dev(bgr, torch.uint8), h * w * 3, n, w, h, block, emit_h, _dev(records, torch.uint8),
                                                  records.stride(0), _dev(pyr, torch.uint8), stride, _stream()))
    _check(load().svc_hip_pyramid_levels_frames(_dev(pyr, torch.uint8), stride, n, w, h, levels, _stream()))
    return records, pyr, stride


def pyramid_levels_frames(pyr: torch.Tensor, stride: int, n: int, w: int, h: int, levels: int) -> torch.Tensor:
    _check(load().svc_hip_pyramid_levels_frames(_dev(pyr, torch.uint8), stride, n, w, h, levels, _stream()))
    return pyr


def dct_quant_luma_frames(bgr: torch.Tensor, block: int, levels: int, bg_step: int = 640, planes: Optional[torch.Tensor] = None,
                          pyr: Optional[torch.Tensor] = None, stride: Optional[int] = None) -> Tuple[torch.Tensor, torch.Tensor, int]:
    n, h, w, _ = bgr.shape
    if planes is None:
        planes = torch.empty((n, 3, h, w), dtype=torch.float32, device=bgr.device)
    stride = pyramid_stride(w, h, levels) if stride is None else stride
    if pyr is None:
        pyr = torch.empty(n * stride, dtype=torch.uint8, device=bgr.device)
    _check(load().svc_hip_dct_quant_luma_frames(_dev(bgr, torch.uint8), h * w * 3, n, w, h, block, bg_step, _dev(planes, torch.float32),
                                                _dev(pyr, torch.uint8), stride, _stream()))
    _check(load().svc_hip_pyramid_levels_frames(_dev(pyr, torch.uint8), stride, n, w, h, levels, _stream()))
    return planes, pyr, stride


def dct_quant_redo_frames(bgr: torch.Tensor, planes: torch.Tensor, block: int, block_types: torch.Tensor, mv_block: int = 16,
                          fg_step: int = 1) -> torch.Tensor:
    n, h, w, _ = bgr.shape
    nbytes = load().svc_hip_dct_redo_workspace_bytes(n, w, h, mv_block, mv_block)
    ws = torch.empty(nbytes, dtype=torch.uint8, device=bgr.device)
    _check(load().svc_hip_dct_quant_redo_frames(_dev(bgr, torch.uint8), h * w * 3, n, w, h, block, _dev(block_types, torch.int32), mv_block,
                                                mv_block, fg_step, _dev(planes, torch.float32), _dev(ws, torch.uint8), nbytes, _stream()))
    return planes


def count_foreground(block_types: torch.Tensor) -> int:
    out = torch.zeros(1, dtype=torch.int32, device=block_types.device)
    _check(load().svc_hip_count_foreground(_dev(block_types, torch.int32) if block_types.numel() else None, block_types.numel(),
                                           _dev(out, torch.int32), _stream()))
    return int(out.item())


def wire_patch_types_frames(records: torch.Tensor, block_types: torch.Tensor, w: int, h: int, block: int, mv_block: int = 16,
                            emit_h: Optional[int] = None, all_tiles: bool = False) -> torch.Tensor:
    n = records.shape[0]
    emit_h = h if emit_h is None else emit_h
    _check(load().svc_hip_wire_patch_types_frames(_dev(block_types, torch.int32), n, w, h, emit_h, block, mv_block, mv_block,
                                                  _dev(records, torch.uint8), records.stride(0), 1 if all_tiles else 0, _stream()))
    return records



def _np_ptr(a):
    return a.ctypes.data_as(_vp)


def hbma_host(tracked_pyr, anchor_pyr, search_range: int, block_w: int = 16, block_h: int = 16,
              flags: int = HBMA_AUTO):
    import numpy as np
    levels = len(tracked_pyr)
    h, w = tracked_pyr[0].shape
    tp = (_vp * levels)(*[_np_ptr(np.ascontiguousarray(p)) for p in tracked_pyr])
    ap = (_vp * levels)(*[_np_ptr(np.ascontiguousarray(p)) for p in anchor_pyr])
    blocks = (w // block_w) * (h // block_h) if block_w and block_h else 0
    mv = np.empty((max(blocks, 1), 2), np.float32)
    mad = np.empty(max(blocks, 1), np.float32)
    _check(load().svc_hip_hbma_host(C.cast(tp, _vp), C.cast(ap, _vp), levels, w, h, search_range, block_w, block_h,
                                    _np_ptr(mv), _np_ptr(mad), flags))
    return mv[:blocks], mad[:blocks]


def ebma_host(tracked, anchor, search_range: int, block_w: int, block_h: int):
    import numpy as np
    h, w = tracked.shape
    blocks = (w // block_w) * (h // block_h)
    mv = np.empty((blocks, 2), np.float32)
    mad = np.empty(blocks, np.float32)
    _check(load().svc_hip_ebma_host(_np_ptr(np.ascontiguousarray(tracked)), _np_ptr(np.ascontiguousarray(anchor)),
                                    w, h, search_range, block_w, block_h, _np_ptr(mv), _np_ptr(mad)))
    return mv, mad


def ransac_host(mv, samples, gm_in=(0.0, 0.0), subset_sz=1, inlier_thresh=7.5, success_prob=0.99,
                inlier_ratio=0.5):
    import numpy as np
    mv = np.ascontiguousarray(mv, np.float32)
    samples = np.ascontiguousarray(samples, np.uint32)
    n = len(mv)
    gm = np.array(gm_in, np.float32)
    rmse = C.c_float(0)
    inl = np.empty(max(n, 1), np.uint32)
    cnt = C.c_uint32(0)
    p = RansacParams(subset_sz, inlier_thresh, success_prob, inlier_ratio)
    iters = samples.size // subset_sz if subset_sz else 0
    _check(load().svc_hip_ransac_host(_np_ptr(mv), n, p, _np_ptr(samples), iters, _np_ptr(gm),
                                      C.cast(C.byref(rmse), _vp), _np_ptr(inl), C.cast(C.byref(cnt), _vp)))
    return gm, np.float32(rmse.value), inl[:cnt.value].copy()


def dct_host(bgr, block):
    import numpy as np
    bgr = np.ascontiguousarray(bgr, np.uint8)
    h, w, _ = bgr.shape
    bw, bh = _bwbh(block)
    out = np.empty((3, h, w), np.float32)
    _check(load().svc_hip_dct_host(_np_ptr(bgr), w, h, bw, bh, _np_ptr(out)))
    return out


def dct_quant_host(bgr, block, block_types, mv_block, fg_step: int, bg_step: int):
    import numpy as np
    bgr = np.ascontiguousarray(bgr, np.uint8)
    bt = np.ascontiguousarray(block_types, np.uint32)
    h, w, _ = bgr.shape
    bw, bh = _bwbh(block)
    mvw, mvh = _bwbh(mv_block)
    out = np.empty((3, h, w), np.float32)
    _check(load().svc_hip_dct_quant_host(_np_ptr(bgr), w, h, bw, bh, _np_ptr(bt), mvw, mvh,
                                         fg_step, bg_step, _np_ptr(out)))
    return out


def quant_host(coeffs, step: int):
    import numpy as np
    out = np.ascontiguousarray(coeffs, np.float32).copy()
    _check(load().svc_hip_quant_host(_np_ptr(out), out.size, step))
    return out


def global_ebma_host(tracked, anchor, search_range: int):
    import numpy as np
    h, w = tracked.shape
    gm = np.zeros(2, np.float32)
    mad = C.c_float(0)
    _check(load().svc_hip_global_ebma_host(_np_ptr(np.ascontiguousarray(tracked)), _np_ptr(np.ascontiguousarray(anchor)), w, h,
                                           search_range, _np_ptr(gm), C.cast(C.byref(mad), _vp)))
    return gm, np.float32(mad.value)


def global_hbma_host(tracked_pyr, anchor_pyr, search_range: int):
    import numpy as np
    levels = len(tracked_pyr)
    h, w = tracked_pyr[0].shape
    tp = (_vp * levels)(*[_np_ptr(np.ascontiguousarray(p)) for p in tracked_pyr])
    ap = (_vp * levels)(*[_np_ptr(np.ascontiguousarray(p)) for p in anchor_pyr])
    gm = np.zeros(2, np.float32)
    _check(load().svc_hip_global_hbma_host(C.cast(tp, _vp), C.cast(ap, _vp), levels, w, h, search_range, _np_ptr(gm)))
    return gm


def global_avg_host(mv):
    import numpy as np
    mv = np.ascontiguousarray(mv, np.float32)
    out = np.zeros(2, np.float32)
    _check(load().svc_hip_global_avg_host(_np_ptr(mv), len(mv), _np_ptr(out)))
    return out


def global_ebma_pairs(tracked: torch.Tensor, anchor: torch.Tensor, pair_stride: int, n_pairs: int, w: int, h: int,
                      search_range: int):
    ws = torch.empty(int(load().svc_hip_global_ebma_workspace_bytes(search_range, n_pairs)), dtype=torch.uint8, device=tracked.device)
    gm = torch.empty((n_pairs, 2), dtype=torch.float32, device=tracked.device)
    mad = torch.empty(n_pairs, dtype=torch.float32, device=tracked.device)
    _check(load().svc_hip_global_ebma_pairs(_dev(tracked, torch.uint8), _dev(anchor, torch.uint8), pair_stride, n_pairs, w, h,
                                            search_range, _dev(ws, torch.uint8), ws.numel(), _dev(gm, torch.float32),
                                            _dev(mad, torch.float32), _stream()))
    return gm, mad


def global_avg_frames(mv: torch.Tensor) -> torch.Tensor:
    frames, blocks, _ = mv.shape
    out = torch.empty((frames, 2), dtype=torch.float32, device=mv.device)
    _check(load().svc_hip_global_avg_frames(_dev(mv, torch.float32), blocks, frames, _dev(out, torch.float32), _stream()))
    return out


def _np(a, dtype):
    import numpy as np
# ... 353 lines not shown
```

Baseline: 126,600.

## Fuse pyramid level-1 downsample into speculative 8x8 DCT-quant kernel

Adds a PYR1 variant of the speculative luma DCT/quant kernel. It stages each 8-row band's luma in LDS together with a 2-row and 2-column halo, then computes the 5-tap Gaussian half-resolution level 1 of the pyramid directly. The separate pyramid pass then starts from level 1, or is skipped when only two levels exist, which avoids re-reading level 0 from global memory. In exchange each workgroup does extra halo BGR loads and luma conversion, uses more LDS, and adds a __syncthreads, which may reduce occupancy of the DCT kernel.

```diff
diff --git a/include/svc_hip.h b/include/svc_hip.h
--- a/include/svc_hip.h
+++ b/include/svc_hip.h
@@ -180,6 +180,10 @@
 int svc_hip_dct_quant_luma_frames(const uint8_t* d_bgr, uint64_t frame_stride_bytes, uint32_t n_frames, uint32_t frame_w,
                                   uint32_t frame_h, uint32_t block, uint32_t bg_step, float* d_planes, uint8_t* d_pyr,
                                   uint64_t pyr_stride_bytes, void* stream);
+int svc_hip_dct_quant_luma_pyr1_frames(const uint8_t* d_bgr, uint64_t frame_stride_bytes, uint32_t n_frames, uint32_t frame_w,
+                                       uint32_t frame_h, uint32_t block, uint32_t bg_step, float* d_planes, uint8_t* d_pyr,
+                                       uint64_t pyr_stride_bytes, void* stream);
+int svc_hip_dct_quant_luma_pyr1_supported(uint32_t frame_w, uint32_t frame_h, uint32_t block, uint32_t level_count);
 int svc_hip_count_foreground(const uint32_t* d_block_types, uint64_t n, uint32_t* d_count, void* stream);
 uint64_t svc_hip_dct_redo_workspace_bytes(uint32_t n_frames, uint32_t frame_w, uint32_t frame_h, uint32_t mv_block_w,
                                           uint32_t mv_block_h);
@@ -323,6 +327,8 @@
                                 void* stream);
 int svc_hip_pyramid_levels_frames(uint8_t* d_pyr, uint64_t pyr_stride_bytes, uint32_t n_frames, uint32_t frame_w,
                                   uint32_t frame_h, uint32_t level_count, void* stream);
+int svc_hip_pyramid_levels_from_frames(uint8_t* d_pyr, uint64_t pyr_stride_bytes, uint32_t n_frames, uint32_t frame_w,
+                                       uint32_t frame_h, uint32_t level_count, uint32_t first_existing_level, void* stream);
 
 uint64_t svc_hip_global_ebma_workspace_bytes(uint32_t search_range, uint32_t n_pairs);
 
diff --git a/scalable_video_codec_amd/csrc/capi.hip b/scalable_video_codec_amd/csrc/capi.hip
--- a/scalable_video_codec_amd/csrc/capi.hip
+++ b/scalable_video_codec_amd/csrc/capi.hip
@@ -539,6 +539,20 @@
   return launch_pyr_down_levels(d_pyr, pyr_stride_bytes, n_frames, frame_w, frame_h, level_count, 0, static_cast<hipStream_t>(stream));
 }
 
+int svc_hip_pyramid_levels_from_frames(uint8_t* d_pyr, uint64_t pyr_stride_bytes, uint32_t n_frames, uint32_t frame_w, uint32_t frame_h,
+                                       uint32_t level_count, uint32_t first_existing_level, void* stream) {
+  if (n_frames == 0) return SVC_OK;
+  SVC_REQUIRE(d_pyr, "pyramid_levels_from: null pointer");
+  SVC_REQUIRE(level_count > 0 && level_count <= 16, "pyramid_levels_from: level_count %u out of range", level_count);
+  SVC_REQUIRE(first_existing_level < level_count, "pyramid_levels_from: level %u is not one of %u levels", first_existing_level, level_count);
+  const uint32_t f = 1u << (level_count - 1);
+  SVC_REQUIRE(frame_w > 0 && frame_h > 0 && frame_w % f == 0 && frame_h % f == 0,
+              "pyramid_levels_from: frame %ux%u must be divisible by 2^(levels-1) = %u", frame_w, frame_h, f);
+  SVC_REQUIRE(n_frames <= 1 || pyr_stride_bytes >= pyramid_bytes(frame_w, frame_h, level_count), "pyramid_levels_from: pyramid stride too small");
+  return launch_pyr_down_levels(d_pyr, pyr_stride_bytes, n_frames, frame_w, frame_h, level_count, first_existing_level,
+                                static_cast<hipStream_t>(stream));
+}
+
 int svc_hip_dct_records_luma_frames(const uint8_t* d_bgr, uint64_t frame_stride_bytes, uint32_t n_frames, uint32_t frame_w,
                                     uint32_t frame_h, uint32_t block, uint32_t emit_frame_h, uint8_t* d_records,
                                     uint64_t records_stride_bytes, uint8_t* d_pyr, uint64_t pyr_stride_bytes, void* stream) {
@@ -569,6 +583,31 @@
               "dct_quant_luma: pyramids must be 16-byte aligned (stride too), a stride of at least one luma plane");
   return launch_dct_quant_speculative(d_bgr, frame_stride_bytes, n_frames, frame_w, frame_h, block, bg_step, d_planes, d_pyr,
                                       pyr_stride_bytes, static_cast<hipStream_t>(stream));
+}
+
+int svc_hip_dct_quant_luma_pyr1_supported(uint32_t frame_w, uint32_t frame_h, uint32_t block, uint32_t level_count) {
+  if (level_count < 2 || level_count > 16) return 0;
+  const uint32_t f = 1u << (level_count - 1);
+  return dct_quant_pyr1_shape_ok(frame_w, frame_h, block) && frame_w % f == 0 && frame_h % f == 0 ? 1 : 0;
+}
+
+int svc_hip_dct_quant_luma_pyr1_frames(const uint8_t* d_bgr, uint64_t frame_stride_bytes, uint32_t n_frames, uint32_t frame_w,
+                                       uint32_t frame_h, uint32_t block, uint32_t bg_step, float* d_planes, uint8_t* d_pyr,
+                                       uint64_t pyr_stride_bytes, void* stream) {
+  if (n_frames == 0) return SVC_OK;
+  int rc = validate_dct(d_bgr, d_planes, frame_w, frame_h, block, block);
+  if (rc) return rc;
+  SVC_REQUIRE(d_pyr, "dct_quant_luma_pyr1: null pyramid");
+  SVC_REQUIRE(bg_step > 0, "dct_quant_luma_pyr1: quant step must be positive (libs/decoder.cpp:35-47)");
+  if (!dct_quant_pyr1_shape_ok(frame_w, frame_h, block))
+    return fail(SVC_ERR_UNSUPPORTED, "dct_quant_luma_pyr1: needs 8x8 blocks, a width that is a multiple of 128 and a height that is a multiple "
+                                     "of 8 (got %ux%u, block %u): call svc_hip_dct_quant_luma_frames", frame_w, frame_h, block);
+  if ((rc = validate_dct_alignment(d_bgr, frame_stride_bytes, d_planes, frame_w, block, block))) return rc;
+  SVC_REQUIRE(aligned(d_pyr, 16) && pyr_stride_bytes % 16 == 0 && pyr_stride_bytes >= pyramid_bytes(frame_w, frame_h, 2),
+              "dct_quant_luma_pyr1: pyramids must be 16-byte aligned (stride too), a stride of at least levels 0 and 1 (%llu bytes)",
+              (unsigned long long)pyramid_bytes(frame_w, frame_h, 2));
+  return launch_dct_quant_speculative(d_bgr, frame_stride_bytes, n_frames, frame_w, frame_h, block, bg_step, d_planes, d_pyr,
+                                      pyr_stride_bytes, static_cast<hipStream_t>(stream), true);
 }
 
 int svc_hip_count_foreground(const uint32_t* d_block_types, uint64_t n, uint32_t* d_count, void* stream) {
diff --git a/scalable_video_codec_amd/csrc/dct.hip b/scalable_video_codec_amd/csrc/dct.hip
--- a/scalable_video_codec_amd/csrc/dct.hip
+++ b/scalable_video_codec_amd/csrc/dct.hip
@@ -2,6 +2,7 @@
 
 #include "dct_core.hpp"
 #include "luma16.hpp"
+#include "pyr1_tile.hpp"
 #include "quant_core.hpp"
 #include "svc_common.hpp"
 
@@ -27,6 +28,7 @@
   const uint32_t* fg_list;
   const uint32_t* fg_count;
   uint32_t segs_per_block_x, segs_per_block;
+  uint32_t wgs_per_band;
 };
 
 
@@ -35,13 +37,17 @@
 
 typedef uint32_t u32x4_a4 __attribute__((ext_vector_type(4), aligned(4)));
 
-template <int N, bool QUANT, bool WIRE, bool LUMA = false, int SPEC = 0>
+constexpr int kP1Off = 16, kP1Pitch = 512 + 2 * kP1Off, kP1Rows = 11;
+static_assert(kP1Pitch % 16 == 0 && kP1Off % 16 == 0, "the tile's rows keep 16-byte alignment for the ds_write_b128");
+
+template <int N, bool QUANT, bool WIRE, bool LUMA = false, int SPEC = 0, bool PYR1 = false>
 __global__ __launch_bounds__(256) void dct_kernel(DctArgs a) {
+  static_assert(!PYR1 || (N == 8 && LUMA && QUANT && SPEC == 1), "level 1 rides on the speculative 8 x 8 transform's luma plane");
   static_assert(!LUMA || (WIRE && !QUANT) || (QUANT && !WIRE && SPEC == 1), "the luma by-product rides on the raw-coefficient record emitter or on the speculative quantiser");
   static_assert(SPEC == 0 || (QUANT && !WIRE), "speculation is about the quantiser's step");
   constexpr int kSegPerWg = 256 / N;
   constexpr int kSlab = WIRE ? (N == 8 ? kSlabWire8 : kSlabWire16) : (N == 8 ? kSlab8 : kSlab16);
-  __shared__ __attribute__((aligned(16))) uint8_t lds[kSegPerWg * kSlab];
+  __shared__ __attribute__((aligned(16))) uint8_t lds[kSegPerWg * kSlab + (PYR1 ? kP1Rows * kP1Pitch : 0)];
 
   const uint32_t tid = threadIdx.x;
   const uint32_t sc_local = tid / N, j = tid % N;
@@ -53,7 +59,18 @@
   }
   for (; unit < n_units; unit += SPEC == 2 ? gridDim.x : 1u) {
   uint32_t gsc, frame, band, seg;
-  if (SPEC == 2) {
+  uint32_t wg_seg0 = 0, wg_segs = kSegPerWg;
+  if (PYR1) {
+    const uint32_t pos = xcd_contiguous_block(blockIdx.x, gridDim.x);
+    const uint32_t band_g = pos / a.wgs_per_band;
+    wg_seg0 = (pos - band_g * a.wgs_per_band) * kSegPerWg;
+    wg_segs = min((uint32_t)kSegPerWg, a.segs_per_band - wg_seg0);
+    seg = wg_seg0 + sc_local;
+    if (seg >= a.segs_per_band) return;
+    gsc = 0;
+    frame = band_g / a.bands_per_frame;
+    band = band_g - frame * a.bands_per_frame;
+  } else if (SPEC == 2) {
     gsc = unit * kSegPerWg + sc_local;
     if (gsc >= *a.fg_count * a.segs_per_block) break;
     const uint32_t item = a.fg_list[gsc / a.segs_per_block], sub = gsc % a.segs_per_block;
@@ -82,10 +99,43 @@
     wds[8] = v2.x; wds[9] = v2.y; wds[10] = v2.z; wds[11] = v2.w;
   }
 
+  uint8_t* p1_tile = lds + kSegPerWg * kSlab;
+  uint32_t p1_seg[12];
+  uint32_t p1_b = 0, p1_g = 0, p1_r = 0;
+  int p1_seg_at = -1, p1_px_at = -1;
+  uint32_t p1_magic = 0;
   if (LUMA) {
     uint32_t y16[4];
     luma16(wds, y16);
-    *reinterpret_cast<uint4*>(a.luma + (size_t)frame * a.luma_stride + (size_t)(y_pix + j) * a.w + x_pix) = make_uint4(y16[0], y16[1], y16[2], y16[3]);
+    const uint4 y4 = make_uint4(y16[0], y16[1], y16[2], y16[3]);
+    *reinterpret_cast<uint4*>(a.luma + (size_t)frame * a.luma_stride + (size_t)(y_pix + j) * a.w + x_pix) = y4;
+    if constexpr (PYR1) {
+      *reinterpret_cast<uint4*>(p1_tile + (2 + j) * kP1Pitch + kP1Off + sc_local * 16) = y4;
+      const uint8_t* fsrc = a.bgr + (size_t)frame * a.frame_stride;
+      const int x0 = (int)wg_seg0 * 16, xe = x0 + (int)wg_segs * 16;
+      const uint32_t nw = wg_segs >> 3;
+      p1_magic = nw == 1 ? 256u : nw == 2 ? 128u : nw == 3 ? 86u : 64u;
+#pragma unroll
+      for (int i = 0; i < 12; ++i) p1_seg[i] = 0;
+      const uint32_t hrow = ((tid >> 3) * p1_magic) >> 8;
+      if (hrow < 3) {
+        const uint32_t sgm = tid - hrow * wg_segs;
+        const int r = hrow < 2 ? (int)hrow : kP1Rows - 1;
+        const int yr = reflect101((int)y_pix - 2 + r, (int)a.h);
+        const uint4* p = reinterpret_cast<const uint4*>(fsrc + ((size_t)yr * a.w + x0 + sgm * 16) * 3);
+        const uint4 v0 = p[0], v1 = p[1], v2 = p[2];
+        p1_seg[0] = v0.x; p1_seg[1] = v0.y; p1_seg[2] = v0.z; p1_seg[3] = v0.w;
+        p1_seg[4] = v1.x; p1_seg[5] = v1.y; p1_seg[6] = v1.z; p1_seg[7] = v1.w;
+        p1_seg[8] = v2.x; p1_seg[9] = v2.y; p1_seg[10] = v2.z; p1_seg[11] = v2.w;
+        p1_seg_at = r * kP1Pitch + kP1Off + (int)sgm * 16;
+      }
+      const int task = (int)tid - ((int)wg_segs * 8 - 4 * kP1Rows);
+      if (task >= 0) {
+        const Pyr1HaloPixel hp = pyr1_halo_pixel<kP1Pitch, kP1Off>(fsrc, (int)a.w, (int)a.h, x0, xe, (int)y_pix, task);
+        p1_b = hp.bgr[0]; p1_g = hp.bgr[1]; p1_r = hp.bgr[2];
+        p1_px_at = hp.tile_index;
+      }
+    }
   }
 
   uint8_t* slab = lds + sc_local * kSlab;
@@ -170,6 +220,20 @@
       }
     }
     wave_lds_sync();
+  }
+
+  if constexpr (PYR1) {
+    if (p1_seg_at >= 0) {
+      uint32_t y16[4];
+      luma16(p1_seg, y16);
+      *reinterpret_cast<uint4*>(p1_tile + p1_seg_at) = make_uint4(y16[0], y16[1], y16[2], y16[3]);
+    }
+    if (p1_px_at >= 0) p1_tile[p1_px_at] = (uint8_t)luma_of(p1_b, p1_g, p1_r);
+    __syncthreads();
+    const uint32_t oy = ((tid >> 4) * p1_magic) >> 8, q = tid - oy * (wg_segs * 2);
+    const int gx = (int)wg_seg0 * 8 + 4 * (int)q, gy = (int)(y_pix >> 1) + (int)oy;
+    pyr1_quad<kP1Pitch, kP1Off>(p1_tile, (int)q, (int)oy, gx, gy, (int)a.w, (int)a.h,
+                                a.luma + (size_t)frame * a.luma_stride + (size_t)a.w * a.h);
   }
 
   if constexpr (WIRE) {
@@ -460,9 +524,13 @@
 }
 
 static bool spec_shape_ok(uint32_t w, uint32_t block) { return (block == 8 || block == 16) && w % 16 == 0; }
+bool dct_quant_pyr1_shape_ok(uint32_t w, uint32_t h, uint32_t block) { return block == 8 && w > 0 && h > 0 && w % 128 == 0 && h % 8 == 0; }
 
 int launch_dct_quant_speculative(const uint8_t* d_bgr, uint64_t frame_stride, uint32_t n_frames, uint32_t w, uint32_t h, uint32_t block,
-                                 uint32_t bg_step, float* d_planes, uint8_t* d_luma, uint64_t luma_stride, hipStream_t stream) {
+                                 uint32_t bg_step, float* d_planes, uint8_t* d_luma, uint64_t luma_stride, hipStream_t stream, bool pyr1) {
+  if (pyr1 && !dct_quant_pyr1_shape_ok(w, h, block))
+    return fail(SVC_ERR_UNSUPPORTED, "dct_quant_luma_pyr1: level 1 from the transform needs 8x8 blocks, a width that is a multiple of 128 and a "
+                                     "height that is a multiple of 8 (got %ux%u, block %u)", w, h, block);
   if (!spec_shape_ok(w, block))
     return fail(SVC_ERR_UNSUPPORTED, "dct_quant_luma: the speculative form needs the tuned transform (8x8 / 16x16 blocks, width a multiple of 16)");
   DctArgs a{};
@@ -478,6 +546,12 @@
   a.luma = d_luma; a.luma_stride = luma_stride;
   a.fg_step = a.bg_step = (float)bg_step;
   a.fg_inv = a.bg_inv = 1.0f / a.bg_step;
+  if (pyr1) {
+    a.wgs_per_band = div_up(a.segs_per_band, 32);
+    const uint64_t wgs = (uint64_t)n_frames * a.bands_per_frame * a.wgs_per_band;
+    hipLaunchKernelGGL((dct_kernel<8, true, false, true, 1, true>), dim3((uint32_t)wgs), dim3(256), 0, stream, a);
+    return check_launch("dct_kernel<speculative, level 1>");
+  }
   const dim3 grid(div_up(a.total_segcols, 256 / block)), blk(256);
   if (block == 8) hipLaunchKernelGGL((dct_kernel<8, true, false, true, 1>), grid, blk, 0, stream, a);
   else hipLaunchKernelGGL((dct_kernel<16, true, false, true, 1>), grid, blk, 0, stream, a);
diff --git a/scalable_video_codec_amd/csrc/host/clip_encoder.cpp b/scalable_video_codec_amd/csrc/host/clip_encoder.cpp
--- a/scalable_video_codec_amd/csrc/host/clip_encoder.cpp
+++ b/scalable_video_codec_amd/csrc/host/clip_encoder.cpp
@@ -82,6 +82,7 @@
   int rec_sets = 1;
   DevBuf<uint8_t>& Records(uint64_t m) { return records[(int)(StepOf(m) % (uint32_t)rec_sets)]; }
   bool spec_quant = false;
+  bool spec_pyr1 = false;
   int coeff_sets = 1;
   DevBuf<float>& Coeffs(uint64_t m) { return coeffs[coeff_sets > 1 ? (int)(StepOf(m) % (uint32_t)coeff_sets) : 0]; }
   bool GrowCoeffSets() {
@@ -209,7 +210,10 @@
       const uint8_t* enc = At(m).frames + (uint64_t)(skip + p0) * frame_bytes;
       uint8_t* slots = pyr[b].p + (uint64_t)(1 + skip + p0) * pyr_stride;
       Run(Stage::kTransform, st, timing, [&] {
-        if (!one_bgr_pass)
+        if (!one_bgr_pass && spec_pyr1)
+          Abi(svc_hip_dct_quant_luma_pyr1_frames(enc, frame_bytes, pn, pw, ph, c.dct_block_w, c.bg_step,
+                                                 Coeffs(m).p + (uint64_t)p0 * 3 * plane_elems, slots, pyr_stride, st), "svc_hip_dct_quant_luma_pyr1_frames");
+        else if (!one_bgr_pass)
           Abi(svc_hip_dct_quant_luma_frames(enc, frame_bytes, pn, pw, ph, c.dct_block_w, c.bg_step,
                                             Coeffs(m).p + (uint64_t)p0 * 3 * plane_elems, slots, pyr_stride, st), "svc_hip_dct_quant_luma_frames");
         else
@@ -218,11 +222,15 @@
       });
       between();
       cur_pairs = pn;
+      const bool tracked_only = skip && first_chunk;
+      const uint32_t have = !one_bgr_pass && spec_pyr1 ? 1u : 0u;
+      if (!tracked_only && have + 1 >= c.levels) return;
       Run(Stage::kLumaPyramid, st, timing, [&] {
-        if (skip && first_chunk)
+        if (tracked_only)
           Abi(svc_hip_luma_pyramid_frames(At(m).frames, frame_bytes, 1, pw, ph, c.levels, pyr[b].p + pyr_stride, pyr_stride, st),
               "svc_hip_luma_pyramid_frames");
-        Abi(svc_hip_pyramid_levels_frames(slots, pyr_stride, pn, pw, ph, c.levels, st), "svc_hip_pyramid_levels_frames");
+        if (have) Abi(svc_hip_pyramid_levels_from_frames(slots, pyr_stride, pn, pw, ph, c.levels, have, st), "svc_hip_pyramid_levels_from_frames");
+        else Abi(svc_hip_pyramid_levels_frames(slots, pyr_stride, pn, pw, ph, c.levels, st), "svc_hip_pyramid_levels_frames");
       });
       return;
     }
@@ -524,6 +532,7 @@
   m.spec_quant = !c.wire && !c.compact && !c.two_bgr_passes && transform && c.dct_block_w == c.dct_block_h && (c.dct_block_w == 8 || c.dct_block_w == 16) &&
                  m.pw % 16 == 0 && c.mv_block % 16 == 0 && c.mv_block % c.dct_block_w == 0 && c.fg_step > 0 && c.bg_step > 0 && P > 0 &&
                  (c.always_speculate || c.idle_rule_any_size || (uint64_t)P * m.pw * m.ph >= Impl::kSpecMinPixels);
+  m.spec_pyr1 = m.spec_quant && svc_hip_dct_quant_luma_pyr1_supported(m.pw, m.ph, c.dct_block_w, c.levels) != 0;
   m.rec_sets = (m.one_bgr_pass || m.spec_quant) && pipelined ? (m.nsets + 1 + (int)m.nch - 1) / (int)m.nch : 1;
   if (transform) {
     if (c.wire)
diff --git a/scalable_video_codec_amd/csrc/luma_pyramid.hip b/scalable_video_codec_amd/csrc/luma_pyramid.hip
--- a/scalable_video_codec_amd/csrc/luma_pyramid.hip
+++ b/scalable_video_codec_amd/csrc/luma_pyramid.hip
@@ -1,4 +1,5 @@
 #include "luma16.hpp"
+#include "pyr1_tile.hpp"
 #include "svc_common.hpp"
 
 namespace svc {
@@ -38,11 +39,6 @@
   uint32_t bytewise;
 };
 
-__device__ __forceinline__ int reflect101(int i, int n) {
-  i = i < 0 ? -i : i;
-  return i >= n ? 2 * (n - 1) - i : i;
-}
-
 __global__ __launch_bounds__(256) void pyr_down_kernel(PyrDownArgs a) {
   const uint32_t q = xcd_contiguous_block(blockIdx.x, gridDim.x) * 256u + threadIdx.x;
   if (q >= a.total) return;
@@ -125,10 +121,6 @@
   uint32_t w, h;
   uint32_t tiles_x, tiles_per_frame, total_tiles;
 };
-
-__device__ __forceinline__ uint32_t luma_of(uint32_t b, uint32_t g, uint32_t r) {
-  return (1868u * b + 9617u * g + 4899u * r + 8192u) >> 14;
-}
 
 __device__ __forceinline__ void luma_pyr1_tile(const LumaPyr1Args& a, uint32_t t, uint8_t* tile) {
   const uint32_t tid = threadIdx.x;
@@ -156,45 +148,17 @@
     if (r >= 2 && r < kTH + 2 && y < h) *reinterpret_cast<uint4*>(y_plane + (size_t)y * w + x) = o4;
   }
   for (int task = (int)tid; task < rows * 4; task += 256) {
-    const int r = task >> 2, k = task & 3;
-    const int yr = reflect101(y0 - 2 + r, h);
-    const int x = k < 2 ? x0 - 2 + k : xe + (k - 2);
-    const uint8_t* p = src + ((size_t)yr * w + reflect101(x, w)) * 3;
-    tile[r * kPitch + kOff + (x - x0)] = (uint8_t)luma_of(p[0], p[1], p[2]);
+    const Pyr1HaloPixel hp = pyr1_halo_pixel<kPitch, kOff>(src, w, h, x0, xe, y0, task);
+    tile[hp.tile_index] = (uint8_t)luma_of(hp.bgr[0], hp.bgr[1], hp.bgr[2]);
   }
   __syncthreads();
 
   constexpr int kQuads = kTW / 8;
-  constexpr uint32_t kTaps = 1u | (4u << 8) | (6u << 16) | (4u << 24);
-  constexpr int taps[5] = {1, 4, 6, 4, 1};
   for (int task = (int)tid; task < kQuads * (kTH / 2); task += 256) {
     const int q = task % kQuads, oy = task / kQuads;
     const int gx = (x0 >> 1) + 4 * q, gy = (y0 >> 1) + oy;
     if (gx >= (w >> 1) || gy >= (h >> 1)) continue;
-    uint32_t acc[4] = {0, 0, 0, 0};
-#pragma unroll
-    for (int r = 0; r < 5; ++r) {
-      const uint8_t* rowp = &tile[(2 * oy + r) * kPitch + kOff + 8 * q];
-      const uint32_t w0 = *reinterpret_cast<const uint32_t*>(rowp - 4);
-      const uint2 mid = *reinterpret_cast<const uint2*>(rowp);
-      const uint32_t w3 = *reinterpret_cast<const uint32_t*>(rowp + 8);
-      const uint32_t h0 = __builtin_amdgcn_udot4(__builtin_amdgcn_alignbyte(mid.x, w0, 2), kTaps, (mid.x >> 16) & 0xFFu, false);
-      const uint32_t h1 = __builtin_amdgcn_udot4(mid.x, kTaps, mid.y & 0xFFu, false);
-      const uint32_t h2 = __builtin_amdgcn_udot4(__builtin_amdgcn_alignbyte(mid.y, mid.x, 2), kTaps, (mid.y >> 16) & 0xFFu, false);
-      const uint32_t h3 = __builtin_amdgcn_udot4(mid.y, kTaps, w3 & 0xFFu, false);
-      acc[0] += (uint32_t)taps[r] * h0;
-      acc[1] += (uint32_t)taps[r] * h1;
-      acc[2] += (uint32_t)taps[r] * h2;
-      acc[3] += (uint32_t)taps[r] * h3;
-    }
-#pragma unroll
-    for (int o = 0; o < 1; ++o) {
-      if (gy + o >= (h >> 1)) break;
-      uint32_t out = 0;
-#pragma unroll
-      for (int k = 0; k < 4; ++k) out |= ((acc[k] + 128u) >> 8) << (8 * k);
-      *reinterpret_cast<uint32_t*>(y_plane + a.dst_off + (size_t)gy * (w >> 1) + gx) = out;
-    }
+    pyr1_quad<kPitch, kOff>(tile, q, oy, gx, gy, w, h, y_plane + a.dst_off);
   }
 }
 
diff --git a/scalable_video_codec_amd/csrc/pyr1_tile.hpp b/scalable_video_codec_amd/csrc/pyr1_tile.hpp
--- /dev/null
+++ b/scalable_video_codec_amd/csrc/pyr1_tile.hpp
@@ -0,0 +1,63 @@
+#ifndef SVC_PYR1_TILE_HPP
+#define SVC_PYR1_TILE_HPP
+
+#include <cstdint>
+
+#include <hip/hip_runtime.h>
+
+namespace svc {
+
+__device__ __forceinline__ int reflect101(int i, int n) {
+  i = i < 0 ? -i : i;
+  return i >= n ? 2 * (n - 1) - i : i;
+}
+
+__device__ __forceinline__ uint32_t luma_of(uint32_t b, uint32_t g, uint32_t r) {
+  return (1868u * b + 9617u * g + 4899u * r + 8192u) >> 14;
+}
+
+struct Pyr1HaloPixel {
+  const uint8_t* bgr;
+  int tile_index;
+};
+template <int kPitch, int kOff>
+__device__ __forceinline__ Pyr1HaloPixel pyr1_halo_pixel(const uint8_t* src, int w, int h, int x0, int xe, int y0, int task) {
+  const int r = task >> 2, k = task & 3;
+  const int yr = reflect101(y0 - 2 + r, h);
+  const int x = k < 2 ? x0 - 2 + k : xe + (k - 2);
+  return {src + ((size_t)yr * w + reflect101(x, w)) * 3, r * kPitch + kOff + (x - x0)};
+}
+
+template <int kPitch, int kOff>
+__device__ __forceinline__ void pyr1_quad(const uint8_t* tile, int q, int oy, int gx, int gy, int w, int h, uint8_t* lvl1) {
+  constexpr uint32_t kTaps = 1u | (4u << 8) | (6u << 16) | (4u << 24);
+  constexpr int taps[5] = {1, 4, 6, 4, 1};
+  uint32_t acc[4] = {0, 0, 0, 0};
+#pragma unroll
+  for (int r = 0; r < 5; ++r) {
+    const uint8_t* rowp = &tile[(2 * oy + r) * kPitch + kOff + 8 * q];
+    const uint32_t w0 = *reinterpret_cast<const uint32_t*>(rowp - 4);
+    const uint2 mid = *reinterpret_cast<const uint2*>(rowp);
+    const uint32_t w3 = *reinterpret_cast<const uint32_t*>(rowp + 8);
+    const uint32_t h0 = __builtin_amdgcn_udot4(__builtin_amdgcn_alignbyte(mid.x, w0, 2), kTaps, (mid.x >> 16) & 0xFFu, false);
+    const uint32_t h1 = __builtin_amdgcn_udot4(mid.x, kTaps, mid.y & 0xFFu, false);
+    const uint32_t h2 = __builtin_amdgcn_udot4(__builtin_amdgcn_alignbyte(mid.y, mid.x, 2), kTaps, (mid.y >> 16) & 0xFFu, false);
+    const uint32_t h3 = __builtin_amdgcn_udot4(mid.y, kTaps, w3 & 0xFFu, false);
+    acc[0] += (uint32_t)taps[r] * h0;
+    acc[1] += (uint32_t)taps[r] * h1;
+    acc[2] += (uint32_t)taps[r] * h2;
+    acc[3] += (uint32_t)taps[r] * h3;
+  }
+#pragma unroll
+  for (int o = 0; o < 1; ++o) {
+    if (gy + o >= (h >> 1)) break;
+    uint32_t out = 0;
+#pragma unroll
+    for (int k = 0; k < 4; ++k) out |= ((acc[k] + 128u) >> 8) << (8 * k);
+    *reinterpret_cast<uint32_t*>(lvl1 + (size_t)gy * (w >> 1) + gx) = out;
+  }
+}
+
+}
+
+#endif
diff --git a/scalable_video_codec_amd/csrc/svc_common.hpp b/scalable_video_codec_amd/csrc/svc_common.hpp
--- a/scalable_video_codec_amd/csrc/svc_common.hpp
+++ b/scalable_video_codec_amd/csrc/svc_common.hpp
@@ -86,7 +86,9 @@
                hipStream_t stream, uint8_t* d_records = nullptr, uint64_t records_stride = 0,
                uint32_t emit_h = 0, uint8_t* d_luma = nullptr, uint64_t luma_stride = 0);
 int launch_dct_quant_speculative(const uint8_t* d_bgr, uint64_t frame_stride, uint32_t n_frames, uint32_t w, uint32_t h, uint32_t block,
-                                 uint32_t bg_step, float* d_planes, uint8_t* d_luma, uint64_t luma_stride, hipStream_t stream);
+                                 uint32_t bg_step, float* d_planes, uint8_t* d_luma, uint64_t luma_stride, hipStream_t stream,
+                                 bool pyr1 = false);
+bool dct_quant_pyr1_shape_ok(uint32_t w, uint32_t h, uint32_t block);
 uint64_t dct_redo_workspace_bytes(uint32_t n_frames, uint32_t mv_blocks);
 int launch_count_foreground(const uint32_t* d_types, uint64_t n, uint32_t* d_count, hipStream_t stream);
 int launch_dct_quant_redo_foreground(const uint8_t* d_bgr, uint64_t frame_stride, uint32_t n_frames, uint32_t w, uint32_t h, uint32_t block,
diff --git a/scalable_video_codec_amd/native.py b/scalable_video_codec_amd/native.py
--- a/scalable_video_codec_amd/native.py
+++ b/scalable_video_codec_amd/native.py
@@ -80,6 +80,9 @@
     "svc_hip_dct_records_luma_frames": (C.c_int, [_vp, _u64, _u32, _u32, _u32, _u32, _u32, _vp, _u64, _vp, _u64, _vp]),
     "svc_hip_wire_patch_types_frames": (C.c_int, [_vp, _u32, _u32, _u32, _u32, _u32, _u32, _u32, _vp, _u64, C.c_int, _vp]),
     "svc_hip_dct_quant_luma_frames": (C.c_int, [_vp, _u64, _u32, _u32, _u32, _u32, _u32, _vp, _vp, _u64, _vp]),
+    "svc_hip_dct_quant_luma_pyr1_frames": (C.c_int, [_vp, _u64, _u32, _u32, _u32, _u32, _u32, _vp, _vp, _u64, _vp]),
+    "svc_hip_dct_quant_luma_pyr1_supported": (C.c_int, [_u32, _u32, _u32, _u32]),
+    "svc_hip_pyramid_levels_from_frames": (C.c_int, [_vp, _u64, _u32, _u32, _u32, _u32, _u32, _vp]),
     "svc_hip_dct_redo_workspace_bytes": (_u64, [_u32, _u32, _u32, _u32, _u32]),
     "svc_hip_count_foreground": (C.c_int, [_vp, _u64, _vp, _vp]),
     "svc_hip_dct_quant_redo_frames": (C.c_int, [_vp, _u64, _u32, _u32, _u32, _u32, _vp, _u32, _u32, _u32, _vp, _vp, _u64, _vp]),
@@ -420,6 +423,26 @@
     return planes, pyr, stride
 
 
+def dct_quant_luma_pyr1_supported(w: int, h: int, block: int, levels: int) -> bool:
+    return bool(load().svc_hip_dct_quant_luma_pyr1_supported(w, h, block, levels))
+
+
+def dct_quant_luma_pyr1_frames(bgr: torch.Tensor, block: int, levels: int, bg_step: int = 640, planes: Optional[torch.Tensor] = None,
+                               pyr: Optional[torch.Tensor] = None, stride: Optional[int] = None, shape: Optional[Tuple[int, int, int]] = None,
+                               frame_stride: Optional[int] = None) -> Tuple[torch.Tensor, torch.Tensor, int]:
+    n, h, w = bgr.shape[:3] if shape is None else shape
+    frame_stride = h * w * 3 if frame_stride is None else frame_stride
+    if planes is None:
+        planes = torch.empty((n, 3, h, w), dtype=torch.float32, device=bgr.device)
+    stride = pyramid_stride(w, h, levels) if stride is None else stride
+    if pyr is None:
+        pyr = torch.empty(n * stride, dtype=torch.uint8, device=bgr.device)
+    _check(load().svc_hip_dct_quant_luma_pyr1_frames(_dev(bgr, torch.uint8), frame_stride, n, w, h, block, bg_step, _dev(planes, torch.float32),
+                                                     _dev(pyr, torch.uint8), stride, _stream()))
+    _check(load().svc_hip_pyramid_levels_from_frames(_dev(pyr, torch.uint8), stride, n, w, h, levels, 1, _stream()))
+    return planes, pyr, stride
+
+
 def dct_quant_redo_frames(bgr: torch.Tensor, planes: torch.Tensor, block: int, block_types: torch.Tensor, mv_block: int = 16,
                           fg_step: int = 1) -> torch.Tensor:
     n, h, w, _ = bgr.shape
```

After: 127,800, median of 6. About the same (+1.0%).
